# rrwick/Autocycler

Measured on NVIDIA H100. Metric: input-assembly Mbp/sec through compress->unitig GFA, higher is better.
Workload: dtype u64

## Files before the change

autocycler_b200/api.py:

```python
import ctypes as C
import os

_HERE = os.path.dirname(os.path.abspath(__file__))
DEFAULT_LIB = os.path.join(_HERE, "libautocycler_gpu.so")

AC_OK = 0


class AutocyclerGpuError(RuntimeError):
    def __init__(self, code, message):
        super().__init__(f"[{code}] {message}")
        self.code = code
        self.message = message


class AcConfig(C.Structure):
    _fields_ = [("k", C.c_uint32), ("device", C.c_int32), ("stream", C.c_void_p), ("keep_positions", C.c_uint32),
                ("n_devices", C.c_int32), ("devices", C.POINTER(C.c_int32))]


class AcCounts(C.Structure):
    _fields_ = [(n, C.c_uint64) for n in ("n_kmers", "n_unitigs", "n_links", "total_length", "seq_bytes", "n_fwd_pos",
                                         "n_rev_pos", "n_next", "n_sequences", "n_path_steps", "length_before_simplify")]


class AcUnitigs(C.Structure):
    _fields_ = [("number", C.POINTER(C.c_uint32)), ("seq_off", C.POINTER(C.c_uint64)), ("seq", C.POINTER(C.c_uint8)),
                ("depth", C.POINTER(C.c_double)),
                ("fpos_off", C.POINTER(C.c_uint64)), ("fpos", C.POINTER(C.c_uint32)), ("fpos_id_strand", C.POINTER(C.c_uint16)),
                ("rpos_off", C.POINTER(C.c_uint64)), ("rpos", C.POINTER(C.c_uint32)), ("rpos_id_strand", C.POINTER(C.c_uint16)),
                ("next_off", C.POINTER(C.c_uint64)), ("next", C.POINTER(C.c_int32))]


class AcTimings(C.Structure):
    _fields_ = [(n, C.c_float) for n in ("h2d", "pack", "insert", "adjacency", "boundaries", "runs", "unitigs", "links", "seed_sort", "emit", "d2h",
                                        "device_total", "host_graph", "host_simplify", "host_gfa", "sample", "device_simplify", "device_gfa", "insert_kernel", "trim_kernel")] + \
               [(n, C.c_uint64) for n in ("insert_occurrences", "table_capacity", "table_used", "kernel_launches", "h2d_bytes", "d2h_bytes")]

    def as_dict(self):
        return {n: getattr(self, n) for n, _ in self._fields_}


class AcResolveInfo(C.Structure):
    _fields_ = [("anchors", C.c_uint32), ("unique_bridges", C.c_uint32), ("conflicting_bridges", C.c_uint32), ("culled_bridges", C.c_uint32),
                ("jobs", C.c_uint64), ("cells", C.c_uint64), ("longest_path", C.c_uint64), ("shared_jobs", C.c_uint32), ("hbm_jobs", C.c_uint32),
                ("kernel_ms", C.c_float)]

    def as_dict(self):
        return {n: getattr(self, n) for n, _ in self._fields_}


EXPORTS = ["ac_last_error", "ac_version", "ac_create", "ac_destroy", "ac_add_sequence", "ac_clear_sequences", "ac_upload",
           "ac_build", "ac_compress", "ac_simplify", "ac_merge_linear_paths", "ac_renumber_unitigs", "ac_load_gfa", "ac_bind_host_to_device", "ac_decompress_gfa", "ac_pairwise_distances", "ac_distance_matrix_text", "ac_sequence_reconstruct", "ac_counts_get", "ac_unitigs_copy", "ac_path_copy", "ac_gfa_size", "ac_gfa_copy",
           "ac_timings_get", "ac_compress_dir", "ac_compress_dir_devices", "ac_load_sequences", "ac_sequence_get",
           "ac_build_local", "ac_entries_count", "ac_entries_export", "ac_entries_merge", "ac_runs_local", "ac_runs_export",
           "ac_runs_import", "ac_runs_import_padded", "ac_build_finish", "ac_compress_finish", "ac_gfa_data",
           "ac_compress_finish_split", "ac_path_tokens_export", "ac_path_lines_render", "ac_path_lines_data", "ac_upload_shard", "ac_strand_block",
           "ac_trim_paths", "ac_trim", "ac_trim_yaml", "ac_trim_stats", "ac_trim_dir",
           "ac_cluster", "ac_cluster_text", "ac_cluster_assignments", "ac_cluster_stats", "ac_upgma", "ac_cluster_dir",
           "ac_bridge_best_paths", "ac_resolve", "ac_resolve_text", "ac_resolve_stats", "ac_resolve_dir", "ac_combine_dir"]

_libs = {}


def load_library(path=None):
    path = os.path.abspath(path or DEFAULT_LIB)
    if path in _libs:
        return _libs[path]
    if not os.path.exists(path):
        raise AutocyclerGpuError(-2, f"{path} is missing: build it with `python -c 'import __graft_entry__ as g; g.build()'` "
                                     "(the GPU path has no CPU fallback)")
    lib = C.CDLL(path)
    lib.ac_last_error.restype = C.c_char_p
    lib.ac_last_error.argtypes = [C.c_void_p]
    lib.ac_version.restype = C.c_char_p
    lib.ac_create.argtypes = [C.POINTER(C.c_void_p), C.POINTER(AcConfig)]
    lib.ac_destroy.argtypes = [C.c_void_p]
    lib.ac_destroy.restype = None
    lib.ac_add_sequence.argtypes = [C.c_void_p, C.c_uint16, C.c_char_p, C.c_uint64, C.c_char_p, C.c_char_p]
    lib.ac_clear_sequences.argtypes = [C.c_void_p]
    for name in ("ac_upload", "ac_build", "ac_compress", "ac_simplify", "ac_renumber_unitigs"):
        getattr(lib, name).argtypes = [C.c_void_p]
    lib.ac_merge_linear_paths.argtypes = [C.c_void_p, C.c_int]
    lib.ac_load_gfa.argtypes = [C.c_void_p, C.c_char_p, C.c_uint64]
    lib.ac_bind_host_to_device.argtypes = [C.c_int32]
    lib.ac_pairwise_distances.argtypes = [C.c_void_p, C.POINTER(C.c_double), C.c_uint64]
    lib.ac_distance_matrix_text.argtypes = [C.c_void_p, C.c_void_p, C.c_uint64, C.POINTER(C.c_uint64)]
    lib.ac_decompress_gfa.argtypes = [C.c_char_p, C.c_char_p, C.c_char_p, C.c_int32, C.c_int32]
    lib.ac_sequence_reconstruct.argtypes = [C.c_void_p, C.c_uint64, C.c_void_p, C.c_uint64, C.POINTER(C.c_uint64)]
    lib.ac_counts_get.argtypes = [C.c_void_p, C.POINTER(AcCounts)]
    lib.ac_unitigs_copy.argtypes = [C.c_void_p, C.POINTER(AcUnitigs)]
    lib.ac_path_copy.argtypes = [C.c_void_p, C.c_uint64, C.POINTER(C.c_int32), C.c_uint64, C.POINTER(C.c_uint64)]
    lib.ac_gfa_size.argtypes = [C.c_void_p, C.POINTER(C.c_uint64)]
    lib.ac_gfa_copy.argtypes = [C.c_void_p, C.c_void_p, C.c_uint64]
    lib.ac_timings_get.argtypes = [C.c_void_p, C.POINTER(AcTimings)]
    lib.ac_compress_dir.argtypes = [C.c_char_p, C.c_char_p, C.c_uint32, C.c_uint32, C.c_uint32, C.c_int32, C.c_int32]
    lib.ac_compress_dir_devices.argtypes = [C.c_char_p, C.c_char_p, C.c_uint32, C.c_uint32, C.c_uint32, C.POINTER(C.c_int32), C.c_int32, C.c_int32]
    lib.ac_load_sequences.argtypes = [C.c_void_p, C.c_char_p, C.c_uint32, C.c_uint32, C.POINTER(C.c_uint64)]
    lib.ac_sequence_get.argtypes = [C.c_void_p, C.c_uint64, C.POINTER(C.c_uint16), C.POINTER(C.c_uint64), C.c_char_p, C.c_uint64,
                                    C.c_char_p, C.c_uint64, C.c_char_p, C.c_uint64]
    lib.ac_build_local.argtypes = [C.c_void_p, C.c_uint32, C.c_uint32, C.c_uint32]
    lib.ac_entries_count.argtypes = [C.c_void_p, C.POINTER(C.c_uint64)]
    lib.ac_entries_export.argtypes = [C.c_void_p, C.c_void_p, C.c_uint64]
    lib.ac_entries_merge.argtypes = [C.c_void_p, C.c_void_p, C.c_uint64]
    lib.ac_runs_local.argtypes = [C.c_void_p, C.POINTER(C.c_uint64)]
    lib.ac_runs_export.argtypes = [C.c_void_p, C.c_void_p, C.c_uint64]
    lib.ac_runs_import.argtypes = [C.c_void_p, C.c_void_p, C.c_uint64]
    lib.ac_runs_import_padded.argtypes = [C.c_void_p, C.c_void_p, C.c_uint64, C.POINTER(C.c_uint64), C.c_uint32]
    lib.ac_build_finish.argtypes = [C.c_void_p]
    lib.ac_compress_finish.argtypes = [C.c_void_p]
    lib.ac_compress_finish_split.argtypes = [C.c_void_p]
    lib.ac_upload_shard.argtypes = [C.c_void_p, C.c_uint32, C.c_uint32]
    lib.ac_strand_block.argtypes = [C.c_void_p, C.c_uint32, C.c_uint32, C.POINTER(C.c_void_p), C.POINTER(C.c_uint64)]
    lib.ac_path_tokens_export.argtypes = [C.c_void_p, C.c_void_p, C.c_uint64, C.POINTER(C.c_uint64), C.c_uint32]
    lib.ac_path_lines_render.argtypes = [C.c_void_p, C.c_void_p, C.c_uint64]
    lib.ac_path_lines_data.argtypes = [C.c_void_p, C.POINTER(C.c_void_p), C.POINTER(C.c_uint64)]
    lib.ac_gfa_data.argtypes = [C.c_void_p, C.POINTER(C.c_void_p), C.POINTER(C.c_uint64)]
    lib.ac_trim_paths.argtypes = [C.c_void_p, C.c_int32, C.POINTER(C.c_int32), C.POINTER(C.c_uint64), C.c_uint64, C.POINTER(C.c_uint32),
                                  C.c_uint64, C.c_double, C.c_uint32, C.POINTER(C.c_int32), C.POINTER(C.c_uint64), C.POINTER(C.c_uint8)]
    lib.ac_trim.argtypes = [C.c_void_p, C.c_double, C.c_uint32, C.c_double]
# ... 438 lines not shown
```

autocycler_b200/csrc/backend.h:

```cpp
#pragma once
#include <cstddef>
#include <cstdint>
#include <cstdio>
#include <cstdlib>
#include <cstring>
#include <stdexcept>
#include <string>

#ifdef AC_EMULATE
#define AC_HD inline
#define AC_D inline

template <class T> inline T ac_atomic_cas(T* p, T cmp, T val) { T old = *p; if (old == cmp) *p = val; return old; }
template <class T> inline T ac_atomic_add(T* p, T v) { T old = *p; *p = (T)(old + v); return old; }
template <class T> inline T ac_atomic_or(T* p, T v) { T old = *p; *p = (T)(old | v); return old; }
template <class T> inline T ac_atomic_and(T* p, T v) { T old = *p; *p = (T)(old & v); return old; }
template <class T> inline T ac_atomic_min(T* p, T v) { T old = *p; if (v < old) *p = v; return old; }
template <class T> inline T ac_atomic_max(T* p, T v) { T old = *p; if (v > old) *p = v; return old; }
template <class T> inline T ac_ld_volatile(const T* p) { return *p; }
template <class T> inline T ac_ld_cg(const T* p) { return *p; }
inline void ac_st_stream(uint32_t* p, uint32_t v) { *p = v; }
inline void ac_ld_group(const uint64_t* p, uint64_t out[4]) { out[0] = p[0]; out[1] = p[1]; out[2] = p[2]; out[3] = p[3]; }
inline uint64_t ac_umul64hi(uint64_t a, uint64_t b) { return (uint64_t)(((unsigned __int128)a * b) >> 64); }
inline uint32_t ac_popc(uint32_t v) { return (uint32_t)__builtin_popcount(v); }
inline int ac_ctz(uint32_t v) { return __builtin_ctz(v); }

struct AcStream { int dummy; };

inline void* ac_dev_alloc(size_t bytes) { void* p = malloc(bytes ? bytes : 1); if (!p) throw std::runtime_error("emu alloc failed"); return p; }
inline void ac_dev_free(void* p) { free(p); }
inline void ac_memset(void* p, int v, size_t bytes, AcStream*) { memset(p, v, bytes); }
inline void ac_h2d(void* d, const void* h, size_t bytes, AcStream*) { memcpy(d, h, bytes); }
inline void ac_d2h(void* h, const void* d, size_t bytes, AcStream*) { memcpy(h, d, bytes); }
inline void ac_copy_dd(void* dst, const void* src, size_t bytes, AcStream*) { memcpy(dst, src, bytes); }
inline void ac_sync(AcStream*) {}
inline void* ac_host_alloc(size_t bytes) { return malloc(bytes ? bytes : 1); }
inline void ac_host_free(void* p) { free(p); }

template <class Body> inline void ac_launch(const char*, AcStream*, const Body& body, uint64_t n);
template <int CTAS, class Body> inline void ac_launch_occ(const char* name, AcStream* st, const Body& body, uint64_t n) { ac_launch(name, st, body, n); }
template <class Body> inline void ac_launch(const char*, AcStream*, const Body& body, uint64_t n) {
    for (uint64_t i = 0; i < n; ++i) body(i);
}
struct AcGridSync { void operator()() const {} };
template <class Body> inline void ac_launch_coop(const char*, AcStream*, const Body& body, uint64_t, uint64_t = 256) { AcGridSync sync; body(0, 1, sync); }

#else
#include <cuda_runtime.h>

#ifdef __CUDACC__
#define AC_HD __host__ __device__ __forceinline__
#define AC_D __device__ __forceinline__
#else
#define AC_HD inline
#define AC_D inline
#endif

#define AC_CUDA_CHECK(expr) do { cudaError_t _e = (expr); if (_e != cudaSuccess) \
    throw std::runtime_error(std::string(#expr) + ": " + cudaGetErrorString(_e)); } while (0)

#ifdef __CUDACC__
AC_D uint64_t ac_atomic_cas(uint64_t* p, uint64_t cmp, uint64_t val) {
    return (uint64_t)atomicCAS((unsigned long long*)p, (unsigned long long)cmp, (unsigned long long)val);
}
AC_D uint32_t ac_atomic_cas(uint32_t* p, uint32_t cmp, uint32_t val) { return atomicCAS(p, cmp, val); }
AC_D uint32_t ac_atomic_add(uint32_t* p, uint32_t v) { return atomicAdd(p, v); }
AC_D uint64_t ac_atomic_add(uint64_t* p, uint64_t v) { return (uint64_t)atomicAdd((unsigned long long*)p, (unsigned long long)v); }
AC_D unsigned long long ac_atomic_add(unsigned long long* p, unsigned long long v) { return atomicAdd(p, v); }
AC_D uint32_t ac_atomic_or(uint32_t* p, uint32_t v) { return atomicOr(p, v); }
AC_D uint32_t ac_atomic_min(uint32_t* p, uint32_t v) { return atomicMin(p, v); }
AC_D uint32_t ac_atomic_max(uint32_t* p, uint32_t v) { return atomicMax(p, v); }
AC_D uint64_t ac_atomic_min(uint64_t* p, uint64_t v) { return (uint64_t)atomicMin((unsigned long long*)p, (unsigned long long)v); }
template <class T> AC_D T ac_ld_volatile(const T* p) { return *(const volatile T*)p; }
AC_D uint64_t ac_ld_cg(const uint64_t* p) { return (uint64_t)__ldcg(reinterpret_cast<const unsigned long long*>(p)); }
AC_D void ac_ld_group(const uint64_t* p, uint64_t out[4]) {
    asm volatile("ld.global.cg.v2.u64 {%0,%1}, [%2];" : "=l"(out[0]), "=l"(out[1]) : "l"(p) : "memory");
    asm volatile("ld.global.cg.v2.u64 {%0,%1}, [%2];" : "=l"(out[2]), "=l"(out[3]) : "l"(p + 2) : "memory");
}
AC_D void ac_st_stream(uint32_t* p, uint32_t v) { __stcs(p, v); }
AC_D uint64_t ac_umul64hi(uint64_t a, uint64_t b) { return __umul64hi(a, b); }
AC_D uint32_t ac_popc(uint32_t v) { return (uint32_t)__popc(v); }
AC_D int ac_ctz(uint32_t v) { return __ffs((int)v) - 1; }
AC_D uint64_t ac_atomic_or(uint64_t* p, uint64_t v) { return (uint64_t)atomicOr((unsigned long long*)p, (unsigned long long)v); }
AC_D uint64_t ac_atomic_and(uint64_t* p, uint64_t v) { return (uint64_t)atomicAnd((unsigned long long*)p, (unsigned long long)v); }
#endif

struct AcStream { cudaStream_t s; };

inline void* ac_dev_alloc(size_t bytes) { void* p = nullptr; AC_CUDA_CHECK(cudaMalloc(&p, bytes ? bytes : 1)); return p; }
inline void ac_dev_free(void* p) { if (p) cudaFree(p); }
inline void ac_memset(void* p, int v, size_t bytes, AcStream* st) { AC_CUDA_CHECK(cudaMemsetAsync(p, v, bytes, st->s)); }
inline void ac_h2d(void* d, const void* h, size_t bytes, AcStream* st) { AC_CUDA_CHECK(cudaMemcpyAsync(d, h, bytes, cudaMemcpyHostToDevice, st->s)); }
inline void ac_d2h(void* h, const void* d, size_t bytes, AcStream* st) { AC_CUDA_CHECK(cudaMemcpyAsync(h, d, bytes, cudaMemcpyDeviceToHost, st->s)); }
inline void ac_copy_dd(void* dst, const void* src, size_t bytes, AcStream* st) { AC_CUDA_CHECK(cudaMemcpyAsync(dst, src, bytes, cudaMemcpyDeviceToDevice, st->s)); }
inline void ac_sync(AcStream* st) { AC_CUDA_CHECK(cudaStreamSynchronize(st->s)); }
inline void ac_debug_sync(const char* name, AcStream* st) {
    static const bool on = getenv("AC_SYNC_LAUNCHES") != nullptr;
    if (!on) return;
    const cudaError_t e = cudaStreamSynchronize(st->s);
    if (e != cudaSuccess) throw std::runtime_error(std::string("kernel ") + name + " failed: " + cudaGetErrorString(e));
}
inline void* ac_host_alloc(size_t bytes) { void* p = nullptr; AC_CUDA_CHECK(cudaMallocHost(&p, bytes ? bytes : 1)); return p; }
inline void ac_host_free(void* p) { if (p) cudaFreeHost(p); }
inline uint64_t ac_sm_count() {
    static int sms = 0;
    if (!sms) { int dev = 0; cudaGetDevice(&dev); cudaDeviceGetAttribute(&sms, cudaDevAttrMultiProcessorCount, dev); if (sms <= 0) sms = 132; }
    return (uint64_t)sms;
}

#ifdef __CUDACC__
#include <cooperative_groups.h>
extern unsigned long long g_ac_kernel_launches;

template <class Body> __global__ void __launch_bounds__(256) ac_body_kernel(const Body body, uint64_t n) {
    const uint64_t stride = (uint64_t)gridDim.x * blockDim.x;
    const uint32_t lane = threadIdx.x & 31u;
    for (uint64_t base = (uint64_t)blockIdx.x * blockDim.x + (threadIdx.x - lane); base < n; base += stride) {
        const uint64_t i = base + lane;
        if (i < n) body(i);
        __syncwarp();
    }
}

template <class Body, int CTAS> __global__ void __launch_bounds__(256, CTAS) ac_body_kernel_occ(const Body body, uint64_t n) {
    const uint64_t stride = (uint64_t)gridDim.x * blockDim.x;
    const uint32_t lane = threadIdx.x & 31u;
    for (uint64_t base = (uint64_t)blockIdx.x * blockDim.x + (threadIdx.x - lane); base < n; base += stride) {
        const uint64_t i = base + lane;
        if (i < n) body(i);
        __syncwarp();
    }
}
template <int CTAS, class Body> inline void ac_launch_occ(const char* name, AcStream* st, const Body& body, uint64_t n) {
    if (n == 0) return;
    const int threads = 256;
    const uint64_t want = (n + threads - 1) / threads, max_blocks = ac_sm_count() * (uint64_t)CTAS * 2;
    const unsigned blocks = (unsigned)(want < max_blocks ? want : max_blocks);
    ac_body_kernel_occ<Body, CTAS><<<blocks, threads, 0, st->s>>>(body, n);
    cudaError_t e = cudaGetLastError();
    if (e != cudaSuccess) throw std::runtime_error(std::string("launch ") + name + ": " + cudaGetErrorString(e));
    ++g_ac_kernel_launches;
    ac_debug_sync(name, st);
}

struct AcGridSync { __device__ __forceinline__ void operator()() const { cooperative_groups::this_grid().sync(); } };
template <class Body> __global__ void __launch_bounds__(256) ac_coop_kernel(const Body body) {
    AcGridSync sync;
    body((uint64_t)blockIdx.x * blockDim.x + threadIdx.x, (uint64_t)gridDim.x * blockDim.x, sync);
}
template <class Body> inline void ac_launch_coop(const char* name, AcStream* st, const Body& body, uint64_t work, uint64_t per_block = 256) {
    static int resident = 0;
    if (!resident) {
        int per_sm = 0;
        cudaOccupancyMaxActiveBlocksPerMultiprocessor(&per_sm, ac_coop_kernel<Body>, 256, 0);
        resident = per_sm * (int)ac_sm_count();
        if (resident <= 0) throw std::runtime_error(std::string("cooperative launch ") + name + ": kernel does not fit");
    }
    uint64_t want = (work + per_block - 1) / per_block;
    if (want < 1) want = 1;
    const int sms = (int)ac_sm_count();
    const uint64_t cap = resident < sms ? (uint64_t)resident : (uint64_t)sms;
    const unsigned blocks = (unsigned)(want < cap ? want : cap);
    void* args[] = {(void*)&body};
    cudaError_t e = cudaLaunchCooperativeKernel((void*)ac_coop_kernel<Body>, dim3(blocks), dim3(256), args, 0, st->s);
    if (e != cudaSuccess) throw std::runtime_error(std::string("cooperative launch ") + name + ": " + cudaGetErrorString(e));
    ++g_ac_kernel_launches;
    ac_debug_sync(name, st);
}

template <class Body> inline void ac_launch(const char* name, AcStream* st, const Body& body, uint64_t n) {
    if (n == 0) return;
    const int threads = 256;
    uint64_t want = (n + threads - 1) / threads;
    const uint64_t max_blocks = ac_sm_count() * 16;
    unsigned blocks = (unsigned)(want < max_blocks ? want : max_blocks);
    ac_body_kernel<Body><<<blocks, threads, 0, st->s>>>(body, n);
    cudaError_t e = cudaGetLastError();
    if (e != cudaSuccess) throw std::runtime_error(std::string("launch ") + name + ": " + cudaGetErrorString(e));
    ++g_ac_kernel_launches;
    ac_debug_sync(name, st);
}
#endif
#endif
```

autocycler_b200/csrc/c_api.cpp:

```cpp
#include "../../include/autocycler_gpu.h"

#include <sched.h>
#include <dirent.h>
#include <sys/stat.h>
#include <unistd.h>
#include <zlib.h>

#include <algorithm>
#include <cerrno>
#include <chrono>
#include <cstdio>
#include <cstring>
#include <memory>
#include <string>
#include <vector>

#include "backend.h"
#include "host_graph.h"
#include "host_io.h"
#include "host_cluster.h"
#include "host_trim.h"
#include "host_resolve.h"
#include <immintrin.h>
#include <functional>
// ... 605 lines not shown
        if (o->seq) memcpy(o->seq + so, g.seq_ptr(u), g.rec[u].len);
        so += g.rec[u].len;
        if (o->fpos_off) o->fpos_off[n] = fo;
        if (o->rpos_off) o->rpos_off[n] = ro;
        if (have_pos) {
            for (uint64_t x = g.fpos_off[u]; x < g.fpos_off[u + 1]; ++x) { if (o->fpos) o->fpos[fo] = (uint32_t)(g.fpos[x] >> 16); if (o->fpos_id_strand) o->fpos_id_strand[fo] = (uint16_t)(g.fpos[x] & 0xFFFF); ++fo; }
            for (uint64_t x = g.rpos_off[u]; x < g.rpos_off[u + 1]; ++x) { if (o->rpos) o->rpos[ro] = (uint32_t)(g.rpos[x] >> 16); if (o->rpos_id_strand) o->rpos_id_strand[ro] = (uint16_t)(g.rpos[x] & 0xFFFF); ++ro; }
        }
        for (uint32_t rev = 0; rev < 2; ++rev) {
            if (o->next_off) o->next_off[2 * (size_t)n + rev] = no;
            const UStrand from = us_make(u, rev != 0);
            for (uint32_t x = g.next_off[from]; x < g.next_off[from + 1]; ++x) {
                if (o->next) { const int32_t num = (int32_t)g.number[us_index(g.next[x])]; o->next[no] = us_reverse(g.next[x]) ? -num : num; }
                ++no;
            }
        }
    }
    if (o->seq_off) o->seq_off[g.U] = so;
    if (o->fpos_off) o->fpos_off[g.U] = fo;
    if (o->rpos_off) o->rpos_off[g.U] = ro;
    if (o->next_off) o->next_off[2 * (size_t)g.U] = no;
    return ok(h);
    AC_GUARD_END(h)
}

int ac_path_copy(const ac_handle* h, uint64_t seq_index, int32_t* out, uint64_t cap, uint64_t* n) {
    if (!h || !n) return set_error(h, AC_EINVAL, "null argument");
    AC_GUARD_BEGIN
    if (h->built) ensure_graph(h);
    const HostGraph& g = h->graph;
    if (!h->built || seq_index >= g.n_seqs) return set_error(h, AC_EINVAL, "no such sequence");
    const uint64_t a = g.path_off[seq_index], b = g.path_off[seq_index + 1];
    *n = b - a;
    if (!out) return ok(h);
    if (cap < b - a) return set_error(h, AC_ERANGE, "path buffer too small");
    for (uint64_t x = a; x < b; ++x) { const int32_t num = (int32_t)g.number[us_index(g.path[x])]; out[x - a] = us_reverse(g.path[x]) ? -num : num; }
    return ok(h);
    AC_GUARD_END(h)
}

int ac_gfa_size(ac_handle* h, uint64_t* n_bytes) {
    if (!h || !n_bytes) return set_error(h, AC_EINVAL, "null argument");
    AC_GUARD_BEGIN
    if (!h->built) return set_error(h, AC_EINVAL, "ac_build must precede ac_gfa_size");
    if (!h->gfa_ready) {
        const double t0 = now_ms();
        ensure_graph(h);
        h->graph.gfa_text(h->seqs, h->gfa);
        h->gfa_ptr = h->gfa.data(); h->gfa_len = h->gfa.size();
        h->t.host_gfa = (float)(now_ms() - t0);
        h->gfa_ready = true;
        if (getenv("AC_HOST_PROFILE")) {
            const HostProfile& p = h->graph.prof;
            fprintf(stderr, "[host] adopt %.1f renumber(total) %.1f expand %.1f (%d passes; candidates %.1f, +compare %.1f, pass1 %.1f) gfa %.1f ms; U=%u\n",
                    p.adopt, p.renumber, p.expand, p.passes, p.candidates, p.compare, p.pass1, (double)h->t.host_gfa, h->graph.U);
        }
    }
    *n_bytes = h->gfa_len;
    return ok(h);
    AC_GUARD_END(h)
}

int ac_gfa_data(ac_handle* h, const char** data, uint64_t* n_bytes) {
    if (!data) return set_error(h, AC_EINVAL, "null argument");
    int rc = ac_gfa_size(h, n_bytes);
    if (rc != AC_OK) return rc;
    *data = h->gfa_ptr;
    return ok(h);
}

int ac_gfa_copy(ac_handle* h, char* buf, uint64_t cap) {
    uint64_t n = 0;
    int rc = ac_gfa_size(h, &n);
    if (rc != AC_OK) return rc;
    if (!buf || cap < n) return set_error(h, AC_ERANGE, "GFA buffer too small");
    memcpy(buf, h->gfa_ptr, n);
    return ok(h);
}

int ac_timings_get(const ac_handle* h, ac_timings* out) {
    if (!h || !out) return set_error(h, AC_EINVAL, "null argument");
    *out = h->t;
    out->kernel_launches = h->pipe->kernel_launches();
    return ok(h);
}

int ac_load_sequences(ac_handle* h, const char* dir, uint32_t max_contigs, uint32_t threads, uint64_t* assembly_count) {
    if (!h || !dir) return set_error(h, AC_EINVAL, "null argument");
    AC_GUARD_BEGIN
    ac_clear_sequences(h);
    const bool device_repair = h->cfg.k / 2 <= 64;
    LoadedInput in = load_sequences(dir, h->cfg.k, max_contigs, threads ? threads : 1, false, device_repair ? h->pipe.get() : nullptr);
    for (size_t i = 0; i < in.seqs.size(); ++i) {
        int rc = ac_add_sequence(h, in.seqs[i].id, (const uint8_t*)in.padded[i].data(), in.padded[i].size(),
                                 in.seqs[i].filename.c_str(), in.seqs[i].contig_header.c_str());
        if (rc != AC_OK) return rc;
    }
    if (assembly_count) *assembly_count = in.assembly_count;
    in.padded.clear(); in.padded.shrink_to_fit();
    h->loaded = std::move(in);
    return ok(h);
    AC_GUARD_END(h)
}

int ac_sequence_get(const ac_handle* h, uint64_t index, uint16_t* seq_id, uint64_t* length, char* fwd, uint64_t cap_fwd,
                    char* filename, uint64_t cap_fn, char* header, uint64_t cap_hd) {
    if (!h) return set_error(nullptr, AC_EINVAL, "null handle");
    if (index >= h->seqs.size()) return set_error(h, AC_EINVAL, "no such sequence");
    const HostSeq& s = h->seqs[index];
    const uint64_t padded = s.length + h->cfg.k - 1;
    if (seq_id) *seq_id = s.id;
    if (length) *length = s.length;
    if (fwd) {
        if (!h->ascii.p || h->infos.empty()) return set_error(h, AC_EINVAL, "this handle holds a loaded graph: its sequences have no bytes (use ac_sequence_reconstruct)");
        if (cap_fwd < padded + 1) return set_error(h, AC_ERANGE, "buffer too small");
        memcpy(fwd, h->ascii.p + s.start, padded); fwd[padded] = 0;
    }
    if (filename) { if (cap_fn < s.filename.size() + 1) return set_error(h, AC_ERANGE, "buffer too small"); memcpy(filename, s.filename.c_str(), s.filename.size() + 1); }
    if (header) { if (cap_hd < s.contig_header.size() + 1) return set_error(h, AC_ERANGE, "buffer too small"); memcpy(header, s.contig_header.c_str(), s.contig_header.size() + 1); }
    return ok(h);
}

int ac_sequence_reconstruct(const ac_handle* h, uint64_t index, char* out, uint64_t cap, uint64_t* length) {
    if (!h) return set_error(nullptr, AC_EINVAL, "null handle");
    AC_GUARD_BEGIN
    if (!h->built) return set_error(h, AC_EINVAL, "ac_build must precede ac_sequence_reconstruct");
    if (index >= h->seqs.size()) return set_error(h, AC_EINVAL, "no such sequence");
    ensure_graph(h);
    const HostGraph& g = h->graph;
    uint64_t total = 0;
    for (uint64_t x = g.path_off[index]; x < g.path_off[index + 1]; ++x) total += g.rec[us_index(g.path[x])].len;
    if (length) *length = total;
    if (!out) return ok(h);
    if (cap < total) return set_error(h, AC_ERANGE, "buffer too small");
    char* p = out;
    for (uint64_t x = g.path_off[index]; x < g.path_off[index + 1]; ++x) {
        const UStrand s = g.path[x]; const uint32_t n = g.rec[us_index(s)].len; const char* src = g.seq_ptr(us_index(s));
        if (!us_reverse(s)) memcpy(p, src, n);
        else for (uint32_t j = 0; j < n; ++j) { const char b = src[n - 1 - j]; p[j] = b == 'A' ? 'T' : b == 'C' ? 'G' : b == 'G' ? 'C' : b == 'T' ? 'A' : b; }
        p += n;
    }
    return ok(h);
    AC_GUARD_END(h)
}

int ac_compress_dir(const char* assemblies_dir, const char* autocycler_dir, uint32_t k, uint32_t max_contigs, uint32_t threads,
                    int32_t device, int32_t verbose) {
    return ac_compress_dir_devices(assemblies_dir, autocycler_dir, k, max_contigs, threads, &device, 1, verbose);
}

int ac_compress_dir_devices(const char* assemblies_dir, const char* autocycler_dir, uint32_t k, uint32_t max_contigs, uint32_t threads,
                            const int32_t* devices, int32_t n_devices, int32_t verbose) {
    if (!assemblies_dir || !autocycler_dir || !devices || n_devices < 1) return set_error(nullptr, AC_EINVAL, "null argument");
    ac_handle* h = nullptr;
    AC_GUARD_BEGIN
    struct stat st;
    if (stat(assemblies_dir, &st) != 0) return set_error(nullptr, AC_EINPUT, std::string("directory does not exist: ") + assemblies_dir);
    if (!S_ISDIR(st.st_mode)) return set_error(nullptr, AC_EINPUT, std::string(assemblies_dir) + " is not a directory");
    if (stat(autocycler_dir, &st) == 0 && !S_ISDIR(st.st_mode)) return set_error(nullptr, AC_EINPUT, std::string(autocycler_dir) + " exists but is not a directory");
    if (k < 11) return set_error(nullptr, AC_EINPUT, "--kmer cannot be less than 11");
    if (k > 501) return set_error(nullptr, AC_EINPUT, "--kmer cannot be greater than 501");
    if (k % 2 == 0) return set_error(nullptr, AC_EINPUT, "--kmer must be odd");
    if (threads < 1) return set_error(nullptr, AC_EINPUT, "--threads cannot be less than 1");
    if (threads > 100) return set_error(nullptr, AC_EINPUT, "--threads cannot be greater than 100");
    if (k > AC_MAX_K) return set_error(nullptr, AC_EINPUT, "--kmer above " + std::to_string(AC_MAX_K) + " is not supported by this build of the GPU path (there is no CPU fallback)");
    ac_config cfg{}; cfg.k = k; cfg.device = devices[0]; cfg.stream = nullptr; cfg.keep_positions = 0; cfg.n_devices = n_devices; cfg.devices = devices;
// ... 537 lines not shown
```

autocycler_b200/csrc/pipeline.cu:

```cuda
#include "pipeline.h"

#include <algorithm>
#include <cmath>
#include <vector>

#ifndef AC_EMULATE
unsigned long long g_ac_kernel_launches = 0;
#else
static unsigned long long g_ac_kernel_launches = 0;
#endif

#define AC_NONE32 0xFFFFFFFFu
#define AC_CHUNK 32
#define AC_MINCHUNK 128
#define AC_MAX_RANKS 16
#define AC_BOUND_STRIPES 64
#ifndef AC_INSERT_CTAS
#define AC_INSERT_CTAS 2
#endif

struct TableView {
    Slot* slots;
    uint64_t cap;
    const uint64_t* packed;
    const SeqInfo* seqs;
    uint32_t n_seqs;
    uint32_t* count_big;
    uint32_t gb;
    uint32_t alarm;
};
AC_D uint64_t table_home(const TableView& t, uint64_t h) { return ac_umul64hi(h, t.cap >> 2) << 2; }
AC_D uint32_t table_depth(const TableView& t, uint64_t slot) { return t.count_big ? t.count_big[slot] : slot_count(t.slots[slot]); }

template <int W> AC_D Key<W> window_key(const TableView& t, uint64_t g, bool dotted, const KParams& p) {
    Key<W> key = fetch_codes<W>(t.packed, g, p);
    if (dotted) {
        const SeqInfo s = t.seqs[find_seq(t.seqs, t.n_seqs, g)];
        key.d = window_dots(s, g - s.start, p.k);
    }
    return key;
}

template <int W> AC_D uint32_t table_find(const TableView& t, const Key<W>& a, const Key<W>& arc, const KParams& p) {
    const uint64_t h = key_hash(key_select(key_is_canonical(a, p), a, arc));
    const uint32_t tag = make_tag(a.d != 0, h, t.gb);
    uint64_t slot = table_home(t, h);
    for (;;) {
        const Slot e = t.slots[slot];
        if (e == AC_EMPTY_SLOT) return AC_NONE32;
        if (slot_tag(e, t.gb) == tag) {
            Key<W> rep = window_key<W>(t, slot_gpos(e, t.gb), a.d != 0, p);
            if (key_eq(rep, a) || key_eq(rep, arc)) return (uint32_t)slot;
        }
        if (++slot == t.cap) slot = 0;
    }
}

AC_D void slot_add_occurrence(const TableView& t, uint64_t slot, Slot seen, uint64_t g, uint32_t add, uint32_t flags, bool track_min, unsigned long long* counters) {
    if (!t.count_big && slot_count(seen) + add >= t.alarm) counters[3] = 1;
    if (!track_min) {
        if (t.count_big) ac_atomic_add(&t.count_big[slot], add);
        else ac_atomic_add(&t.slots[slot], (uint64_t)add << AC_SLOT_COUNT_SHIFT);
        if (flags & ~slot_flags(seen)) ac_atomic_or(&t.slots[slot], (uint64_t)flags);
        return;
    }
    if (t.count_big) ac_atomic_add(&t.count_big[slot], add);
    Slot old = seen;
    for (;;) {
        Slot nw = old | flags;
        if (!t.count_big) { nw += (uint64_t)add << AC_SLOT_COUNT_SHIFT; if (slot_count(old) + add >= t.alarm) counters[3] = 1; }
        if (g < slot_gpos(old, t.gb)) nw = slot_with_gpos(nw, g, t.gb);
        const Slot was = ac_atomic_cas(&t.slots[slot], old, nw);
        if (was == old) return;
        old = was;
    }
}

template <int W, class F> AC_D void for_each_successor(const Key<W>& a, const Key<W>& arc, bool any_dotted, const KParams& p, F&& f) {
    if (a.d == 0) {
        for (uint64_t x = 0; x < 4; ++x) {
            Key<W> s = a, src = arc;
            key_push_right(s, x, p); key_push_left(src, 3 - x, p);
            f(s, src);
        }
        if (any_dotted) { Key<W> s = a; key_push_right(s, 0, p); s.d = -1; f(s, key_rc(s, p)); }
    } else if (a.d > 0) {
        for (uint64_t x = 0; x < 4; ++x) { Key<W> s = a; key_push_right(s, x, p); s.d = a.d - 1; f(s, key_rc(s, p)); }
        if (a.d == 1) { Key<W> s = a; key_push_right(s, 0, p); s.d = -1; f(s, key_rc(s, p)); }
    } else {
        Key<W> s = a; key_push_right(s, 0, p); s.d = a.d - 1; f(s, key_rc(s, p));
    }
}

struct PackBody {
    const uint8_t* ascii; uint64_t total; uint64_t* packed; const SeqInfo* seqs; uint32_t n_seqs; uint8_t* interior;
// ... 601 lines not shown
        }
        uint32_t n = 0;
        for_each_successor<W>(tail, tail_rc, any_dotted, p, [&](const Key<W>& a, const Key<W>& arc) {
            const uint32_t s2 = table_find<W>(t, a, arc, p);
            if (s2 == AC_NONE32) return;
            const uint32_t j2 = slot_unitig[s2];
            const DeviceUnitig v = unitigs[j2];
            const bool a_canon = key_is_canonical(a, p);
            const bool head_fwd = v.head_slot == s2 && ((packed_base(t.packed, v.start + p.h) < 2) == a_canon);
            if (n < AC_MAX_LINKS) links[i * AC_MAX_LINKS + n] = (j2 << 1) | (head_fwd ? 0u : 1u);
            ++n;
        });
        link_count[i] = n;
    }
};

struct alignas(16) SortRec { uint64_t a, b; uint32_t c, d, id, pad; };
struct SeedLess {
    const DeviceUnitig* unitigs; int W;
    typedef SortRec Key;
    AC_D Key load(uint32_t id) const {
        const DeviceUnitig& x = unitigs[id];
        Key k; k.id = id; k.pad = 0; k.a = x.min_w[0]; k.b = W > 1 ? x.min_w[1] : 0; k.c = x.min_d > 0 ? (uint32_t)x.min_d : 0u; k.d = x.min_d < 0 ? (uint32_t)-x.min_d : 0u;
        return k;
    }
    AC_D bool less_keys(const Key& x, const Key& y, uint32_t ia, uint32_t ib) const {
        if (x.c != y.c) return x.c > y.c;
        if (x.a != y.a) return x.a < y.a;
        if (x.b != y.b) return x.b < y.b;
        if (W > 2) return (*this)(ia, ib);
        return x.d > y.d;
    }
    AC_D bool operator()(uint32_t a, uint32_t b) const {
        const DeviceUnitig& x = unitigs[a]; const DeviceUnitig& y = unitigs[b];
        const int lx = x.min_d > 0 ? x.min_d : 0, ly = y.min_d > 0 ? y.min_d : 0;
        if (lx != ly) return lx > ly;
        for (int w = 0; w < W; ++w) if (x.min_w[w] != y.min_w[w]) return x.min_w[w] < y.min_w[w];
        const int tx = x.min_d < 0 ? -x.min_d : 0, ty = y.min_d < 0 ? -y.min_d : 0;
        return tx > ty;
    }
};
#define AC_SORT_LEAF 8
#define AC_SORT_WAYS 8
template <class Less> struct MergeWaysBody {
    Less less; uint32_t n, width, steps; const SortRec* in; SortRec* out; uint32_t* idx_out;
    AC_D void operator()(uint64_t i) const {
        const SortRec me = in[i];
        const uint64_t run = i / width, group = run / AC_SORT_WAYS, group_start = group * AC_SORT_WAYS * (uint64_t)width;
        uint32_t lo[AC_SORT_WAYS], hi[AC_SORT_WAYS];
#pragma unroll
        for (int s = 0; s < AC_SORT_WAYS; ++s) {
            const uint64_t first = group_start + (uint64_t)s * width, last = first + width;
            lo[s] = (uint32_t)(first < n ? first : n); hi[s] = (uint32_t)(last < n ? last : n);
            if (group * AC_SORT_WAYS + s == run) hi[s] = lo[s];
        }
        for (uint32_t step = 0; step < steps; ++step) {
#pragma unroll
            for (int s = 0; s < AC_SORT_WAYS; ++s) {
                if (lo[s] < hi[s]) {
                    const uint32_t mid = (lo[s] + hi[s]) >> 1;
                    const SortRec x = in[mid];
                    const bool earlier = group * AC_SORT_WAYS + s < run;
                    const bool before = earlier ? !less.less_keys(me, x, me.id, x.id) : less.less_keys(x, me, x.id, me.id);
                    if (before) lo[s] = mid + 1; else hi[s] = mid;
                }
            }
        }
        uint64_t pos = group_start + (i - run * width);
#pragma unroll
        for (int s = 0; s < AC_SORT_WAYS; ++s) {
            const uint64_t first = group_start + (uint64_t)s * width;
            if (group * AC_SORT_WAYS + s != run && first < n) pos += lo[s] - (uint32_t)first;
        }
        out[pos] = me; idx_out[pos] = me.id;
    }
};

#ifndef AC_EMULATE
#define AC_SORT_TILE 2048
#else
#define AC_SORT_TILE 16
#endif
#ifndef AC_EMULATE
template <class Less> __global__ void __launch_bounds__(1024) ac_tile_sort_kernel(const Less less, uint32_t n, uint32_t* __restrict__ idx, SortRec* __restrict__ recs) {
    extern __shared__ __align__(16) unsigned char tile_smem[];
    SortRec* keys = reinterpret_cast<SortRec*>(tile_smem);
    uint16_t* buf0 = reinterpret_cast<uint16_t*>(tile_smem + AC_SORT_TILE * sizeof(SortRec));
    uint16_t* buf1 = buf0 + AC_SORT_TILE;
    const uint32_t base = blockIdx.x * AC_SORT_TILE, count = n - base < AC_SORT_TILE ? n - base : AC_SORT_TILE;
    for (uint32_t i = threadIdx.x; i < count; i += blockDim.x) { SortRec r = less.load(base + i); r.id = base + i; r.pad = 0; keys[i] = r; }
    __syncthreads();
    auto before = [&](uint32_t x, uint32_t y) { return less.less_keys(keys[x], keys[y], base + x, base + y); };
    if (threadIdx.x < AC_SORT_TILE / AC_SORT_LEAF) {
        const uint32_t a = threadIdx.x * AC_SORT_LEAF, b = a + AC_SORT_LEAF < count ? a + AC_SORT_LEAF : count;
        uint16_t v[AC_SORT_LEAF];
        for (uint32_t x = a; x < b; ++x) {
            uint32_t y = x - a;
            while (y > 0 && before(x, v[y - 1])) { v[y] = v[y - 1]; --y; }
            v[y] = (uint16_t)x;
        }
        for (uint32_t x = a; x < b; ++x) buf0[x] = v[x - a];
    }
    __syncthreads();
    uint16_t* in = buf0; uint16_t* out = buf1;
    for (uint32_t width = AC_SORT_LEAF; width < count; width *= 2) {
        for (uint32_t i = threadIdx.x; i < count; i += blockDim.x) {
            const uint32_t me = in[i];
            const uint32_t run = i / width, pair_start = (run & ~1u) * width, run_start = run * width;
            const bool left = !(run & 1u);
            uint32_t lo, hi;
            if (left) { lo = run_start + width; hi = lo + width; } else { lo = pair_start; hi = run_start; }
            if (lo > count) lo = count;
            if (hi > count) hi = count;
            const uint32_t first = lo;
            while (lo < hi) { const uint32_t mid = (lo + hi) >> 1; const bool bf = left ? before(in[mid], me) : !before(me, in[mid]); if (bf) lo = mid + 1; else hi = mid; }
            out[pair_start + (i - run_start) + (lo - first)] = (uint16_t)me;
        }
        __syncthreads();
        uint16_t* t = in; in = out; out = t;
    }
    for (uint32_t i = threadIdx.x; i < count; i += blockDim.x) { const SortRec r = keys[in[i]]; recs[base + i] = r; idx[base + i] = r.id; }
}
#endif
template <class Less> struct TileSortBody {
    Less less; uint32_t n; uint32_t* idx; SortRec* recs;
    AC_D void operator()(uint64_t c) const {
        const uint32_t a = (uint32_t)c * AC_SORT_TILE, b = a + AC_SORT_TILE < n ? a + AC_SORT_TILE : n;
        for (uint32_t x = a; x < b; ++x) {
            uint32_t y = x;
            while (y > a && less(x, idx[y - 1])) { idx[y] = idx[y - 1]; --y; }
            idx[y] = x;
        }
        for (uint32_t x = a; x < b; ++x) { SortRec r = less.load(idx[x]); r.id = idx[x]; r.pad = 0; recs[x] = r; }
    }
};
template <class Less> static uint32_t* sort_indices(AcStream* stream, const Less& less, uint32_t n, uint32_t* a, uint32_t* b, SortRec* ra, SortRec* rb) {
    if (n == 0) return a;
    const uint64_t tiles = ((uint64_t)n + AC_SORT_TILE - 1) / AC_SORT_TILE;
#ifndef AC_EMULATE
    const size_t smem = AC_SORT_TILE * (sizeof(SortRec) + 2 * sizeof(uint16_t));
    AC_CUDA_CHECK(cudaFuncSetAttribute(ac_tile_sort_kernel<Less>, cudaFuncAttributeMaxDynamicSharedMemorySize, (int)smem));
    ac_tile_sort_kernel<Less><<<(unsigned)tiles, 1024, smem, stream->s>>>(less, n, a, ra); ++g_ac_kernel_launches;
    cudaError_t e = cudaGetLastError();
    if (e != cudaSuccess) throw std::runtime_error(std::string("launch tile sort: ") + cudaGetErrorString(e));
    ac_debug_sync("tile_sort", stream);
#else
    ac_launch("tile_sort", stream, TileSortBody<Less>{less, n, a, ra}, tiles);
#endif
    for (uint64_t width = AC_SORT_TILE; width < n; width *= AC_SORT_WAYS) {
        uint32_t steps = 1; while ((1ull << steps) <= width) ++steps;
        ac_launch("merge_pass", stream, MergeWaysBody<Less>{less, n, (uint32_t)width, steps, ra, rb, b}, n);
        std::swap(a, b); std::swap(ra, rb);
    }
    return a;
}

struct NumberKeyBody {
    const UnitigRec* rec; const char* arena; uint64_t* prefix;
    AC_D void operator()(uint64_t s) const {
        const unsigned char* q = (const unsigned char*)(arena + rec[s].seq_off);
        const uint32_t m = rec[s].len < 8 ? rec[s].len : 8;
        uint64_t v = 0;
        for (uint32_t i = 0; i < m; ++i) v |= (uint64_t)q[i] << (56 - 8 * i);
        prefix[s] = v;
    }
};
struct InversePermBody { const uint32_t* order; uint32_t* pos; AC_D void operator()(uint64_t n) const { pos[order[n]] = (uint32_t)n; } };
struct NumberLess {
    const UnitigRec* rec; const uint32_t* depth; const char* arena; const uint64_t* prefix;
    const uint32_t* pos;
    typedef SortRec Key;
    AC_D Key load(uint32_t id) const { Key k; k.id = id; k.pad = 0; k.a = prefix[id]; k.b = pos ? pos[id] : id; k.c = rec[id].len; k.d = depth[id]; return k; }
    AC_D bool less_keys(const Key& x, const Key& y, uint32_t ia, uint32_t ib) const {
        if (x.c != y.c) return x.c > y.c;
        if (x.a != y.a) return x.a < y.a;
        if (x.c > 8) return (*this)(ia, ib);
        if (x.d != y.d) return x.d > y.d;
        return x.b < y.b;
    }
    AC_D bool operator()(uint32_t a, uint32_t b) const {
        const uint32_t la = rec[a].len, lb = rec[b].len;
        if (la != lb) return la > lb;
        if (prefix[a] != prefix[b]) return prefix[a] < prefix[b];
        const char* x = arena + rec[a].seq_off; const char* y = arena + rec[b].seq_off;
        for (uint32_t i = 8; i < la; ++i) if (x[i] != y[i]) return (unsigned char)x[i] < (unsigned char)y[i];
        if (depth[a] != depth[b]) return depth[a] > depth[b];
        return pos ? pos[a] < pos[b] : a < b;
    }
};


struct SeedGatherBody {
    const uint32_t* perm; const DeviceUnitig* unitigs; uint32_t n;
    uint32_t* rank; uint32_t* len; uint32_t* depth; uint32_t* need; uint32_t* min_fpos; uint32_t* min_rpos;
    AC_D void operator()(uint64_t s) const {
        if (s == n) { need[s] = 0; return; }
        const uint32_t j = perm[s];
        const DeviceUnitig& u = unitigs[j];
        rank[j] = (uint32_t)s; len[s] = u.len; depth[s] = u.depth; need[s] = u.len + 2 * AC_SEQ_SLACK;
        min_fpos[s] = 0xFFFFFFFFu; min_rpos[s] = 0xFFFFFFFFu;
    }
};
struct SeqOffBody { const uint32_t* need_off; uint64_t* seq_off; AC_D void operator()(uint64_t s) const { seq_off[s] = (uint64_t)need_off[s] + AC_SEQ_SLACK; } };

struct EmitSeqBody {
    const uint64_t* packed; uint32_t h; const DeviceUnitig* unitigs; uint32_t n_unitigs; const uint32_t* chunk_off;
    const uint32_t* rank; const uint64_t* seq_off; char* arena;
    AC_D void operator()(uint64_t c) const {
        uint32_t lo = 0, hi = n_unitigs;
        while (hi - lo > 1) { uint32_t mid = (lo + hi) >> 1; if (chunk_off[mid] <= c) lo = mid; else hi = mid; }
        const DeviceUnitig u = unitigs[lo];
        const uint64_t first = (c - chunk_off[lo]) * AC_MINCHUNK;
        const uint64_t n = (u.len - first < AC_MINCHUNK) ? u.len - first : AC_MINCHUNK;
        char* dst = arena + seq_off[rank[lo]];
        const uint64_t g0 = u.start + h + first;
        if (!u.flip) for (uint64_t t = 0; t < n; ++t) dst[first + t] = "ACGT"[packed_base(packed, g0 + t)];
        else for (uint64_t t = 0; t < n; ++t) dst[u.len - 1 - (first + t)] = "TGCA"[packed_base(packed, g0 + t)];
    }
};

AC_D UStrand seed_strand(uint32_t dev_strand, const uint32_t* rank, const DeviceUnitig* unitigs) {
    const uint32_t j = dev_strand >> 1;
    return (rank[j] << 1) | ((dev_strand & 1u) ^ (unitigs[j].flip & 1u));
}

struct LinkCountBody {
    const uint32_t* link_count; const uint32_t* rank; const DeviceUnitig* unitigs; uint32_t n_strands; uint32_t* cnt;
    AC_D void operator()(uint64_t i) const {
        if (i == n_strands) { cnt[i] = 0; return; }
        cnt[seed_strand((uint32_t)i, rank, unitigs)] = link_count[i];
    }
};

struct LinkOrderBody {
// ... 787 lines not shown
#define AC_BRIDGE_THREADS 256
AC_HD uint32_t bridge_weight(const uint32_t* w, int32_t u) { return w[u < 0 ? (uint32_t)(-(int64_t)u) : (uint32_t)u]; }
AC_HD void bridge_cell(uint32_t* cur, const uint32_t* prev, const uint32_t* prev2, uint32_t i, uint32_t j, const int32_t* pa, const int32_t* pb,
                       const uint32_t* w) {
    if (i == 0) { cur[0] = prev[0] + bridge_weight(w, pb[j - 1]); return; }
    const int32_t a = pa[i - 1];
    const uint32_t wa = bridge_weight(w, a);
    if (j == 0) { cur[i] = prev[i - 1] + wa; return; }
    const int32_t b = pb[j - 1];
    const uint32_t wb = bridge_weight(w, b);
    const uint32_t match_or_mismatch = prev2[i - 1] + (a == b ? 0u : (wa > wb ? wa : wb));
    const uint32_t delete_cost = prev[i - 1] + wa, insert_cost = prev[i] + wb;
    const uint32_t m = match_or_mismatch < delete_cost ? match_or_mismatch : delete_cost;
    cur[i] = m < insert_cost ? m : insert_cost;
}
AC_HD uint32_t bridge_diag_lo(uint32_t d, uint32_t m) { return d > m ? d - m : 0u; }
AC_HD uint32_t bridge_diag_hi(uint32_t d, uint32_t n) { return d < n ? d : n; }
struct BridgeLaunchJob { uint64_t a_off, b_off, scratch_off; uint32_t n, m, slot, pad; };

#ifndef AC_EMULATE
__global__ void __launch_bounds__(AC_BRIDGE_THREADS) ac_bridge_distance_kernel(const BridgeLaunchJob* __restrict__ jobs, const int32_t* __restrict__ values,
                                                                               const uint32_t* __restrict__ weights, uint32_t* scratch,
                                                                               uint32_t* __restrict__ dist, int use_shared) {
    extern __shared__ uint32_t bridge_smem[];
    const BridgeLaunchJob J = jobs[blockIdx.x];
    const uint32_t n = J.n, m = J.m, stride = n + 1;
    uint32_t* D = use_shared ? bridge_smem : scratch + J.scratch_off;
    const int32_t* pa = values + J.a_off;
    const int32_t* pb = values + J.b_off;
    if (threadIdx.x == 0) D[0] = 0;
    __syncthreads();
    for (uint32_t d = 1; d <= n + m; ++d) {
        uint32_t* cur = D + (size_t)(d % 3) * stride;
        const uint32_t* prev = D + (size_t)((d - 1) % 3) * stride;
        const uint32_t* prev2 = D + (size_t)((d + 1) % 3) * stride;
        const uint32_t hi = bridge_diag_hi(d, n);
        for (uint32_t i = bridge_diag_lo(d, m) + threadIdx.x; i <= hi; i += AC_BRIDGE_THREADS) bridge_cell(cur, prev, prev2, i, d - i, pa, pb, weights);
        __syncthreads();
    }
    if (threadIdx.x == 0) dist[J.slot] = D[(size_t)((n + m) % 3) * stride + n];
}
#endif

#ifndef AC_EMULATE
#define AC_SCAN_TILE 4096
__global__ void __launch_bounds__(256) ac_scan_reduce_kernel(const uint32_t* __restrict__ in, uint64_t n, uint32_t* __restrict__ sums) {
    const uint64_t tile0 = (uint64_t)blockIdx.x * AC_SCAN_TILE;
    uint32_t s = 0;
#pragma unroll
    for (int r = 0; r < AC_SCAN_TILE / 256; ++r) { const uint64_t i = tile0 + (uint64_t)r * 256 + threadIdx.x; if (i < n) s += in[i]; }
    for (int o = 16; o; o >>= 1) s += __shfl_down_sync(0xFFFFFFFFu, s, o);
    __shared__ uint32_t w[8];
    if ((threadIdx.x & 31) == 0) w[threadIdx.x >> 5] = s;
    __syncthreads();
    if (threadIdx.x == 0) { uint32_t t = 0; for (int i = 0; i < 8; ++i) t += w[i]; sums[blockIdx.x] = t; }
}
__global__ void __launch_bounds__(256) ac_scan_apply_kernel(const uint32_t* in, uint64_t n, const uint32_t* __restrict__ block_off, uint32_t* out) {
    __shared__ uint32_t warp_tot[8];
    const uint32_t lane = threadIdx.x & 31, warp = threadIdx.x >> 5;
    uint32_t carry = block_off ? block_off[blockIdx.x] : 0;
    const uint64_t tile0 = (uint64_t)blockIdx.x * AC_SCAN_TILE;
#pragma unroll 1
    for (int r = 0; r < AC_SCAN_TILE / 1024; ++r) {
        const uint64_t i = tile0 + (uint64_t)r * 1024 + threadIdx.x * 4;
        uint32_t v[4];
        if (i + 3 < n) { const uint4 q = *reinterpret_cast<const uint4*>(in + i); v[0] = q.x; v[1] = q.y; v[2] = q.z; v[3] = q.w; }
        else { for (int j = 0; j < 4; ++j) v[j] = (i + j < n) ? in[i + j] : 0; }
        const uint32_t t = v[0] + v[1] + v[2] + v[3];
        uint32_t inc = t;
        for (int o = 1; o < 32; o <<= 1) { const uint32_t u = __shfl_up_sync(0xFFFFFFFFu, inc, o); if (lane >= (uint32_t)o) inc += u; }
        if (lane == 31) warp_tot[warp] = inc;
        __syncthreads();
        uint32_t wbase = 0, total = 0;
        for (uint32_t w2 = 0; w2 < 8; ++w2) { const uint32_t x = warp_tot[w2]; if (w2 < warp) wbase += x; total += x; }
        uint32_t e = carry + wbase + inc - t;
        if (i + 3 < n) { uint4 q; q.x = e; q.y = e + v[0]; q.z = q.y + v[1]; q.w = q.z + v[2]; *reinterpret_cast<uint4*>(out + i) = q; }
        else { for (int j = 0; j < 4; ++j) { if (i + j < n) out[i + j] = e; e += v[j]; } }
        carry += total;
        __syncthreads();
    }
}
#define AC_SCAN_STATE(epoch, status, value) (((unsigned long long)(epoch) << 34) | ((unsigned long long)(status) << 32) | (unsigned long long)(value))
__global__ void __launch_bounds__(256) ac_scan_chained_kernel(const uint32_t* in, uint64_t n, uint32_t* out, unsigned long long* state, unsigned long long epoch,
                                                               unsigned long long* ticket, unsigned long long ticket_base, uint32_t n_tiles, uint32_t* total_out) {
    __shared__ uint32_t warp_tot[8];
    __shared__ uint32_t s_tile, s_prefix;
    const uint32_t lane = threadIdx.x & 31, warp = threadIdx.x >> 5;
    if (threadIdx.x == 0) s_tile = (uint32_t)(atomicAdd(ticket, 1ull) - ticket_base);
    __syncthreads();
    const uint32_t tile = s_tile;
    const uint64_t tile0 = (uint64_t)tile * AC_SCAN_TILE;
    uint32_t v[AC_SCAN_TILE / 1024][4], t[AC_SCAN_TILE / 1024], mine = 0;
#pragma unroll
    for (int r = 0; r < AC_SCAN_TILE / 1024; ++r) {
        const uint64_t i = tile0 + (uint64_t)r * 1024 + threadIdx.x * 4;
        if (i + 3 < n) { const uint4 q = *reinterpret_cast<const uint4*>(in + i); v[r][0] = q.x; v[r][1] = q.y; v[r][2] = q.z; v[r][3] = q.w; }
        else { for (int j = 0; j < 4; ++j) v[r][j] = (i + j < n) ? in[i + j] : 0; }
        t[r] = v[r][0] + v[r][1] + v[r][2] + v[r][3]; mine += t[r];
    }
    uint32_t sum = mine;
    for (int o = 16; o; o >>= 1) sum += __shfl_down_sync(0xFFFFFFFFu, sum, o);
    if (lane == 0) warp_tot[warp] = sum;
    __syncthreads();
    if (warp == 0) {
        uint32_t total = 0;
        for (int w2 = 0; w2 < 8; ++w2) total += warp_tot[w2];
        uint32_t prefix = 0;
        if (tile > 0) {
            if (lane == 0) *(volatile unsigned long long*)&state[tile] = AC_SCAN_STATE(epoch, 1, total);
            for (int64_t first = (int64_t)tile - 1; first >= 0; first -= 32) {
                const int64_t j = first - lane;
                unsigned long long w = AC_SCAN_STATE(epoch, 2, 0);
                if (j >= 0) do { w = *(volatile unsigned long long*)&state[j]; } while ((w >> 34) != epoch || ((w >> 32) & 3ull) == 0);
                const unsigned closed = __ballot_sync(0xFFFFFFFFu, ((w >> 32) & 3ull) == 2);
                const int stop = closed ? __ffs((int)closed) - 1 : 31;
                uint32_t part = (int)lane <= stop ? (uint32_t)w : 0u;
                for (int o = 16; o; o >>= 1) part += __shfl_down_sync(0xFFFFFFFFu, part, o);
                prefix += __shfl_sync(0xFFFFFFFFu, part, 0);
                if (closed) break;
            }
        }
        if (lane == 0) {
            *(volatile unsigned long long*)&state[tile] = AC_SCAN_STATE(epoch, 2, prefix + total);
            s_prefix = prefix;
            if (tile + 1 == n_tiles && total_out) *total_out = prefix + total;
        }
    }
    __syncthreads();
    uint32_t carry = s_prefix;
#pragma unroll
    for (int r = 0; r < AC_SCAN_TILE / 1024; ++r) {
        const uint64_t i = tile0 + (uint64_t)r * 1024 + threadIdx.x * 4;
        uint32_t inc = t[r];
        for (int o = 1; o < 32; o <<= 1) { const uint32_t u = __shfl_up_sync(0xFFFFFFFFu, inc, o); if (lane >= (uint32_t)o) inc += u; }
        __syncthreads();
        if (lane == 31) warp_tot[warp] = inc;
        __syncthreads();
        uint32_t wbase = 0, total = 0;
        for (uint32_t w2 = 0; w2 < 8; ++w2) { const uint32_t x = warp_tot[w2]; if (w2 < warp) wbase += x; total += x; }
        uint32_t e = carry + wbase + inc - t[r];
        if (i + 3 < n) { uint4 q; q.x = e; q.y = e + v[r][0]; q.z = q.y + v[r][1]; q.w = q.z + v[r][2]; *reinterpret_cast<uint4*>(out + i) = q; }
        else { for (int j = 0; j < 4; ++j) { if (i + j < n) out[i + j] = e; e += v[r][j]; } }
        carry += total;
    }
}
#endif

struct DevBuf {
    void* p = nullptr; size_t cap = 0;
    void ensure(size_t bytes) {
        if (bytes > cap) {
            ac_dev_free(p); p = nullptr; cap = 0; p = ac_dev_alloc(bytes); cap = bytes;
#ifdef AC_EMULATE
            static const bool poison = getenv("AC_EMU_POISON") != nullptr;
            if (poison) memset(p, 0xA5, cap);
#endif
        }
    }
    template <class T> T* as() { return (T*)p; }
    ~DevBuf() { ac_dev_free(p); }
};

struct PinBuf {
    void* p = nullptr; size_t cap = 0;
    void ensure(size_t bytes) { if (bytes > cap) { ac_host_free(p); p = nullptr; cap = 0; p = ac_host_alloc(bytes); cap = bytes; } }
    template <class T> T* as() { return (T*)p; }
    ~PinBuf() { ac_host_free(p); }
};

struct DevicePipeline::Impl {
    int device = 0;
    AcStream stream;
    bool own_stream = false;
    uint64_t total = 0; uint32_t n_seqs = 0, k = 0; int W = 0;
    DevBuf ascii, packed, seqs, slots, pos_slot, flags8, bmask, bcount, boff, counters, uid_rep, slot_unitig;
    DevBuf run_start, run_len, run_uk, run_dir, is_rep, rep_idx, run_unitig, unitigs, nchunks, chunk_off, partial, link_count, links;
    DevBuf scan_tmp[4];
    DevBuf d_fixed, cand_flag, cand_index, d_cands, d_cand_at, d_deps, d_spec;
    DevBuf sort_a, sort_b, sort_ra, sort_rb, num_prefix, rank, d_len, d_depth, need, d_seq_off, d_arena, d_min_fpos, d_min_rpos;
    DevBuf strand_cnt, d_next_off, d_next, prev_cnt, d_prev_off, d_prev, d_path, d_path_off;
    DevBuf d_rec;
    PinBuf h_cands, h_deps, h_spec, h_fixed;
    DevBuf dist_member, dist_shared, d_pred, d_level, d_flagmax, d_counters64, d_dirty, d_exhausted, d_arena2, d_arena3, d_pos, sort_c, sort_d, d_pos2, gfa_s_size, gfa_l_size, gfa_p_size, gfa_pieces, d_text, d_ptext, d_last, d_pbound, d_due;
    PinBuf h_order2, h_text, h_ptext, h_pbound;
    PinBuf h_rec, h_depth, h_order, h_arena, h_next_off, h_next, h_prev_off, h_prev, h_path, h_path_off, h_run_start, h_run_len;
#ifndef AC_EMULATE
    cudaEvent_t ev[24];
#endif

    void mark(int i) {
#ifndef AC_EMULATE
        AC_CUDA_CHECK(cudaEventRecord(ev[i], stream.s));
#else
        (void)i;
#endif
    }
    void wait_mark(int i) {
#ifndef AC_EMULATE
        AC_CUDA_CHECK(cudaEventSynchronize(ev[i]));
#else
        (void)i;
#endif
    }
    bool arena_pending = false;
    const std::function<void()>* before_results = nullptr;
    void do_complete(PipelineResult& out);
    float between(int a, int b) {
#ifndef AC_EMULATE
        float ms = 0; AC_CUDA_CHECK(cudaEventElapsedTime(&ms, ev[a], ev[b])); return ms;
#else
        (void)a; (void)b; return 0.f;
#endif
    }

#ifndef AC_EMULATE
    DevBuf scan_state; unsigned long long scan_epoch = 0, scan_tickets = 0;
    uint32_t exclusive_scan(const uint32_t* in, uint32_t* out, uint64_t n, int = 0, bool want_total = true) {
        if (n == 0) return 0;
        const uint64_t nb = (n + AC_SCAN_TILE - 1) / AC_SCAN_TILE;
        if (nb > 0x7FFFFFFFull) throw std::runtime_error("scan too large");
        if ((nb + 4) * 8 > scan_state.cap) {
            scan_state.ensure((nb + 4) * 8 * 2);
            ac_memset(scan_state.p, 0, scan_state.cap, &stream);
            scan_tickets = 0;
        }
        unsigned long long* st = scan_state.as<unsigned long long>();
        scan_epoch = (scan_epoch + 1) & 0x3FFFFFFFull; if (scan_epoch == 0) scan_epoch = 1;
        ac_scan_chained_kernel<<<(unsigned)nb, 256, 0, stream.s>>>(in, n, out, st + 2, scan_epoch, st, scan_tickets, (uint32_t)nb, (uint32_t*)(st + 1)); ++g_ac_kernel_launches;
        scan_tickets += nb;
        cudaError_t e = cudaGetLastError();
        if (e != cudaSuccess) throw std::runtime_error(std::string("launch scan: ") + cudaGetErrorString(e));
        ac_debug_sync("scan", &stream);
        uint32_t total_sum = 0;
        if (want_total) { ac_d2h(&total_sum, st + 1, sizeof(uint32_t), &stream); ac_sync(&stream); }
        return total_sum;
    }
#else
    uint32_t exclusive_scan(const uint32_t* in, uint32_t* out, uint64_t n, int level = 0, bool want_total = true) {
        if (n == 0) return 0;
        if (level >= 4) throw std::runtime_error("scan too deep");
        const uint64_t tile = 256;
        const uint64_t nb = (n + tile - 1) / tile;
        scan_tmp[level].ensure((nb + 4) * sizeof(uint32_t));
        uint32_t* sums = scan_tmp[level].as<uint32_t>();
        if (nb > 0x7FFFFFFFull) throw std::runtime_error("scan too large");
        ac_launch("scan_reduce", &stream, ScanReduceBody{in, n, sums}, nb);
        uint32_t total_sum = 0;
        if (nb == 1) {
            if (want_total) { ac_d2h(&total_sum, sums, sizeof(uint32_t), &stream); ac_sync(&stream); }
            ac_launch("scan_apply", &stream, ScanApplyBody{in, n, nullptr, out}, nb);
        } else {
            total_sum = exclusive_scan(sums, sums, nb, level + 1, want_total);
            ac_launch("scan_apply", &stream, ScanApplyBody{in, n, sums, out}, nb);
        }
        return total_sum;
    }
#endif

    std::vector<SeqInfo> host_seqs;
    uint64_t cap = 0, n_windows = 0, n_runs = 0, g_begin = 0, g_end = 0, n_slots_used = 0, n_dotted = 0, n_fwords = 0;
    bool any_dotted = false, is_multi = false, big_counts = false;
    int stage = 0;
    DevBuf run_hs, run_ts, claimed, claimed_cnt, occ_list, ext_filter, needles, hits, count_big, interior8;
    TableView table_view() { return TableView{slots.as<Slot>(), cap, packed.as<uint64_t>(), seqs.as<SeqInfo>(), n_seqs, big_counts ? count_big.as<uint32_t>() : nullptr, slot_gpos_bits(total), count_alarm()}; }
    static uint32_t count_alarm() { static const uint32_t a = getenv("AC_COUNT_ALARM") ? (uint32_t)atoi(getenv("AC_COUNT_ALARM")) : AC_SLOT_COUNT_ALARM; return a; }
    void set_device() {
#ifndef AC_EMULATE
        AC_CUDA_CHECK(cudaSetDevice(device));
#endif
    }
    template <int W> void local_w(uint32_t seq_lo, uint32_t seq_hi, bool multi);
    template <int W> void insert_w();
    uint64_t safe_cap = 0;
    int table_attempt = 0;
    std::vector<std::pair<const void*, uint64_t>> merged;
    template <int W> void merge_w(const void* dev_ptr, uint64_t n);
    template <int W> void runs_local_w();
    template <int W> void finish_w(PipelineResult& out, bool keep_positions, bool fused, bool split_paths);
    struct Pending {
        uint32_t U = 0, n_strands = 0; uint64_t n_links = 0, n_cands = 0;
        uint32_t* order_built = nullptr; uint32_t* final_order = nullptr; uint8_t* fix_start = nullptr;
        DevBuf* arena_src = nullptr; uint64_t arena_final = 0;
        bool any_moved = false, gfa_on_device = false, hairpins_ready = false, paths_split = false;
        uint64_t bases_removed = 0, gfa_bytes = 0;
    } R;
    bool pending_keep_positions = false;
    void pull_graph(PipelineResult& out, bool keep_positions);
    DevBuf d_small, d_totals, d_wrap_off, d_pre_len, d_suf_len, d_blob, d_blob_off;
    std::vector<char> path_blob; std::vector<uint32_t> path_pre, path_suf; uint64_t path_wrap_total = 0;
    void scan_keep_total(uint32_t* x, uint64_t n, uint32_t* total_dst) {
        exclusive_scan(x, x, n, 0, false);
        ac_copy_dd(total_dst, x + (n - 1), 4, &stream);
    }
    uint64_t uploaded_bytes = 0;
    uint64_t exp_n = 0, n_own_runs = 0; uint32_t own_seq_lo = 0, own_seq_hi = 0; bool exp_valid = false;
    void do_export_path_tokens(void* dst, uint64_t stride, const uint64_t* counts, uint32_t n_ranks);
    void do_render_path_lines(const void* tokens, uint64_t n_tokens, const char** text, uint64_t* bytes);
    DevBuf d_own_off, d_own_last, d_own_size; uint64_t path_lines_d2h = 0;
    template <int W> uint64_t list_claimed(bool with_filter);
    template <int W> uint64_t do_count_entries();
    void do_export_entries(void* dst, uint64_t cap_records);
    void do_export_runs(void* dst, uint64_t cap_records);
    void do_import_runs(const void* dev_ptr, uint64_t n);
    void do_import_runs_from(const void* const* ptrs, const uint64_t* counts, uint32_t n_ranks);
    DevBuf own_entries, own_runs;
    DevBuf trim_jobs, trim_vals, trim_w, trim_bits, trim_scratch, trim_out, trim_len;
    DevBuf br_jobs, br_vals, br_w, br_scratch, br_dist;
    DevBuf dist_asym, upgma_m, upgma_alive, upgma_cnt, upgma_node, upgma_rd, upgma_rj, upgma_list, upgma_out, upgma_done;
    uint32_t sym_n = 0;
    void upload_paths(const UStrand* path, const uint64_t* path_off, uint32_t n, const uint32_t* unitig_len, uint32_t U);
    void share_lengths(uint64_t steps, uint32_t n, uint32_t U);
#ifdef AC_EMULATE
    void poison() {
        static const bool on = getenv("AC_EMU_POISON") != nullptr;
        if (!on) return;
        DevBuf* all[] = {&packed, &slots, &pos_slot, &flags8, &bmask, &bcount, &boff, &counters, &uid_rep, &slot_unitig, &run_start, &run_len, &run_uk, &run_dir, &is_rep, &rep_idx,
                         &run_unitig, &unitigs, &nchunks, &chunk_off, &partial, &link_count, &links, &scan_tmp[0], &scan_tmp[1], &scan_tmp[2], &scan_tmp[3], &d_fixed, &cand_flag, &cand_index,
                         &d_cands, &d_cand_at, &d_deps, &d_spec, &sort_a, &sort_b, &sort_ra, &sort_rb, &num_prefix, &rank, &d_len, &d_depth, &need, &d_seq_off, &d_arena, &d_min_fpos, &d_min_rpos,
                         &strand_cnt, &d_next_off, &d_next, &prev_cnt, &d_prev_off, &d_prev, &d_path, &d_path_off, &d_rec, &d_pred, &d_level, &d_flagmax, &d_counters64, &d_dirty, &d_exhausted,
                         &d_arena2, &d_arena3, &d_pos, &sort_c, &sort_d, &d_pos2, &gfa_s_size, &gfa_l_size, &gfa_p_size, &gfa_pieces, &d_text, &d_ptext, &d_last, &run_hs, &run_ts, &claimed,
                         &claimed_cnt, &occ_list, &ext_filter, &count_big, &interior8, &d_small, &d_totals, &d_own_off, &d_own_last, &d_own_size, &own_entries, &own_runs, &d_due};
        for (DevBuf* b : all) if (b->p) memset(b->p, 0xA5, b->cap);
    }
    void poison_table() {
        static const bool on = getenv("AC_EMU_POISON") != nullptr;
        if (!on) return;
        DevBuf* all[] = {&slots, &pos_slot, &claimed, &claimed_cnt, &occ_list, &count_big, &counters};
        for (DevBuf* b : all) if (b->p) memset(b->p, 0xA5, b->cap);
    }
#else
    void poison() {}
    void poison_table() {}
#endif
};

DevicePipeline::DevicePipeline(int device, void* stream) : impl(new Impl) {
    impl->device = device; impl->before_results = &before_results;
#ifndef AC_EMULATE
    int n = 0;
    cudaError_t e = cudaGetDeviceCount(&n);
    if (e != cudaSuccess || n == 0)
        throw std::runtime_error(std::string("autocycler_gpu: no CUDA device available (") + cudaGetErrorString(e) +
                                 "); this library has no CPU path");
    AC_CUDA_CHECK(cudaSetDevice(device));
    if (stream) { impl->stream.s = (cudaStream_t)stream; }
    else { AC_CUDA_CHECK(cudaStreamCreateWithFlags(&impl->stream.s, cudaStreamNonBlocking)); impl->own_stream = true; }
    for (auto& ev : impl->ev) AC_CUDA_CHECK(cudaEventCreate(&ev));
#else
    (void)stream;
#endif
}

DevicePipeline::~DevicePipeline() {
#ifndef AC_EMULATE
    cudaSetDevice(impl->device);
    for (auto& ev : impl->ev) cudaEventDestroy(ev);
#endif
    Impl* p = impl; impl = nullptr;
#ifndef AC_EMULATE
    cudaStream_t s = p->stream.s; bool own = p->own_stream;
    delete p;
    if (own) cudaStreamDestroy(s);
#else
    delete p;
#endif
}

unsigned long long DevicePipeline::kernel_launches() const { return g_ac_kernel_launches; }

void DevicePipeline::upload(const uint8_t* ascii, uint64_t total, const SeqInfo* seqs, uint32_t n_seqs, uint32_t k, uint32_t seq_lo, uint32_t seq_hi) {
    Impl& m = *impl;
#ifndef AC_EMULATE
    AC_CUDA_CHECK(cudaSetDevice(m.device));
#endif
    if (k < 3 || (k & 1) == 0) throw std::runtime_error("k must be odd and >= 3");
    const int W = (int)((2 * k + 63) / 64);
    if (W > AC_MAX_W) throw std::runtime_error("k-mer sizes above " + std::to_string(AC_MAX_K) + " are not supported by the GPU path (no CPU fallback exists)");
    if (total >= 0xFFFFFFF0ull) throw std::runtime_error("more than 2^32 padded input bytes are not supported");
    if (n_seqs == 0 || total == 0) throw std::runtime_error("no sequences");
    m.total = total; m.n_seqs = n_seqs; m.k = k; m.W = W; m.stage = 0;
    m.host_seqs.assign(seqs, seqs + n_seqs);
    m.mark(0);
    m.ascii.ensure(total);
    if (seq_lo == 0 && seq_hi >= n_seqs) { ac_h2d(m.ascii.p, ascii, total, &m.stream); m.uploaded_bytes = total; }
    else {
        if (seq_lo > seq_hi || seq_hi > n_seqs) throw std::runtime_error("bad sequence shard");
        const uint64_t b0 = seq_lo < n_seqs ? seqs[seq_lo].start : total, b1 = seq_hi < n_seqs ? seqs[seq_hi].start : total;
        if (b1 > b0) ac_h2d(m.ascii.as<uint8_t>() + b0, ascii + b0, b1 - b0, &m.stream);
        m.uploaded_bytes = b1 - b0;
    }
    m.seqs.ensure(n_seqs * sizeof(SeqInfo));
    ac_h2d(m.seqs.p, seqs, n_seqs * sizeof(SeqInfo), &m.stream);
    if (m.path_pre.size() == n_seqs) {
        std::vector<uint64_t> wrap((size_t)n_seqs + 1, 0), boff((size_t)n_seqs + 1, 0);
        for (uint32_t i = 0; i < n_seqs; ++i) { wrap[i + 1] = wrap[i] + m.path_pre[i] + m.path_suf[i]; boff[i + 1] = wrap[i + 1]; }
        m.path_wrap_total = wrap[n_seqs];
        m.d_wrap_off.ensure(wrap.size() * 8); m.d_blob_off.ensure(boff.size() * 8); m.d_pre_len.ensure((size_t)n_seqs * 4); m.d_suf_len.ensure((size_t)n_seqs * 4); m.d_blob.ensure(m.path_blob.size() + 8);
        ac_h2d(m.d_wrap_off.p, wrap.data(), wrap.size() * 8, &m.stream); ac_h2d(m.d_blob_off.p, boff.data(), boff.size() * 8, &m.stream);
        ac_h2d(m.d_pre_len.p, m.path_pre.data(), (size_t)n_seqs * 4, &m.stream); ac_h2d(m.d_suf_len.p, m.path_suf.data(), (size_t)n_seqs * 4, &m.stream);
        if (!m.path_blob.empty()) ac_h2d(m.d_blob.p, m.path_blob.data(), m.path_blob.size(), &m.stream);
        ac_sync(&m.stream);
    } else m.path_wrap_total = 0;
    m.mark(1);
}

void DevicePipeline::set_path_line_texts(const char* blob, const uint32_t* prefix_len, const uint32_t* suffix_len, uint32_t n) {
    Impl& m = *impl;
    m.path_pre.assign(prefix_len, prefix_len + n); m.path_suf.assign(suffix_len, suffix_len + n);
    uint64_t bytes = 0; for (uint32_t i = 0; i < n; ++i) bytes += (uint64_t)prefix_len[i] + suffix_len[i];
    m.path_blob.assign(blob, blob + bytes);
}

void DevicePipeline::Impl::upload_paths(const UStrand* path, const uint64_t* path_off, uint32_t n, const uint32_t* unitig_len, uint32_t U) {
    const uint64_t steps = path_off[n];
    const uint32_t words = (n + 31) / 32;
    d_path.ensure(steps * 4 + 4); d_path_off.ensure(((size_t)n + 1) * 8); d_len.ensure((size_t)U * 4 + 4);
    dist_member.ensure((size_t)U * words * 4 + 4); dist_shared.ensure((size_t)n * n * 8);
    if (steps) ac_h2d(d_path.p, path, steps * 4, &stream);
    ac_h2d(d_path_off.p, path_off, ((size_t)n + 1) * 8, &stream);
    if (U) ac_h2d(d_len.p, unitig_len, (size_t)U * 4, &stream);
    ac_memset(dist_member.p, 0, (size_t)U * words * 4 + 4, &stream);
    ac_memset(dist_shared.p, 0, (size_t)n * n * 8, &stream);
}
void DevicePipeline::Impl::share_lengths(uint64_t steps, uint32_t n, uint32_t U) {
    const uint32_t words = (n + 31) / 32;
    ac_launch("path_member", &stream, PathMemberBody{d_path.as<UStrand>(), d_path_off.as<uint64_t>(), n, words, dist_member.as<uint32_t>()}, steps);
    ac_launch("pair_share", &stream, PairShareBody{dist_member.as<uint32_t>(), d_len.as<uint32_t>(), n, words, dist_shared.as<unsigned long long>()}, U);
}

void DevicePipeline::pair_shared_lengths(const UStrand* path, const uint64_t* path_off, uint32_t n, const uint32_t* unitig_len, uint32_t U, uint64_t* shared) {
    Impl& m = *impl; m.set_device();
    if (n == 0) return;
    m.upload_paths(path, path_off, n, unitig_len, U);
    m.share_lengths(path_off[n], n, U);
    ac_d2h(shared, m.dist_shared.p, (size_t)n * n * 8, &m.stream);
    ac_sync(&m.stream);
}

float DevicePipeline::cluster_distances(const UStrand* path, const uint64_t* path_off, uint32_t n, const uint32_t* unitig_len, uint32_t U, double* asym) {
    Impl& m = *impl; m.set_device();
    m.sym_n = 0;
    if (n == 0) return 0.f;
    const size_t nn = (size_t)n * n;
    m.dist_asym.ensure(nn * 8); m.upgma_m.ensure(nn * 8);
    float ms = 0.f;
    m.upload_paths(path, path_off, n, unitig_len, U);
#ifndef AC_EMULATE
    cudaEvent_t e0, e1;
    AC_CUDA_CHECK(cudaEventCreate(&e0)); AC_CUDA_CHECK(cudaEventCreate(&e1));
    AC_CUDA_CHECK(cudaEventRecord(e0, m.stream.s));
#endif
// ... 246 lines not shown
    std::vector<uint32_t> own;
    for (const BridgeLaunchJob& L : lj) {
        const uint32_t stride = L.n + 1;
        uint32_t* D;
        if (L.n <= shared_n) { own.assign(3 * (size_t)stride, 0xA5A5A5A5u); D = own.data(); }
        else D = m.br_scratch.as<uint32_t>() + L.scratch_off;
        D[0] = 0;
        for (uint32_t d = 1; d <= L.n + L.m; ++d) {
            uint32_t* cur = D + (size_t)(d % 3) * stride;
            const uint32_t* prev = D + (size_t)((d - 1) % 3) * stride;
            const uint32_t* prev2 = D + (size_t)((d + 1) % 3) * stride;
            for (uint32_t i = bridge_diag_lo(d, L.m); i <= bridge_diag_hi(d, L.n); ++i) bridge_cell(cur, prev, prev2, i, d - i, vals + L.a_off, vals + L.b_off, w);
        }
        m.br_dist.as<uint32_t>()[L.slot] = D[(size_t)((L.n + L.m) % 3) * stride + L.n];
    }
    ac_d2h(dist, m.br_dist.p, (size_t)n_jobs * 4, &m.stream);
#endif
    return ms;
}

void DevicePipeline::find_literals(const uint8_t* ascii_host, uint64_t total_bytes, const SeqInfo* host_seq, uint32_t n, uint32_t h,
                                   const uint64_t* needle_words, uint32_t n_needles, std::vector<LiteralHit>& out) {
    Impl& m = *impl; m.set_device();
    const int WH = (int)((2 * h + 63) / 64);
    if (WH > 2) throw std::runtime_error("end repair literals longer than 64 bases are not supported by the GPU path");
    const KParams p = make_kparams(h, WH);
    m.ascii.ensure(total_bytes); ac_h2d(m.ascii.p, ascii_host, total_bytes, &m.stream);
    m.seqs.ensure(n * sizeof(SeqInfo)); ac_h2d(m.seqs.p, host_seq, n * sizeof(SeqInfo), &m.stream);
    const uint64_t n_words = (total_bytes + 31) / 32;
    m.packed.ensure((n_words + 6) * sizeof(uint64_t));
    ac_memset(m.packed.as<uint64_t>() + n_words, 0, 6 * sizeof(uint64_t), &m.stream);
    ac_launch("pack", &m.stream, PackBody{m.ascii.as<uint8_t>(), total_bytes, m.packed.as<uint64_t>(), nullptr, 0, nullptr}, n_words);
    uint64_t cap = 64; while (cap < 4ull * n_needles) cap <<= 1;
    std::vector<NeedleSlot> table(cap);
    for (auto& t : table) { t.w[0] = t.w[1] = 0; t.id = 0; t.used = 0; }
    for (uint32_t i = 0; i < n_needles; ++i) {
        Key<2> k2; k2.w[0] = needle_words[2 * i]; k2.w[1] = needle_words[2 * i + 1]; k2.d = 0;
        uint64_t hsh;
        if (WH == 1) { Key<1> k1; k1.w[0] = k2.w[1]; k1.d = 0; hsh = key_hash(k1); } else hsh = key_hash(k2);
        uint64_t slot = hsh & (cap - 1);
        while (table[slot].used) slot = (slot + 1) & (cap - 1);
        table[slot].w[0] = WH == 1 ? k2.w[1] : k2.w[0]; table[slot].w[1] = k2.w[1]; table[slot].id = i; table[slot].used = 1;
    }
    m.needles.ensure(cap * sizeof(NeedleSlot)); ac_h2d(m.needles.p, table.data(), cap * sizeof(NeedleSlot), &m.stream);
    m.counters.ensure(8 * sizeof(unsigned long long));
    uint64_t hit_cap = 1u << 20;
    for (;;) {
        m.hits.ensure(hit_cap * sizeof(LiteralHit));
        ac_memset(m.counters.p, 0, sizeof(unsigned long long), &m.stream);
        if (WH == 1) ac_launch("literal_scan", &m.stream, LiteralScanBody<1>{m.packed.as<uint64_t>(), m.seqs.as<SeqInfo>(), n, p, total_bytes, m.needles.as<NeedleSlot>(), cap - 1,
                                                                           m.hits.as<LiteralHit>(), hit_cap, m.counters.as<unsigned long long>()}, (total_bytes + 63) / 64);
        else ac_launch("literal_scan", &m.stream, LiteralScanBody<2>{m.packed.as<uint64_t>(), m.seqs.as<SeqInfo>(), n, p, total_bytes, m.needles.as<NeedleSlot>(), cap - 1,
                                                                     m.hits.as<LiteralHit>(), hit_cap, m.counters.as<unsigned long long>()}, (total_bytes + 63) / 64);
        unsigned long long found = 0;
        ac_d2h(&found, m.counters.p, sizeof found, &m.stream); ac_sync(&m.stream);
        if (found <= hit_cap) { out.resize(found); if (found) { ac_d2h(out.data(), m.hits.p, found * sizeof(LiteralHit), &m.stream); ac_sync(&m.stream); } break; }
        hit_cap = found + 1024;
    }
    m.stage = 0;
}

#define AC_N_COUNTERS 4
template <int W> void DevicePipeline::Impl::local_w(uint32_t seq_lo, uint32_t seq_hi, bool multi) {
    const KParams p = make_kparams(k, W);
    if (seq_lo > seq_hi || seq_hi > n_seqs) throw std::runtime_error("bad sequence shard");
    const SeqInfo* hs = host_seqs.data();
    if (seq_lo == seq_hi) { g_begin = g_end = 0; }
    else { g_begin = hs[seq_lo].start; g_end = hs[seq_hi - 1].start + hs[seq_hi - 1].len; }
    is_multi = multi; own_seq_lo = seq_lo; own_seq_hi = seq_hi; exp_valid = false;
    poison();
    n_windows = total - (uint64_t)n_seqs * (k - 1);
    cap = (n_windows + n_windows / 2 + 64 + 3) & ~3ull;
    if (cap >= 0xFFFFFFF0ull) throw std::runtime_error("input too large for 32-bit slot indices");

    mark(2);
    const uint64_t n_words = (total + 31) / 32;
    packed.ensure((n_words + W + 2) * sizeof(uint64_t));
    ac_memset(packed.as<uint64_t>() + n_words, 0, (W + 2) * sizeof(uint64_t), &stream);
    interior8.ensure(n_words + 8);
    ac_launch("pack", &stream, PackBody{ascii.as<uint8_t>(), total, packed.as<uint64_t>(), seqs.as<SeqInfo>(), n_seqs, interior8.as<uint8_t>()}, n_words);
    mark(3);

    const uint64_t safe_cap = cap;
    counters.ensure(AC_N_COUNTERS * sizeof(unsigned long long));
    unsigned long long hc[AC_N_COUNTERS] = {0, 0, 0, 0};
    big_counts = getenv("AC_BIG_COUNTS") != nullptr;
    const double load = getenv("AC_TABLE_LOAD") ? atof(getenv("AC_TABLE_LOAD")) : 0.5;
    if (load > 0 && n_windows > (1u << 16) && k >= 7) {
        const uint64_t sample_cap = (n_windows / 64 * 4 + 4096) & ~3ull;
        slots.ensure(sample_cap * sizeof(Slot));
        ac_memset(slots.p, 0xFF, sample_cap * sizeof(Slot), &stream);
        ac_memset(counters.p, 0, sizeof hc, &stream);
        const TableView sv{slots.as<Slot>(), sample_cap, packed.as<uint64_t>(), seqs.as<SeqInfo>(), n_seqs, nullptr, slot_gpos_bits(total), AC_SLOT_COUNT_ALARM};
        const InsertBody<W> sample_ins{sv, p, interior8.as<uint8_t>(), 0, 0, (uint32_t)total, false, nullptr, counters.as<unsigned long long>(), true, nullptr};
        ac_launch("sample", &stream, SampleBody<W>{sample_ins, (uint32_t)total}, ((total + 31) / 32 + 31) / 32 * 32);
        ac_d2h(hc, counters.p, sizeof hc, &stream); ac_sync(&stream);
        if (!hc[2]) {
            const uint64_t est = (hc[0] + 3 * (uint64_t)std::sqrt((double)hc[0]) + 16) * 64 + (uint64_t)n_seqs * 2 * k;
            cap = std::min<uint64_t>(safe_cap, ((uint64_t)((double)est / load) + 4096 + 3) & ~3ull);
        }
    }
    mark(15);
    this->safe_cap = safe_cap;
    table_attempt = 0;
    merged.clear();
    insert_w<W>();
    mark(4);
    stage = 1;
}

template <int W> void DevicePipeline::Impl::insert_w() {
    const KParams p = make_kparams(k, W);
    const uint64_t n_words = (total + 31) / 32;
    unsigned long long hc[AC_N_COUNTERS] = {0, 0, 0, 0};
    pos_slot.ensure(total * sizeof(uint32_t));
    for (;; ++table_attempt) {
        if (table_attempt > 3) throw std::runtime_error("k-mer table build did not settle");
        if (getenv("AC_HOST_PROFILE")) fprintf(stderr, "[device] k-mer table attempt %d: capacity %llu, side counts %d\n", table_attempt, (unsigned long long)cap, (int)big_counts);
        poison_table();
        slots.ensure(cap * sizeof(Slot));
        ac_memset(slots.p, 0xFF, cap * sizeof(Slot), &stream);
        if (big_counts) { count_big.ensure(cap * 4); ac_memset(count_big.p, 0, cap * 4, &stream); }
        ac_memset(counters.p, 0, sizeof hc, &stream);
        const TableView tv = table_view();
        const uint64_t g_first = g_begin & ~63ull;
        claimed.ensure((n_words + 8) * 4); ac_memset(claimed.p, 0, (n_words + 8) * 4, &stream);
        const InsertBody<W> ins{tv, p, interior8.as<uint8_t>(), (uint32_t)g_first, (uint32_t)g_begin, (uint32_t)g_end, is_multi, pos_slot.as<uint32_t>(), counters.as<unsigned long long>(), false, claimed.as<uint32_t>()};
        mark(20);
        ac_launch_occ<AC_INSERT_CTAS>("insert", &stream, ins, (g_end - g_first + 63) / 64 * 32);
        mark(21);
        ac_d2h(hc, counters.p, sizeof hc, &stream); ac_sync(&stream);
        if (hc[2] && cap != safe_cap) { cap = safe_cap; continue; }
        if (hc[2]) throw std::runtime_error("k-mer table overflow");
        if (hc[3] && !big_counts) { big_counts = true; continue; }
        break;
    }
    ++table_attempt;
    n_dotted = hc[1];
}

template <int W> uint64_t DevicePipeline::Impl::list_claimed(bool with_filter) {
    const uint64_t n_words = (total + 31) / 32;
    claimed_cnt.ensure((n_words + 1) * 4);
    ac_launch("claimed_count", &stream, ClaimedCountBody{claimed.as<uint32_t>(), n_words, claimed_cnt.as<uint32_t>()}, n_words + 1);
    const uint64_t n = exclusive_scan(claimed_cnt.as<uint32_t>(), claimed_cnt.as<uint32_t>(), n_words + 1);
    occ_list.ensure((n + 1) * 4);
    if (with_filter) {
        static const uint64_t words_env = getenv("AC_EXT_FILTER_WORDS") ? strtoull(getenv("AC_EXT_FILTER_WORDS"), nullptr, 10) : 0;
        n_fwords = words_env ? words_env : n / 2 + 64;
        ext_filter.ensure(n_fwords * 8);
        ac_memset(ext_filter.p, 0, n_fwords * 8, &stream);
    }
    ac_launch("claimed_list", &stream, ClaimedListBody<W>{claimed.as<uint32_t>(), claimed_cnt.as<uint32_t>(), pos_slot.as<uint32_t>(), occ_list.as<uint32_t>(),
                                                          table_view(), make_kparams(k, W), interior8.as<uint8_t>(), with_filter ? ext_filter.as<uint64_t>() : nullptr, n_fwords}, n_words * 32);
    return n;
}
template <int W> uint64_t DevicePipeline::Impl::do_count_entries() {
    if (stage < 1) throw std::runtime_error("build_local must precede the entry export");
    exp_n = list_claimed<W>(false);
    exp_valid = true;
    return exp_n;
}
void DevicePipeline::Impl::do_export_entries(void* dst, uint64_t cap_records) {
    if (cap_records < exp_n) throw std::runtime_error("entry buffer too small");
    ac_launch("export_scatter", &stream, ExportScatterBody{table_view(), occ_list.as<uint32_t>(), (SlotRec*)dst}, exp_n);
    ac_sync(&stream);
}

template <int W> void DevicePipeline::Impl::merge_w(const void* dev_ptr, uint64_t n) {
    if (stage < 1) throw std::runtime_error("build_local must precede merge_entries");
    const KParams p = make_kparams(k, W);
    ac_launch("merge", &stream, MergeBody<W>{table_view(), p, (const SlotRec*)dev_ptr, pos_slot.as<uint32_t>(), counters.as<unsigned long long>(), claimed.as<uint32_t>()}, n);
    merged.emplace_back(dev_ptr, n);
}

template <int W> void DevicePipeline::Impl::runs_local_w() {
    if (stage < 1) throw std::runtime_error("build_local must precede runs_local");
    const KParams p = make_kparams(k, W);
    mark(13);
    if (is_multi) {
        unsigned long long hc[AC_N_COUNTERS];
        ac_d2h(hc, counters.p, sizeof hc, &stream); ac_sync(&stream);
        if (hc[2] && cap != safe_cap) {
            cap = safe_cap;
            insert_w<W>();
            const TableView tv = table_view();
            for (const auto& e : merged)
                ac_launch("merge", &stream, MergeBody<W>{tv, p, (const SlotRec*)e.first, pos_slot.as<uint32_t>(), counters.as<unsigned long long>(), claimed.as<uint32_t>()}, e.second);
            ac_d2h(hc, counters.p, sizeof hc, &stream); ac_sync(&stream);
        }
        if (hc[2]) throw std::runtime_error("k-mer table overflow while merging");
        if (hc[3] && !big_counts) throw std::runtime_error("a k-mer occurs more than 524287 times across the ranks: not supported by the multi-GPU exchange");
        n_dotted = hc[1];
    }
    any_dotted = n_dotted != 0;
    const TableView tv = table_view();

    flags8.ensure(cap);
    n_slots_used = list_claimed<W>(true);
    const AdjacencyBody<W> adj{tv, p, any_dotted, occ_list.as<uint32_t>(), flags8.as<uint8_t>(), ext_filter.as<uint64_t>(), n_fwords};
    if (is_multi && exp_valid && exp_n + 64 < n_slots_used) {
        const uint64_t n_cw = (total + 31) / 32, n_adj = exp_n + 64;
        if (getenv("AC_HOST_PROFILE")) fprintf(stderr, "[device] adjacency flags for this rank's own k-mers: at most %llu of %llu\n", (unsigned long long)n_adj, (unsigned long long)n_slots_used);
        ac_launch("adjacency", &stream, AdjacencyOwnBody<W>{adj, claimed_cnt.as<uint32_t>(), g_begin >> 5, std::min<uint64_t>((g_end + 31) >> 5, n_cw)}, n_adj);
    } else ac_launch("adjacency", &stream, adj, n_slots_used);
    mark(5);

    const uint64_t n_bwords = (total + 31) / 32;
    bmask.ensure(n_bwords * sizeof(uint32_t)); bcount.ensure(n_bwords * sizeof(uint32_t)); boff.ensure(n_bwords * sizeof(uint32_t));
    ac_launch("boundaries", &stream, BoundaryBody{packed.as<uint64_t>(), seqs.as<SeqInfo>(), n_seqs, p.h, g_begin, g_end, pos_slot.as<uint32_t>(),
                                                  flags8.as<uint8_t>(), interior8.as<uint8_t>(), bmask.as<uint32_t>(), bcount.as<uint32_t>()}, n_bwords * 32);
    n_runs = exclusive_scan(bcount.as<uint32_t>(), boff.as<uint32_t>(), n_bwords);
    mark(6);
    run_start.ensure(n_runs * sizeof(uint64_t)); run_len.ensure(n_runs * 4); run_hs.ensure(n_runs * 4); run_ts.ensure(n_runs * 4);
    ac_launch("run_scatter", &stream, RunScatterBody{bmask.as<uint32_t>(), boff.as<uint32_t>(), run_start.as<uint64_t>()}, n_bwords);
    ac_launch("run_ends", &stream, RunEndsLocalBody{seqs.as<SeqInfo>(), n_seqs, run_start.as<uint64_t>(), n_runs, pos_slot.as<uint32_t>(),
                                                    run_len.as<uint32_t>(), run_hs.as<uint32_t>(), run_ts.as<uint32_t>()}, n_runs);
    n_own_runs = n_runs;
    stage = 2;
}

void DevicePipeline::Impl::do_export_runs(void* dst, uint64_t cap_records) {
    if (stage < 2) throw std::runtime_error("runs_local must precede export_runs");
    if (cap_records < n_runs) throw std::runtime_error("run buffer too small");
    ac_launch("run_export", &stream, RunExportBody{run_start.as<uint64_t>(), run_len.as<uint32_t>(), run_hs.as<uint32_t>(), run_ts.as<uint32_t>(),
                                                   slots.as<Slot>(), slot_gpos_bits(total), (RunRec*)dst}, n_runs);
    ac_sync(&stream);
}

void DevicePipeline::Impl::do_import_runs(const void* dev_ptr, uint64_t n) {
    if (stage < 2) throw std::runtime_error("runs_local must precede import_runs");
    n_runs = n;
    run_start.ensure(n_runs * sizeof(uint64_t)); run_len.ensure(n_runs * 4); run_hs.ensure(n_runs * 4); run_ts.ensure(n_runs * 4);
    RunImportBody body{(const RunRec*)dev_ptr, pos_slot.as<uint32_t>(), run_start.as<uint64_t>(), run_len.as<uint32_t>(), run_hs.as<uint32_t>(), run_ts.as<uint32_t>(), 0, {0}, {nullptr}};
    ac_launch("run_import", &stream, body, n_runs);
}

void DevicePipeline::Impl::do_import_runs_from(const void* const* ptrs, const uint64_t* counts, uint32_t n_ranks) {
    if (stage < 2) throw std::runtime_error("runs_local must precede import_runs");
    if (n_ranks == 0 || n_ranks > AC_MAX_RANKS) throw std::runtime_error("import_runs: bad rank count");
    RunImportBody body{nullptr, pos_slot.as<uint32_t>(), nullptr, nullptr, nullptr, nullptr, n_ranks, {0}, {nullptr}};
    for (uint32_t q = 0; q < n_ranks; ++q) { body.first[q + 1] = body.first[q] + counts[q]; body.src[q] = (const RunRec*)ptrs[q]; }
    n_runs = body.first[n_ranks];
    run_start.ensure(n_runs * sizeof(uint64_t)); run_len.ensure(n_runs * 4); run_hs.ensure(n_runs * 4); run_ts.ensure(n_runs * 4);
    body.run_start = run_start.as<uint64_t>(); body.run_len = run_len.as<uint32_t>(); body.run_hs = run_hs.as<uint32_t>(); body.run_ts = run_ts.as<uint32_t>();
    ac_launch("run_import", &stream, body, n_runs);
}

template <int W> void DevicePipeline::Impl::finish_w(PipelineResult& out, bool keep_positions, bool fused, bool split_paths) {
    if (stage < 2) throw std::runtime_error("runs_local must precede finish");
    const KParams p = make_kparams(k, W);
    const TableView tv = table_view();
    out = PipelineResult();
    out.W = W; out.capacity = cap; out.n_slots_used = n_slots_used; out.n_dotted = n_dotted;
    const uint64_t n_runs = this->n_runs;
    const bool any_dotted = this->any_dotted;
    const uint64_t n_windows = this->n_windows;
    mark(14);
    run_uk.ensure(n_runs * 4); run_dir.ensure(n_runs);
    is_rep.ensure(n_runs * 4); rep_idx.ensure(n_runs * 4); run_unitig.ensure(n_runs * 4);
    uid_rep.ensure(cap * 4); slot_unitig.ensure(cap * 4);
    ac_memset(uid_rep.p, 0xFF, cap * 4, &stream);
    ac_launch("run_key", &stream, RunKeyBody{packed.as<uint64_t>(), p.h, run_start.as<uint64_t>(), run_hs.as<uint32_t>(), run_ts.as<uint32_t>(),
                                             run_uk.as<uint32_t>(), run_dir.as<uint8_t>(), uid_rep.as<uint32_t>()}, n_runs);
    ac_launch("rep_flag", &stream, RepFlagBody{run_uk.as<uint32_t>(), uid_rep.as<uint32_t>(), is_rep.as<uint32_t>()}, n_runs);
    const uint32_t n_unitigs = exclusive_scan(is_rep.as<uint32_t>(), rep_idx.as<uint32_t>(), n_runs);
    unitigs.ensure((size_t)n_unitigs * sizeof(DeviceUnitig));
    ac_launch("run_assign", &stream, RunAssignBody{run_start.as<uint64_t>(), run_len.as<uint32_t>(), run_uk.as<uint32_t>(), run_dir.as<uint8_t>(),
                                                   uid_rep.as<uint32_t>(), rep_idx.as<uint32_t>(), run_hs.as<uint32_t>(), run_ts.as<uint32_t>(), tv,
                                                   run_unitig.as<uint32_t>(), unitigs.as<DeviceUnitig>(), slot_unitig.as<uint32_t>()}, n_runs);
    mark(7);

    nchunks.ensure(((size_t)n_unitigs + 1) * 4); chunk_off.ensure(((size_t)n_unitigs + 1) * 4);
    ac_launch("chunk_count", &stream, ChunkCountBody{unitigs.as<DeviceUnitig>(), nchunks.as<uint32_t>()}, n_unitigs);
    ac_memset(nchunks.as<uint32_t>() + n_unitigs, 0, 4, &stream);
    const uint32_t n_chunks = exclusive_scan(nchunks.as<uint32_t>(), chunk_off.as<uint32_t>(), (uint64_t)n_unitigs + 1);
    partial.ensure((size_t)n_chunks * sizeof(MinPartial<W>));
    ac_launch("chunk_min", &stream, ChunkMinBody<W>{packed.as<uint64_t>(), seqs.as<SeqInfo>(), n_seqs, p, unitigs.as<DeviceUnitig>(), n_unitigs,
                                                    chunk_off.as<uint32_t>(), partial.as<MinPartial<W>>()}, n_chunks);
    ac_launch("unitig_min", &stream, UnitigMinBody<W>{chunk_off.as<uint32_t>(), partial.as<MinPartial<W>>(), unitigs.as<DeviceUnitig>()}, n_unitigs);
    mark(8);

    link_count.ensure((size_t)n_unitigs * 2 * 4); links.ensure((size_t)n_unitigs * 2 * AC_MAX_LINKS * 4);
    ac_launch("links", &stream, LinkBody<W>{tv, p, any_dotted, unitigs.as<DeviceUnitig>(), pos_slot.as<uint32_t>(), slot_unitig.as<uint32_t>(),
                                            link_count.as<uint32_t>(), links.as<uint32_t>()}, (uint64_t)n_unitigs * 2);
    mark(9);

    const uint32_t U = n_unitigs;
    sort_a.ensure((size_t)U * 4); sort_b.ensure((size_t)U * 4); sort_ra.ensure((size_t)U * sizeof(SortRec)); sort_rb.ensure((size_t)U * sizeof(SortRec));
    const SeedLess seed_less{unitigs.as<DeviceUnitig>(), W};
    const uint32_t* perm = sort_indices(&stream, seed_less, U, sort_a.as<uint32_t>(), sort_b.as<uint32_t>(), sort_ra.as<SortRec>(), sort_rb.as<SortRec>());
    mark(10);

    rank.ensure((size_t)U * 4); d_len.ensure((size_t)U * 4); d_depth.ensure((size_t)U * 4); need.ensure(((size_t)U + 1) * 4);
    d_seq_off.ensure((size_t)U * 8); d_min_fpos.ensure((size_t)U * 4); d_min_rpos.ensure((size_t)U * 4);
    ac_launch("seed_gather", &stream, SeedGatherBody{perm, unitigs.as<DeviceUnitig>(), U, rank.as<uint32_t>(), d_len.as<uint32_t>(), d_depth.as<uint32_t>(),
                                                     need.as<uint32_t>(), d_min_fpos.as<uint32_t>(), d_min_rpos.as<uint32_t>()}, (uint64_t)U + 1);
    {
        if (n_windows + (uint64_t)U * 2 * AC_SEQ_SLACK >= 0xFFFFFFF0ull) throw std::runtime_error("unitig sequence arena would exceed 4 GB");
    }
    const uint64_t arena_bytes = exclusive_scan(need.as<uint32_t>(), need.as<uint32_t>(), (uint64_t)U + 1);
    ac_launch("seq_off", &stream, SeqOffBody{need.as<uint32_t>(), d_seq_off.as<uint64_t>()}, U);
    d_arena.ensure(arena_bytes);
    ac_launch("emit_seq", &stream, EmitSeqBody{packed.as<uint64_t>(), p.h, unitigs.as<DeviceUnitig>(), U, chunk_off.as<uint32_t>(), rank.as<uint32_t>(),
                                               d_seq_off.as<uint64_t>(), d_arena.as<char>()}, n_chunks);
    const uint32_t n_strands = 2 * U;
    strand_cnt.ensure(((size_t)n_strands + 1) * 4); d_next_off.ensure(((size_t)n_strands + 1) * 4);
    prev_cnt.ensure(((size_t)n_strands + 1) * 4); d_prev_off.ensure(((size_t)n_strands + 1) * 4);
    ac_launch("link_count", &stream, LinkCountBody{link_count.as<uint32_t>(), rank.as<uint32_t>(), unitigs.as<DeviceUnitig>(), n_strands, strand_cnt.as<uint32_t>()},
              (uint64_t)n_strands + 1);
    const uint64_t n_links = exclusive_scan(strand_cnt.as<uint32_t>(), d_next_off.as<uint32_t>(), (uint64_t)n_strands + 1);
    d_next.ensure(n_links * 4); d_prev.ensure(n_links * 4);
    ac_memset(prev_cnt.p, 0, ((size_t)n_strands + 1) * 4, &stream);
    d_small.ensure(64); ac_memset(d_small.p, 0, 64, &stream);
    ac_launch("link_order", &stream, LinkOrderBody{link_count.as<uint32_t>(), links.as<uint32_t>(), rank.as<uint32_t>(), unitigs.as<DeviceUnitig>(),
                                                   d_next_off.as<uint32_t>(), d_next.as<UStrand>(), prev_cnt.as<uint32_t>(), d_small.as<uint32_t>()}, n_strands);
    exclusive_scan(prev_cnt.as<uint32_t>(), d_prev_off.as<uint32_t>(), (uint64_t)n_strands + 1, 0, false);
    ac_memset(prev_cnt.p, 0, ((size_t)n_strands + 1) * 4, &stream);
    ac_launch("prev_fill", &stream, PrevFillBody{d_next_off.as<uint32_t>(), d_next.as<UStrand>(), d_prev_off.as<uint32_t>(), prev_cnt.as<uint32_t>(), d_prev.as<UStrand>()}, n_strands);
    ac_launch("prev_sort", &stream, PrevSortBody{d_prev_off.as<uint32_t>(), d_prev.as<UStrand>()}, n_strands);
    d_path.ensure(n_runs * 4); d_path_off.ensure(((size_t)n_seqs + 1) * 8);
    ac_launch("path", &stream, PathBody{seqs.as<SeqInfo>(), n_seqs, run_start.as<uint64_t>(), run_len.as<uint32_t>(), run_unitig.as<uint32_t>(), rank.as<uint32_t>(),
                                        unitigs.as<DeviceUnitig>(), d_path.as<UStrand>(), d_min_fpos.as<uint32_t>(), d_min_rpos.as<uint32_t>()}, n_runs);
    d_rec.ensure((size_t)U * sizeof(UnitigRec));
    ac_launch("pack_rec", &stream, PackRecBody{d_seq_off.as<uint64_t>(), d_len.as<uint32_t>(), d_min_fpos.as<uint32_t>(), d_min_rpos.as<uint32_t>(), d_rec.as<UnitigRec>()}, U);
    ac_launch("path_off", &stream, PathOffBody{seqs.as<SeqInfo>(), n_seqs, run_start.as<uint64_t>(), n_runs, d_path_off.as<uint64_t>()}, (uint64_t)n_seqs + 1);
    num_prefix.ensure((size_t)U * 8);
    ac_launch("number_key", &stream, NumberKeyBody{d_rec.as<UnitigRec>(), d_arena.as<char>(), num_prefix.as<uint64_t>()}, U);
    const NumberLess number_less{d_rec.as<UnitigRec>(), d_depth.as<uint32_t>(), d_arena.as<char>(), num_prefix.as<uint64_t>(), nullptr};
    uint32_t* ord_in = sort_indices(&stream, number_less, U, sort_a.as<uint32_t>(), sort_b.as<uint32_t>(), sort_ra.as<SortRec>(), sort_rb.as<SortRec>());
    d_fixed.ensure((size_t)U * 4); ac_memset(d_fixed.p, 0, (size_t)U * 4, &stream);
    uint8_t* seed_start = d_fixed.as<uint8_t>(); uint8_t* seed_end = seed_start + U; uint8_t* fix_start = seed_end + U; uint8_t* fix_end = fix_start + U;
    ac_launch("fixed_seed", &stream, FixedSeedBody{d_path_off.as<uint64_t>(), d_path.as<UStrand>(), seed_start, seed_end}, n_seqs);
    ac_copy_dd(fix_start, seed_start, (size_t)U * 2, &stream);
    ac_launch("fixed_spread", &stream, FixedSpreadBody{seed_start, seed_end, d_next_off.as<uint32_t>(), d_next.as<UStrand>(), d_prev_off.as<uint32_t>(), d_prev.as<UStrand>(),
                                                       fix_start, fix_end}, U);
    const CandidateView cview{ord_in, d_next_off.as<uint32_t>(), d_next.as<UStrand>(), d_prev_off.as<uint32_t>(), d_prev.as<UStrand>(), fix_start, fix_end};
    cand_flag.ensure((2 * (size_t)U + 1) * 4); cand_index.ensure((2 * (size_t)U + 1) * 4);
    ac_launch("candidate_flag", &stream, CandidateFlagBody{cview, U, cand_flag.as<uint32_t>()}, 2ull * U + 1);
    const uint64_t n_cands = exclusive_scan(cand_flag.as<uint32_t>(), cand_index.as<uint32_t>(), 2ull * U + 1);
    d_cands.ensure((n_cands + 1) * sizeof(ExpandCandidate)); d_cand_at.ensure(2 * (size_t)U * 4 + 4); d_deps.ensure((size_t)U * sizeof(ExpandDeps) + 4); d_spec.ensure((n_cands + 1) * 4);
    ac_launch("candidate_fill", &stream, CandidateFillBody{cview, cand_flag.as<uint32_t>(), cand_index.as<uint32_t>(), d_cands.as<ExpandCandidate>(), d_cand_at.as<int32_t>()}, 2ull * U);
    ac_launch("dependents", &stream, DependentsBody{d_next_off.as<uint32_t>(), d_next.as<UStrand>(), d_prev_off.as<uint32_t>(), d_prev.as<UStrand>(), d_cand_at.as<int32_t>(),
                                                    d_deps.as<ExpandDeps>()}, U);
    ac_launch("common_length", &stream, CommonLengthBody{d_cands.as<ExpandCandidate>(), d_rec.as<UnitigRec>(), d_arena.as<char>(), d_spec.as<uint32_t>()}, n_cands);
    R = Pending();
    R.U = U; R.n_links = n_links; R.n_cands = n_cands; R.n_strands = n_strands; R.order_built = ord_in; R.fix_start = fix_start;
    R.arena_final = arena_bytes; R.arena_src = &d_arena;
    mark(11);
    if (fused && n_cands > 0) {
        d_pred.ensure(n_cands * 7 * 4); d_level.ensure(n_cands * 4); d_flagmax.ensure(32); d_counters64.ensure((AC_PASS_WORDS + 8) * 8);
        d_dirty.ensure(((n_cands + 63) / 64) * 8 + 8); d_exhausted.ensure(n_cands + 8);
        unsigned long long* c64 = d_counters64.as<unsigned long long>();
        unsigned long long* res = c64 + AC_PASS_WORDS;
        ac_launch("level_pred", &stream, LevelPredBody{d_cands.as<ExpandCandidate>(), d_deps.as<ExpandDeps>(), d_pred.as<int32_t>()}, n_cands);
        ac_memset(d_level.p, 0, n_cands * 4, &stream); ac_memset(d_flagmax.p, 0, 32, &stream);
        ac_launch_coop("levels", &stream, LevelsCoopBody{d_pred.as<int32_t>(), d_level.as<uint32_t>(), d_flagmax.as<uint32_t>(), n_cands}, n_cands, 4096);
        ac_memset(d_counters64.p, 0, (AC_PASS_WORDS + 8) * 8, &stream);
        const RelocBoundBody bound_body{d_cands.as<ExpandCandidate>(), d_rec.as<UnitigRec>(), d_cand_at.as<int32_t>(), c64 + AC_PASS_SET(1) + 1};
        ac_launch("reloc_bound", &stream, bound_body, n_cands);
        uint32_t fm[8]; unsigned long long h64[AC_PASS_WORDS + 8];
        ac_d2h(fm, d_flagmax.p, 32, &stream); ac_d2h(h64, c64, sizeof h64, &stream); ac_sync(&stream);
        if (fm[4]) throw std::runtime_error("candidate levels did not settle");
        unsigned long long bound = 0; for (int x = 0; x < AC_BOUND_STRIPES; ++x) bound += h64[AC_PASS_SET(1) + 1 + x];
        if (arena_bytes + bound >= 0xFFFFFFF0ull) throw std::runtime_error("unitig sequence arena would exceed 4 GB");
        d_arena2.ensure(arena_bytes + 2 * bound + 64);
        ac_copy_dd(d_arena2.p, d_arena.p, arena_bytes, &stream);
        const unsigned long long start = arena_bytes;
        ac_h2d(c64, &start, 8, &stream);
        ac_memset(c64 + AC_PASS_SET(1), 0, AC_PASS_SET_WORDS * 8, &stream);
        ac_memset(d_dirty.p, 0, ((n_cands + 63) / 64) * 8 + 8, &stream); ac_memset(d_exhausted.p, 0, n_cands + 8, &stream);
        static const bool always_grow = getenv("AC_DEVICE_TIGHT_ARENA") != nullptr;
        uint32_t next_set = 0, next_due = 0; uint64_t passes = 0;
        const uint32_t due_stride = fm[3] + 2;
        d_due.ensure((size_t)3 * due_stride * 4); ac_memset(d_due.p, 0, (size_t)3 * due_stride * 4, &stream);
        for (bool first = true;; first = false) {
            const ApplyLevelBody apply{d_cands.as<ExpandCandidate>(), d_deps.as<ExpandDeps>(), d_level.as<uint32_t>(), 0, d_spec.as<uint32_t>(),
                                       d_rec.as<UnitigRec>(), d_arena2.as<char>(), c64, c64, d_dirty.as<uint64_t>(), d_exhausted.as<uint8_t>(), first, c64 + AC_PASS_REMOVED};
            const uint64_t room = always_grow ? 0 : d_arena2.cap;
            ac_launch_coop("simplify", &stream, SimplifyCoopBody{apply, bound_body, n_cands, d_flagmax.as<uint32_t>() + 3, c64, res, room, next_set, first,
                                                                 d_due.as<uint32_t>(), due_stride, next_due}, n_cands, 64);
            ac_d2h(h64, c64, sizeof h64, &stream); ac_sync(&stream);
            const unsigned long long* r = h64 + AC_PASS_WORDS;
            R.arena_final = h64[0]; R.bases_removed = h64[AC_PASS_REMOVED]; R.any_moved = r[1] != 0;
            passes += r[2]; next_set = (uint32_t)r[5]; next_due = (uint32_t)r[7];
            if (getenv("AC_HOST_PROFILE")) fprintf(stderr, "[device] expand_repeats launch: %llu passes (%llu so far), %u levels, %llu candidates, %llu left on the work list, last pass moved %llu bases\n",
                                                   r[2], (unsigned long long)passes, fm[3], (unsigned long long)n_cands, r[4], r[0]);
            if (r[0] == 0) break;
            if (passes > 1000000) throw std::runtime_error("repeat expansion did not settle");
            bound = r[3];
            if (R.arena_final + bound >= 0xFFFFFFF0ull) throw std::runtime_error("unitig sequence arena would exceed 4 GB");
            d_arena3.ensure(std::max<size_t>((R.arena_final + bound) * 2 + 64, d_arena3.cap + (always_grow ? 64 : 0)));
            ac_copy_dd(d_arena3.p, d_arena2.p, R.arena_final, &stream); ac_sync(&stream);
            std::swap(d_arena2.p, d_arena3.p); std::swap(d_arena2.cap, d_arena3.cap);
        }
        R.arena_src = &d_arena2;
    }
    mark(17);
    if (fused) {
        if (R.any_moved) {
            d_pos.ensure((size_t)U * 4); sort_c.ensure((size_t)U * 4); sort_d.ensure((size_t)U * 4);
            ac_launch("inverse_perm", &stream, InversePermBody{ord_in, d_pos.as<uint32_t>()}, U);
            ac_launch("number_key", &stream, NumberKeyBody{d_rec.as<UnitigRec>(), R.arena_src->as<char>(), num_prefix.as<uint64_t>()}, U);
            const NumberLess final_less{d_rec.as<UnitigRec>(), d_depth.as<uint32_t>(), R.arena_src->as<char>(), num_prefix.as<uint64_t>(), d_pos.as<uint32_t>()};
            R.final_order = sort_indices(&stream, final_less, U, sort_c.as<uint32_t>(), sort_d.as<uint32_t>(), sort_ra.as<SortRec>(), sort_rb.as<SortRec>());
        } else R.final_order = ord_in;
        if (U < 100000000u) {
            uint32_t* fin = R.final_order;
            d_pos2.ensure((size_t)U * 4);
            ac_launch("inverse_perm", &stream, InversePermBody{fin, d_pos2.as<uint32_t>()}, U);
            const GfaView gv{fin, d_pos2.as<uint32_t>(), d_rec.as<UnitigRec>(), R.arena_src->as<char>(), d_depth.as<uint32_t>(), d_next_off.as<uint32_t>(), d_next.as<UStrand>()};
            gfa_s_size.ensure(((size_t)U + 1) * 4); gfa_l_size.ensure(((size_t)U + 1) * 4); gfa_pieces.ensure(((size_t)U + 1) * 4);
            const uint64_t steps = split_paths ? 0 : n_runs;
            d_last.ensure(steps + 8); gfa_p_size.ensure((steps + 1) * 4);
            ac_launch("gfa_size", &stream, GfaSizeBody{gv, U, gfa_s_size.as<uint32_t>(), gfa_l_size.as<uint32_t>()}, (uint64_t)U + 1);
            ac_launch("gfa_chunk_count", &stream, GfaChunkCountBody{gv, U, gfa_pieces.as<uint32_t>()}, (uint64_t)U + 1);
            d_totals.ensure(64); ac_memset(d_totals.p, 0, 64, &stream);
            if (!split_paths) {
                ac_memset(d_last.p, 0, steps + 8, &stream);
                ac_launch("path_last", &stream, PathLastBody{d_path_off.as<uint64_t>(), d_last.as<uint8_t>()}, n_seqs);
                ac_launch("path_size", &stream, PathSizeBody{d_path.as<UStrand>(), d_pos2.as<uint32_t>(), d_last.as<uint8_t>(), steps, gfa_p_size.as<uint32_t>()}, steps + 1);
                scan_keep_total(gfa_p_size.as<uint32_t>(), steps + 1, d_totals.as<uint32_t>() + 3);
            }
            scan_keep_total(gfa_s_size.as<uint32_t>(), (uint64_t)U + 1, d_totals.as<uint32_t>() + 0);
            scan_keep_total(gfa_l_size.as<uint32_t>(), (uint64_t)U + 1, d_totals.as<uint32_t>() + 1);
            scan_keep_total(gfa_pieces.as<uint32_t>(), (uint64_t)U + 1, d_totals.as<uint32_t>() + 2);
            uint32_t tot[4];
            ac_d2h(tot, d_totals.p, 16, &stream); ac_sync(&stream);
            const uint64_t s_bytes = tot[0], l_bytes = tot[1], n_pieces = tot[2], p_list_bytes = tot[3];
            char head[64]; const uint64_t head_bytes = (uint64_t)snprintf(head, sizeof head, "H\tVN:Z:1.0\tKM:i:%u\n", k);
            if (path_wrap_total == 0 && n_seqs) throw std::runtime_error("set_path_line_texts() must precede a build that renders the GFA");
            const uint64_t p_bytes = split_paths ? 0 : p_list_bytes + path_wrap_total;
            R.gfa_bytes = head_bytes + s_bytes + l_bytes + p_bytes;
            d_text.ensure(R.gfa_bytes + 64);
            char* text = d_text.as<char>();
            ac_h2d(text, head, head_bytes, &stream);
            ac_launch("gfa_segment", &stream, GfaSegmentBody{gv, gfa_s_size.as<uint32_t>(), text + head_bytes}, U);
            ac_launch("gfa_sequence", &stream, GfaSequenceBody{gv, U, gfa_pieces.as<uint32_t>(), gfa_s_size.as<uint32_t>(), text + head_bytes}, n_pieces);
            ac_launch("gfa_link", &stream, GfaLinkBody{gv, gfa_l_size.as<uint32_t>(), text + head_bytes + s_bytes}, U);
            const PathLineView pv{d_path_off.as<uint64_t>(), n_seqs, gfa_p_size.as<uint32_t>(), d_wrap_off.as<uint64_t>(), d_pre_len.as<uint32_t>(), d_suf_len.as<uint32_t>(),
                                  d_blob.as<char>(), d_blob_off.as<uint64_t>(), 0};
            char* p_text = text + head_bytes + s_bytes + l_bytes;
            if (!split_paths) {
                ac_launch("path_text", &stream, PathTextFullBody{d_path.as<UStrand>(), d_pos2.as<uint32_t>(), d_last.as<uint8_t>(), pv, p_text}, steps);
                ac_launch("path_wrap", &stream, PathWrapBody{pv, p_text}, 2ull * n_seqs);
            }
            R.paths_split = split_paths;
            R.gfa_on_device = true;
        }
    }
    mark(18);
    R.hairpins_ready = true;

    if (before_results && *before_results) (*before_results)();
    out.fused = fused; out.graph_fetched = false;
    if (fused && !R.gfa_on_device) throw std::runtime_error("fused build: the device GFA writer did not run");
    uint64_t d2h = 0;
    if (R.gfa_on_device) {
        h_text.ensure(R.gfa_bytes + 64);
        ac_d2h(h_text.p, d_text.p, R.gfa_bytes, &stream); d2h += R.gfa_bytes;
    }
    uint32_t small[16];
    ac_d2h(small, d_small.p, 64, &stream); ac_sync(&stream); d2h += 64;
    out.links_single = (n_links - small[0]) / 2 + small[0];
    out.length_before = n_slots_used;
    out.length_after = n_slots_used - R.bases_removed;
    out.gfa_text = R.gfa_on_device ? h_text.as<char>() : nullptr; out.gfa_bytes = R.gfa_on_device ? R.gfa_bytes : 0;
    out.n_unitigs = U; out.n_runs = n_runs; out.n_seqs = n_seqs; out.n_links = n_links;
    out.h2d_bytes = uploaded_bytes + (uint64_t)n_seqs * sizeof(SeqInfo);
    out.d2h_bytes = d2h;
    pending_keep_positions = keep_positions;
    if (!fused) pull_graph(out, keep_positions);
    else { mark(16); mark(12); arena_pending = true; }
}

void DevicePipeline::Impl::pull_graph(PipelineResult& out, bool keep_positions) {
    const uint32_t U = R.U; const uint64_t n_links = R.n_links, n_cands = R.n_cands; const uint32_t n_strands = R.n_strands;
    const uint64_t arena_cap = R.arena_final + R.arena_final / 4 + (1u << 20);
    h_rec.ensure((size_t)U * sizeof(UnitigRec)); h_depth.ensure((size_t)U * 4);
    h_arena.ensure(arena_cap); h_next_off.ensure(((size_t)n_strands + 1) * 4); h_prev_off.ensure(((size_t)n_strands + 1) * 4);
    h_next.ensure(n_links * 4 + 4); h_prev.ensure(n_links * 4 + 4); h_path.ensure(n_runs * 4 + 4); h_path_off.ensure(((size_t)n_seqs + 1) * 8);
    uint64_t d2h = 0;
    auto pull = [&](PinBuf& dst, DevBuf& src, size_t bytes) { if (bytes) ac_d2h(dst.p, src.p, bytes, &stream); d2h += bytes; };
    pull(h_rec, d_rec, (size_t)U * sizeof(UnitigRec)); pull(h_depth, d_depth, (size_t)U * 4);
    const bool plain = !out.fused;
    if (plain) { h_order.ensure((size_t)U * 4 + 4); if (U) { ac_d2h(h_order.p, R.order_built, (size_t)U * 4, &stream); d2h += (size_t)U * 4; } }
    pull(h_next_off, d_next_off, ((size_t)n_strands + 1) * 4); pull(h_prev_off, d_prev_off, ((size_t)n_strands + 1) * 4);
    pull(h_next, d_next, n_links * 4); pull(h_prev, d_prev, n_links * 4); pull(h_path, d_path, n_runs * 4); pull(h_path_off, d_path_off, ((size_t)n_seqs + 1) * 8);
    if (keep_positions) {
        h_run_start.ensure(n_runs * 8 + 8); h_run_len.ensure(n_runs * 4 + 4);
        pull(h_run_start, run_start, n_runs * 8); pull(h_run_len, run_len, n_runs * 4);
    }
    if (plain) {
        h_cands.ensure((n_cands + 1) * sizeof(ExpandCandidate)); h_deps.ensure((size_t)U * sizeof(ExpandDeps) + 4); h_spec.ensure((n_cands + 1) * 4); h_fixed.ensure((size_t)U * 2 + 4);
        pull(h_cands, d_cands, n_cands * sizeof(ExpandCandidate)); pull(h_deps, d_deps, (size_t)U * sizeof(ExpandDeps)); pull(h_spec, d_spec, n_cands * 4);
        if (U) { ac_d2h(h_fixed.p, R.fix_start, (size_t)U * 2, &stream); d2h += (size_t)U * 2; }
    } else { h_order2.ensure((size_t)U * 4 + 4); if (U) { ac_d2h(h_order2.p, R.final_order, (size_t)U * 4, &stream); d2h += (size_t)U * 4; } }
    mark(16);
    pull(h_arena, *R.arena_src, R.arena_final);
    out.d2h_bytes += d2h;
    mark(12);
    wait_mark(16);
    out.graph_fetched = true;
    out.rec = h_rec.as<UnitigRec>(); out.depth = h_depth.as<uint32_t>();
    out.order = plain ? h_order.as<uint32_t>() : nullptr; out.final_order = plain ? nullptr : h_order2.as<uint32_t>();
    out.n_cands = plain ? n_cands : 0; out.cands = plain ? h_cands.as<ExpandCandidate>() : nullptr; out.deps = plain ? h_deps.as<ExpandDeps>() : nullptr;
    out.spec_len = plain ? h_spec.as<uint32_t>() : nullptr;
    out.fixed_start = plain ? h_fixed.as<uint8_t>() : nullptr; out.fixed_end = plain ? h_fixed.as<uint8_t>() + U : nullptr;
    out.arena = h_arena.as<char>(); out.arena_used = R.arena_final; out.arena_cap = arena_cap;
    out.next_off = h_next_off.as<uint32_t>(); out.next = h_next.as<UStrand>(); out.prev_off = h_prev_off.as<uint32_t>(); out.prev = h_prev.as<UStrand>();
    out.path_off = h_path_off.as<uint64_t>(); out.path = h_path.as<UStrand>();
    out.run_start = keep_positions ? h_run_start.as<uint64_t>() : nullptr; out.run_len = keep_positions ? h_run_len.as<uint32_t>() : nullptr;
    arena_pending = true;
}

void DevicePipeline::Impl::do_complete(PipelineResult& out) {
    if (!arena_pending) return;
    ac_sync(&stream);
    arena_pending = false;
    out.t.h2d = between(0, 1); out.t.pack = between(2, 3); out.t.insert = between(15, 4); out.t.insert_kernel = between(20, 21); out.t.sample = between(3, 15); out.t.adjacency = between(13, 5);
    out.t.boundaries = between(5, 6); out.t.runs = between(14, 7); out.t.unitigs = between(7, 8); out.t.links = between(8, 9);
    out.t.seed_sort = between(9, 10); out.t.emit = between(10, 11); out.t.simplify = between(11, 17); out.t.gfa = between(17, 18);
    out.t.d2h = between(18, 12); out.t.total = between(2, 4) + between(13, 6) + between(14, 12);
}

void DevicePipeline::Impl::do_export_path_tokens(void* dst, uint64_t stride, const uint64_t* counts, uint32_t n_ranks) {
    if (stage < 2 || !R.gfa_on_device || !R.paths_split) throw std::runtime_error("export_path_tokens follows a finish with split path lines");
    if (n_ranks == 0 || n_ranks > AC_MAX_RANKS) throw std::runtime_error("export_path_tokens: bad rank count");
    PathTokenBody body{d_path.as<UStrand>(), d_pos2.as<uint32_t>(), (uint32_t*)dst, stride, n_ranks, {0}};
    for (uint32_t q = 0; q < n_ranks; ++q) { if (counts[q] > stride) throw std::runtime_error("export_path_tokens: a rank holds more occurrences than the stride"); body.first[q + 1] = body.first[q] + counts[q]; }
    if (body.first[n_ranks] != n_runs) throw std::runtime_error("export_path_tokens: the counts do not add up to the occurrences imported");
    ac_launch("path_tokens", &stream, body, n_runs);
}
void DevicePipeline::Impl::do_render_path_lines(const void* tokens, uint64_t n_tokens, const char** text, uint64_t* bytes) {
    if (stage < 2) throw std::runtime_error("runs_local must precede render_path_lines");
    if (n_tokens != n_own_runs) throw std::runtime_error("render_path_lines: one token per occurrence of this rank's sequences is expected");
    if (path_pre.size() != n_seqs) throw std::runtime_error("set_path_line_texts() must precede render_path_lines");
    const uint32_t n_own = own_seq_hi - own_seq_lo;
    uint64_t wrap_lo = 0, wrap_hi = 0;
    for (uint32_t i = 0; i < own_seq_hi; ++i) { if (i == own_seq_lo) wrap_lo = wrap_hi; wrap_hi += (uint64_t)path_pre[i] + path_suf[i]; }
    if (own_seq_lo == own_seq_hi) wrap_lo = wrap_hi;
    mark(19);
    uint64_t total_bytes = 0;
    if (n_own) {
        const uint64_t steps = n_tokens;
        d_own_off.ensure(((size_t)n_own + 1) * 8); d_own_last.ensure(steps + 8); d_own_size.ensure((steps + 1) * 4);
        ac_launch("path_off", &stream, PathOffBody{seqs.as<SeqInfo>() + own_seq_lo, n_own, run_start.as<uint64_t>(), steps, d_own_off.as<uint64_t>()}, (uint64_t)n_own + 1);
        ac_memset(d_own_last.p, 0, steps + 8, &stream);
        ac_launch("path_last", &stream, PathLastBody{d_own_off.as<uint64_t>(), d_own_last.as<uint8_t>()}, n_own);
        ac_launch("path_size", &stream, PathSizeBody{(const UStrand*)tokens, nullptr, d_own_last.as<uint8_t>(), steps, d_own_size.as<uint32_t>()}, steps + 1);
        const uint64_t list_bytes = exclusive_scan(d_own_size.as<uint32_t>(), d_own_size.as<uint32_t>(), steps + 1);
        total_bytes = list_bytes + (wrap_hi - wrap_lo);
        d_ptext.ensure(total_bytes + 64);
        const PathLineView pv{d_own_off.as<uint64_t>(), n_own, d_own_size.as<uint32_t>(), d_wrap_off.as<uint64_t>() + own_seq_lo, d_pre_len.as<uint32_t>() + own_seq_lo,
                              d_suf_len.as<uint32_t>() + own_seq_lo, d_blob.as<char>(), d_blob_off.as<uint64_t>() + own_seq_lo, wrap_lo};
        ac_launch("path_text", &stream, PathTextFullBody{(const UStrand*)tokens, nullptr, d_own_last.as<uint8_t>(), pv, d_ptext.as<char>()}, steps);
        ac_launch("path_wrap", &stream, PathWrapBody{pv, d_ptext.as<char>()}, 2ull * n_own);
        h_ptext.ensure(total_bytes + 64);
        ac_d2h(h_ptext.p, d_ptext.p, total_bytes, &stream);
    }
    ac_sync(&stream);
    path_lines_d2h = total_bytes;
    *text = total_bytes ? h_ptext.as<char>() : nullptr; *bytes = total_bytes;
}

#define AC_W_CASE(fn, n, ...) case n: fn<n>(__VA_ARGS__); break;
#define AC_DISPATCH_W(fn, ...) switch (W) { AC_W_CASE(fn, 1, __VA_ARGS__) AC_W_CASE(fn, 2, __VA_ARGS__) AC_W_CASE(fn, 3, __VA_ARGS__) AC_W_CASE(fn, 4, __VA_ARGS__) \
    AC_W_CASE(fn, 5, __VA_ARGS__) AC_W_CASE(fn, 6, __VA_ARGS__) AC_W_CASE(fn, 7, __VA_ARGS__) AC_W_CASE(fn, 8, __VA_ARGS__) AC_W_CASE(fn, 9, __VA_ARGS__) AC_W_CASE(fn, 10, __VA_ARGS__) \
    AC_W_CASE(fn, 11, __VA_ARGS__) AC_W_CASE(fn, 12, __VA_ARGS__) AC_W_CASE(fn, 13, __VA_ARGS__) AC_W_CASE(fn, 14, __VA_ARGS__) AC_W_CASE(fn, 15, __VA_ARGS__) AC_W_CASE(fn, 16, __VA_ARGS__) \
    default: throw std::runtime_error("upload() must precede build()"); }

void DevicePipeline::build_local(uint32_t seq_lo, uint32_t seq_hi, bool multi) {
    Impl& m = *impl; m.set_device(); const int W = m.W;
    AC_DISPATCH_W(m.local_w, seq_lo, seq_hi, multi)
}
uint64_t DevicePipeline::count_entries() {
    Impl& m = *impl; m.set_device(); const int W = m.W;
    uint64_t count = 0;
    AC_DISPATCH_W(count = m.do_count_entries)
// ... 84 lines not shown
```

autocycler_b200/csrc/pipeline.h:

```cpp
#pragma once
#include <cstdint>
#include <functional>
#include <string>
#include <vector>

#include "kmer_key.h"

#define AC_MAX_W 16
#define AC_MAX_K (32 * AC_MAX_W - 1)
#define AC_MAX_LINKS 5
#define AC_SEQ_SLACK 32

struct PipelineTimings {
    float h2d = 0, pack = 0, sample = 0, insert = 0, insert_kernel = 0, adjacency = 0, boundaries = 0, runs = 0, unitigs = 0, links = 0, seed_sort = 0, emit = 0, simplify = 0, gfa = 0, d2h = 0, total = 0;
};

struct DeviceUnitig {
    uint64_t start;
    uint32_t len;
    uint32_t depth;
    uint32_t flip;
    int32_t min_d;
    uint64_t min_w[AC_MAX_W];
    uint32_t head_slot, tail_slot;
// ... 16 lines not shown

struct PipelineResult {
    uint32_t W = 0;
    uint64_t n_slots_used = 0;
    uint64_t capacity = 0;
    uint64_t n_dotted = 0;
    uint64_t h2d_bytes = 0, d2h_bytes = 0;
    uint32_t n_unitigs = 0;
    uint64_t n_runs = 0;
    uint32_t n_seqs = 0;
    UnitigRec* rec = nullptr;
    uint32_t* depth = nullptr;
    uint32_t* order = nullptr;
    uint64_t n_cands = 0;
    ExpandCandidate* cands = nullptr;
    uint32_t* spec_len = nullptr;
    ExpandDeps* deps = nullptr;
    uint8_t* fixed_start = nullptr; uint8_t* fixed_end = nullptr;
    uint32_t* final_order = nullptr;
    char* gfa_text = nullptr; uint64_t gfa_bytes = 0;
    bool fused = false, graph_fetched = true;
    uint64_t links_single = 0;
    uint64_t length_before = 0, length_after = 0;
    char* arena = nullptr; uint64_t arena_used = 0, arena_cap = 0;
    uint32_t* next_off = nullptr;
    UStrand* next = nullptr;
    uint32_t* prev_off = nullptr;
    UStrand* prev = nullptr;
    uint64_t n_links = 0;
    uint64_t* path_off = nullptr;
    UStrand* path = nullptr;
    uint64_t* run_start = nullptr;
    uint32_t* run_len = nullptr;
    PipelineTimings t;
};

struct LiteralHit { uint32_t needle; uint32_t pad; uint64_t gpos; };

struct OverlapJob { uint64_t a_off, b_off; uint32_t n, k, skip_diagonal, pad; };
struct AlignPiece { int32_t a_unitig, a_index, b_unitig, b_index; };
struct BridgeJob { uint64_t a_off, b_off; uint32_t n, m; };
struct BridgeRun { uint32_t shared_jobs = 0, hbm_jobs = 0; };
struct UpgmaMerge { uint32_t node, left, right, pad; double dist; };

class DevicePipeline {
public:
    DevicePipeline(int device, void* stream);
    ~DevicePipeline();
    void upload(const uint8_t* ascii, uint64_t total, const SeqInfo* seqs, uint32_t n_seqs, uint32_t k, uint32_t seq_lo = 0, uint32_t seq_hi = 0xFFFFFFFFu);
    void* strand_block(uint32_t seq_lo, uint32_t seq_hi, uint64_t* n_bytes);
    void set_path_line_texts(const char* blob, const uint32_t* prefix_len, const uint32_t* suffix_len, uint32_t n_seqs);
    void complete(PipelineResult& out);
    std::function<void()> before_results;
    void build(PipelineResult& out, bool keep_positions, bool fused = false);
    void fetch_graph(PipelineResult& out, bool keep_positions);
    void build_local(uint32_t seq_lo, uint32_t seq_hi, bool multi);
    uint64_t count_entries();
    void export_entries(void* dst, uint64_t cap_records);
    void merge_entries(const void* dev_ptr, uint64_t n);
    void runs_local();
    uint64_t local_runs() const;
    void export_runs(void* dst, uint64_t cap_records);
    void import_runs(const void* dev_ptr, uint64_t n);
    void import_runs_padded(const void* dev_ptr, uint64_t stride, const uint64_t* counts, uint32_t n_ranks);
    static void enable_peer_access(const int* devices, int n);
    const void* export_entries_own(uint64_t* n);
    const void* export_runs_own(uint64_t* n);
    void import_runs_from(const void* const* ptrs, const uint64_t* counts, uint32_t n_ranks);
    void finish(PipelineResult& out, bool keep_positions, bool fused = false, bool split_paths = false);
    void export_path_tokens(void* dst, uint64_t stride, const uint64_t* counts, uint32_t n_ranks);
    void render_path_lines(const void* tokens_dev, uint64_t n_tokens, const char** text, uint64_t* bytes);
    void pair_shared_lengths(const UStrand* path, const uint64_t* path_off, uint32_t n_seqs, const uint32_t* unitig_len, uint32_t n_unitigs, uint64_t* shared);
    float cluster_distances(const UStrand* path, const uint64_t* path_off, uint32_t n_seqs, const uint32_t* unitig_len, uint32_t n_unitigs, double* asym);
    float upgma(const double* sym, uint32_t n, const uint32_t* ids, UpgmaMerge* merges);
    float overlap_align(const int32_t* values, uint64_t n_values, const uint32_t* weights, uint64_t n_weights,
                        const OverlapJob* jobs, uint32_t n_jobs, std::vector<std::vector<AlignPiece>>& out);
    uint32_t overlap_shared_k_max();
    float bridge_distances(const int32_t* values, uint64_t n_values, const uint32_t* weights, uint64_t n_weights,
                           const BridgeJob* jobs, uint32_t n_jobs, uint32_t* dist, BridgeRun* run);
    uint32_t bridge_shared_n_max();
    void find_literals(const uint8_t* ascii, uint64_t total, const SeqInfo* seqs, uint32_t n_seqs, uint32_t h,
                       const uint64_t* needle_words, uint32_t n_needles, std::vector<LiteralHit>& hits);
    unsigned long long kernel_launches() const;
    struct Impl;
private:
    Impl* impl;
};
```

include/autocycler_gpu.h:

```cpp
#ifndef AUTOCYCLER_GPU_H
#define AUTOCYCLER_GPU_H

#include <stdint.h>

#ifdef __cplusplus
extern "C" {
#endif

#define AC_OK 0
#define AC_EINVAL (-1)
#define AC_ENODEVICE (-2)
#define AC_ECUDA (-3)
#define AC_ERANGE (-4)
#define AC_EIO (-5)
#define AC_EINPUT (-6)

typedef struct ac_handle ac_handle;

typedef struct {
    uint32_t k;
    int32_t device;
    void* stream;
    uint32_t keep_positions;
    int32_t n_devices;
    const int32_t* devices;
} ac_config;

typedef struct {
    uint64_t n_kmers;
    uint64_t n_unitigs;
    uint64_t n_links;
    uint64_t total_length;
    uint64_t seq_bytes;
    uint64_t n_fwd_pos, n_rev_pos;
    uint64_t n_next;
    uint64_t n_sequences;
    uint64_t n_path_steps;
    uint64_t length_before_simplify;
} ac_counts;

typedef struct {
    uint32_t* number;
    uint64_t* seq_off;
    uint8_t* seq;
    double* depth;
    uint64_t* fpos_off;
    uint32_t* fpos;
    uint16_t* fpos_id_strand;
    uint64_t* rpos_off; uint32_t* rpos; uint16_t* rpos_id_strand;
    uint64_t* next_off;
    int32_t* next;
} ac_unitigs;

typedef struct {
    float h2d, pack, insert, adjacency, boundaries, runs, unitigs, links, seed_sort, emit, d2h, device_total;
    float host_graph, host_simplify, host_gfa;
    float sample, device_simplify, device_gfa;
    float insert_kernel;
    float trim_kernel;
    uint64_t insert_occurrences;
    uint64_t table_capacity, table_used;
    uint64_t kernel_launches;
    uint64_t h2d_bytes, d2h_bytes;
} ac_timings;

const char* ac_last_error(const ac_handle* h);
const char* ac_version(void);

int ac_create(ac_handle** out, const ac_config* cfg);
void ac_destroy(ac_handle* h);

int ac_add_sequence(ac_handle* h, uint16_t seq_id, const uint8_t* fwd_padded, uint64_t padded_len,
                    const char* filename, const char* contig_header);
int ac_clear_sequences(ac_handle* h);
int ac_upload(ac_handle* h);
int ac_upload_shard(ac_handle* h, uint32_t seq_lo, uint32_t seq_hi);
int ac_strand_block(ac_handle* h, uint32_t seq_lo, uint32_t seq_hi, void** dev_ptr, uint64_t* n_bytes);
int ac_build(ac_handle* h);
int ac_simplify(ac_handle* h);
int ac_compress(ac_handle* h);
int ac_merge_linear_paths(ac_handle* h, int use_paths);
int ac_renumber_unitigs(ac_handle* h);

int ac_build_local(ac_handle* h, uint32_t seq_lo, uint32_t seq_hi, uint32_t multi);
int ac_entries_count(ac_handle* h, uint64_t* n);
int ac_entries_export(ac_handle* h, void* dst, uint64_t cap_records);
int ac_entries_merge(ac_handle* h, const void* src, uint64_t n);
int ac_runs_local(ac_handle* h, uint64_t* n_runs);
int ac_runs_export(ac_handle* h, void* dst, uint64_t cap_records);
int ac_runs_import(ac_handle* h, const void* src, uint64_t n);
int ac_runs_import_padded(ac_handle* h, const void* src, uint64_t stride_records, const uint64_t* counts, uint32_t n_ranks);
int ac_build_finish(ac_handle* h);
int ac_compress_finish(ac_handle* h);
int ac_compress_finish_split(ac_handle* h);
int ac_path_tokens_export(ac_handle* h, void* dst, uint64_t stride_tokens, const uint64_t* counts, uint32_t n_ranks);
int ac_path_lines_render(ac_handle* h, const void* tokens, uint64_t n_tokens);
int ac_path_lines_data(ac_handle* h, const char** data, uint64_t* n_bytes);
int ac_counts_get(const ac_handle* h, ac_counts* out);
int ac_unitigs_copy(const ac_handle* h, ac_unitigs* out);
int ac_path_copy(const ac_handle* h, uint64_t seq_index, int32_t* out, uint64_t cap, uint64_t* n);
int ac_gfa_size(ac_handle* h, uint64_t* n_bytes);
int ac_gfa_copy(ac_handle* h, char* buf, uint64_t cap);
int ac_gfa_data(ac_handle* h, const char** data, uint64_t* n_bytes);
int ac_timings_get(const ac_handle* h, ac_timings* out);

int ac_compress_dir(const char* assemblies_dir, const char* autocycler_dir, uint32_t k, uint32_t max_contigs,
                    uint32_t threads, int32_t device, int32_t verbose);
int ac_compress_dir_devices(const char* assemblies_dir, const char* autocycler_dir, uint32_t k, uint32_t max_contigs,
                            uint32_t threads, const int32_t* devices, int32_t n_devices, int32_t verbose);

int ac_load_sequences(ac_handle* h, const char* assemblies_dir, uint32_t max_contigs, uint32_t threads,
                      uint64_t* assembly_count);
int ac_sequence_get(const ac_handle* h, uint64_t index, uint16_t* seq_id, uint64_t* length,
                    char* fwd_padded, uint64_t cap_fwd, char* filename, uint64_t cap_fn, char* header, uint64_t cap_hd);

int ac_load_gfa(ac_handle* h, const char* gfa_text, uint64_t length);

int ac_bind_host_to_device(int32_t device);

int ac_pairwise_distances(ac_handle* h, double* out, uint64_t cap);
int ac_distance_matrix_text(ac_handle* h, char* out, uint64_t cap, uint64_t* length);

int ac_decompress_gfa(const char* in_gfa, const char* out_dir, const char* out_file, int32_t device, int32_t verbose);

int ac_sequence_reconstruct(const ac_handle* h, uint64_t index, char* out, uint64_t cap, uint64_t* length);

#define AC_TRIM_START_END 0
#define AC_TRIM_HAIRPIN_START 1
#define AC_TRIM_HAIRPIN_END 2
int ac_trim_paths(ac_handle* h, int32_t mode, const int32_t* paths, const uint64_t* path_off, uint64_t n_paths,
                  const uint32_t* weights, uint64_t n_weights, double min_identity, uint32_t max_unitigs,
                  int32_t* out, uint64_t* out_off, uint8_t* trimmed);
int ac_trim(ac_handle* h, double min_identity, uint32_t max_unitigs, double mad);
int ac_trim_yaml(ac_handle* h, char* out, uint64_t cap, uint64_t* length);
int ac_trim_stats(const ac_handle* h, uint64_t* jobs, uint64_t* cells, uint32_t* max_window, uint64_t* max_path);
int ac_trim_dir(const char* cluster_dir, double min_identity, uint32_t max_unitigs, double mad, uint32_t threads, int32_t device, int32_t verbose);

#define AC_CLUSTER_PHYLIP 0
#define AC_CLUSTER_NEWICK 1
#define AC_CLUSTER_TSV 2
#define AC_CLUSTER_YAML 3
#define AC_CLUSTER_GFA 4
#define AC_CLUSTER_UNTRIMMED_YAML 5
int ac_cluster(ac_handle* h, double cutoff, int64_t min_assemblies, const uint16_t* manual, uint64_t n_manual);
int ac_cluster_text(ac_handle* h, int32_t what, uint32_t cluster, char* out, uint64_t cap, uint64_t* length);
int ac_cluster_assignments(const ac_handle* h, uint16_t* cluster, uint8_t* pass, uint64_t cap);
// ... 30 lines not shown
```

Measured before the change: 5323.

## Drive kernel sizes from device-side counts to remove host round-trip syncs

Adds launch helpers (ac_launch_n, count-aware scan and tile sort) that read element counts from a device metadata buffer inside the kernel instead of copying them to the host first. Many stream synchronisations and small D2H reads in compress/simplify are dropped or deferred, so the host can keep queuing work while the GPU runs. In exchange, grids are sized by an upper bound and can spawn idle threads, and correctness now depends on the bound checks. It also adds a host_waits counter and a profiling script for idle gaps.

```diff
diff --git a/autocycler_b200/api.py b/autocycler_b200/api.py
--- a/autocycler_b200/api.py
+++ b/autocycler_b200/api.py
@@ -35,7 +35,7 @@
 class AcTimings(C.Structure):
     _fields_ = [(n, C.c_float) for n in ("h2d", "pack", "insert", "adjacency", "boundaries", "runs", "unitigs", "links", "seed_sort", "emit", "d2h",
                                         "device_total", "host_graph", "host_simplify", "host_gfa", "sample", "device_simplify", "device_gfa", "insert_kernel", "trim_kernel")] + \
-               [(n, C.c_uint64) for n in ("insert_occurrences", "table_capacity", "table_used", "kernel_launches", "h2d_bytes", "d2h_bytes")]
+               [(n, C.c_uint64) for n in ("insert_occurrences", "table_capacity", "table_used", "kernel_launches", "h2d_bytes", "d2h_bytes", "host_waits")]
 
     def as_dict(self):
         return {n: getattr(self, n) for n, _ in self._fields_}
diff --git a/autocycler_b200/csrc/backend.h b/autocycler_b200/csrc/backend.h
--- a/autocycler_b200/csrc/backend.h
+++ b/autocycler_b200/csrc/backend.h
@@ -7,9 +7,15 @@
 #include <stdexcept>
 #include <string>
 
+#include <type_traits>
+
+struct AcDevCount { const uint32_t* p = nullptr; uint32_t mul = 1, add = 0; };
+#define AC_COUNT_FIELD(name, member) struct name { template <class B> AC_HD static void set(B& b, uint64_t v) { b.member = (decltype(b.member))v; } };
+
 #ifdef AC_EMULATE
 #define AC_HD inline
 #define AC_D inline
+struct AcNoField { template <class B> AC_HD static void set(B&, uint64_t) {} };
 
 template <class T> inline T ac_atomic_cas(T* p, T cmp, T val) { T old = *p; if (old == cmp) *p = val; return old; }
 template <class T> inline T ac_atomic_add(T* p, T v) { T old = *p; *p = (T)(old + v); return old; }
@@ -25,7 +31,7 @@
 inline uint32_t ac_popc(uint32_t v) { return (uint32_t)__builtin_popcount(v); }
 inline int ac_ctz(uint32_t v) { return __builtin_ctz(v); }
 
-struct AcStream { int dummy; };
+struct AcStream { int dummy; unsigned long long waits = 0; };
 
 inline void* ac_dev_alloc(size_t bytes) { void* p = malloc(bytes ? bytes : 1); if (!p) throw std::runtime_error("emu alloc failed"); return p; }
 inline void ac_dev_free(void* p) { free(p); }
@@ -33,14 +39,22 @@
 inline void ac_h2d(void* d, const void* h, size_t bytes, AcStream*) { memcpy(d, h, bytes); }
 inline void ac_d2h(void* h, const void* d, size_t bytes, AcStream*) { memcpy(h, d, bytes); }
 inline void ac_copy_dd(void* dst, const void* src, size_t bytes, AcStream*) { memcpy(dst, src, bytes); }
-inline void ac_sync(AcStream*) {}
+inline void ac_sync(AcStream* st) { ++st->waits; }
 inline void* ac_host_alloc(size_t bytes) { return malloc(bytes ? bytes : 1); }
 inline void ac_host_free(void* p) { free(p); }
 
 template <class Body> inline void ac_launch(const char*, AcStream*, const Body& body, uint64_t n);
+inline uint64_t ac_count_value(const AcDevCount& c) { return c.p ? (uint64_t)*c.p * c.mul + c.add : 0; }
 template <int CTAS, class Body> inline void ac_launch_occ(const char* name, AcStream* st, const Body& body, uint64_t n) { ac_launch(name, st, body, n); }
 template <class Body> inline void ac_launch(const char*, AcStream*, const Body& body, uint64_t n) {
     for (uint64_t i = 0; i < n; ++i) body(i);
+}
+template <class Set = AcNoField, class Body> inline void ac_launch_n(const char* name, AcStream* st, const Body& body, AcDevCount c, uint64_t bound, AcDevCount field = AcDevCount{}) {
+    const uint64_t n = ac_count_value(c);
+    if (n > bound) throw std::runtime_error(std::string("launch ") + name + ": count " + std::to_string(n) + " above its bound " + std::to_string(bound));
+    Body b = body;
+    Set::set(b, ac_count_value(field));
+    ac_launch(name, st, b, n);
 }
 struct AcGridSync { void operator()() const {} };
 template <class Body> inline void ac_launch_coop(const char*, AcStream*, const Body& body, uint64_t, uint64_t = 256) { AcGridSync sync; body(0, 1, sync); }
@@ -55,6 +69,7 @@
 #define AC_HD inline
 #define AC_D inline
 #endif
+struct AcNoField { template <class B> AC_HD static void set(B&, uint64_t) {} };
 
 #define AC_CUDA_CHECK(expr) do { cudaError_t _e = (expr); if (_e != cudaSuccess) \
     throw std::runtime_error(std::string(#expr) + ": " + cudaGetErrorString(_e)); } while (0)
@@ -85,7 +100,7 @@
 AC_D uint64_t ac_atomic_and(uint64_t* p, uint64_t v) { return (uint64_t)atomicAnd((unsigned long long*)p, (unsigned long long)v); }
 #endif
 
-struct AcStream { cudaStream_t s; };
+struct AcStream { cudaStream_t s; unsigned long long waits = 0; };
 
 inline void* ac_dev_alloc(size_t bytes) { void* p = nullptr; AC_CUDA_CHECK(cudaMalloc(&p, bytes ? bytes : 1)); return p; }
 inline void ac_dev_free(void* p) { if (p) cudaFree(p); }
@@ -93,7 +108,7 @@
 inline void ac_h2d(void* d, const void* h, size_t bytes, AcStream* st) { AC_CUDA_CHECK(cudaMemcpyAsync(d, h, bytes, cudaMemcpyHostToDevice, st->s)); }
 inline void ac_d2h(void* h, const void* d, size_t bytes, AcStream* st) { AC_CUDA_CHECK(cudaMemcpyAsync(h, d, bytes, cudaMemcpyDeviceToHost, st->s)); }
 inline void ac_copy_dd(void* dst, const void* src, size_t bytes, AcStream* st) { AC_CUDA_CHECK(cudaMemcpyAsync(dst, src, bytes, cudaMemcpyDeviceToDevice, st->s)); }
-inline void ac_sync(AcStream* st) { AC_CUDA_CHECK(cudaStreamSynchronize(st->s)); }
+inline void ac_sync(AcStream* st) { ++st->waits; AC_CUDA_CHECK(cudaStreamSynchronize(st->s)); }
 inline void ac_debug_sync(const char* name, AcStream* st) {
     static const bool on = getenv("AC_SYNC_LAUNCHES") != nullptr;
     if (!on) return;
@@ -110,6 +125,7 @@
 
 #ifdef __CUDACC__
 #include <cooperative_groups.h>
+AC_HD uint64_t ac_count_value(const AcDevCount& c) { return c.p ? (uint64_t)*c.p * c.mul + c.add : 0; }
 extern unsigned long long g_ac_kernel_launches;
 
 template <class Body> __global__ void __launch_bounds__(256) ac_body_kernel(const Body body, uint64_t n) {
@@ -180,5 +196,29 @@
     ++g_ac_kernel_launches;
     ac_debug_sync(name, st);
 }
-#endif
-#endif
+
+template <class Body, class Set> __global__ void __launch_bounds__(256) ac_body_kernel_n(const Body body0, const AcDevCount c, const AcDevCount field) {
+    const uint64_t n = ac_count_value(c);
+    Body body = body0;
+    Set::set(body, ac_count_value(field));
+    const uint64_t stride = (uint64_t)gridDim.x * blockDim.x;
+    const uint32_t lane = threadIdx.x & 31u;
+    for (uint64_t base = (uint64_t)blockIdx.x * blockDim.x + (threadIdx.x - lane); base < n; base += stride) {
+        const uint64_t i = base + lane;
+        if (i < n) body(i);
+        __syncwarp();
+    }
+}
+template <class Set = AcNoField, class Body> inline void ac_launch_n(const char* name, AcStream* st, const Body& body, AcDevCount c, uint64_t bound, AcDevCount field = AcDevCount{}) {
+    if (bound == 0) return;
+    const int threads = 256;
+    const uint64_t want = (bound + threads - 1) / threads, max_blocks = ac_sm_count() * 16;
+    const unsigned blocks = (unsigned)(want < max_blocks ? want : max_blocks);
+    ac_body_kernel_n<Body, Set><<<blocks, threads, 0, st->s>>>(body, c, field);
+    cudaError_t e = cudaGetLastError();
+    if (e != cudaSuccess) throw std::runtime_error(std::string("launch ") + name + ": " + cudaGetErrorString(e));
+    ++g_ac_kernel_launches;
+    ac_debug_sync(name, st);
+}
+#endif
+#endif
diff --git a/autocycler_b200/csrc/c_api.cpp b/autocycler_b200/csrc/c_api.cpp
--- a/autocycler_b200/csrc/c_api.cpp
+++ b/autocycler_b200/csrc/c_api.cpp
@@ -711,6 +711,7 @@
     if (!h || !out) return set_error(h, AC_EINVAL, "null argument");
     *out = h->t;
     out->kernel_launches = h->pipe->kernel_launches();
+    out->host_waits = h->pipe->host_waits();
     return ok(h);
 }
 
diff --git a/autocycler_b200/csrc/pipeline.cu b/autocycler_b200/csrc/pipeline.cu
--- a/autocycler_b200/csrc/pipeline.cu
+++ b/autocycler_b200/csrc/pipeline.cu
@@ -11,6 +11,7 @@
 #endif
 
 #define AC_NONE32 0xFFFFFFFFu
+AC_COUNT_FIELD(AcSetN, n) AC_COUNT_FIELD(AcSetNUnitigs, n_unitigs) AC_COUNT_FIELD(AcSetNStrands, n_strands)
 #define AC_CHUNK 32
 #define AC_MINCHUNK 128
 #define AC_MAX_RANKS 16
@@ -778,8 +779,9 @@
 #define AC_SORT_TILE 16
 #endif
 #ifndef AC_EMULATE
-template <class Less> __global__ void __launch_bounds__(1024) ac_tile_sort_kernel(const Less less, uint32_t n, uint32_t* __restrict__ idx, SortRec* __restrict__ recs) {
+template <class Less> __global__ void __launch_bounds__(1024) ac_tile_sort_kernel(const Less less, uint32_t n, uint32_t* __restrict__ idx, SortRec* __restrict__ recs, AcDevCount dn) {
     extern __shared__ __align__(16) unsigned char tile_smem[];
+    if (dn.p) { n = (uint32_t)ac_count_value(dn); if (blockIdx.x * AC_SORT_TILE >= n) return; }
     SortRec* keys = reinterpret_cast<SortRec*>(tile_smem);
     uint16_t* buf0 = reinterpret_cast<uint16_t*>(tile_smem + AC_SORT_TILE * sizeof(SortRec));
     uint16_t* buf1 = buf0 + AC_SORT_TILE;
@@ -830,22 +832,28 @@
         for (uint32_t x = a; x < b; ++x) { SortRec r = less.load(idx[x]); r.id = idx[x]; r.pad = 0; recs[x] = r; }
     }
 };
-template <class Less> static uint32_t* sort_indices(AcStream* stream, const Less& less, uint32_t n, uint32_t* a, uint32_t* b, SortRec* ra, SortRec* rb) {
+template <class Less> static uint32_t* sort_indices(AcStream* stream, const Less& less, uint32_t n, uint32_t* a, uint32_t* b, SortRec* ra, SortRec* rb, AcDevCount dn = AcDevCount{}) {
     if (n == 0) return a;
     const uint64_t tiles = ((uint64_t)n + AC_SORT_TILE - 1) / AC_SORT_TILE;
 #ifndef AC_EMULATE
     const size_t smem = AC_SORT_TILE * (sizeof(SortRec) + 2 * sizeof(uint16_t));
     AC_CUDA_CHECK(cudaFuncSetAttribute(ac_tile_sort_kernel<Less>, cudaFuncAttributeMaxDynamicSharedMemorySize, (int)smem));
-    ac_tile_sort_kernel<Less><<<(unsigned)tiles, 1024, smem, stream->s>>>(less, n, a, ra); ++g_ac_kernel_launches;
+    ac_tile_sort_kernel<Less><<<(unsigned)tiles, 1024, smem, stream->s>>>(less, n, a, ra, dn); ++g_ac_kernel_launches;
     cudaError_t e = cudaGetLastError();
     if (e != cudaSuccess) throw std::runtime_error(std::string("launch tile sort: ") + cudaGetErrorString(e));
     ac_debug_sync("tile_sort", stream);
 #else
-    ac_launch("tile_sort", stream, TileSortBody<Less>{less, n, a, ra}, tiles);
+    if (dn.p) {
+        const uint64_t m = ac_count_value(dn);
+        if (m > n) throw std::runtime_error("sort: count above its bound");
+        ac_launch("tile_sort", stream, TileSortBody<Less>{less, (uint32_t)m, a, ra}, (m + AC_SORT_TILE - 1) / AC_SORT_TILE);
+    } else ac_launch("tile_sort", stream, TileSortBody<Less>{less, n, a, ra}, tiles);
 #endif
     for (uint64_t width = AC_SORT_TILE; width < n; width *= AC_SORT_WAYS) {
         uint32_t steps = 1; while ((1ull << steps) <= width) ++steps;
-        ac_launch("merge_pass", stream, MergeWaysBody<Less>{less, n, (uint32_t)width, steps, ra, rb, b}, n);
+        const MergeWaysBody<Less> pass{less, n, (uint32_t)width, steps, ra, rb, b};
+        if (dn.p) ac_launch_n<AcSetN>("merge_pass", stream, pass, dn, n, dn);
+        else ac_launch("merge_pass", stream, pass, n);
         std::swap(a, b); std::swap(ra, rb);
     }
     return a;
@@ -1799,7 +1807,8 @@
 }
 #define AC_SCAN_STATE(epoch, status, value) (((unsigned long long)(epoch) << 34) | ((unsigned long long)(status) << 32) | (unsigned long long)(value))
 __global__ void __launch_bounds__(256) ac_scan_chained_kernel(const uint32_t* in, uint64_t n, uint32_t* out, unsigned long long* state, unsigned long long epoch,
-                                                               unsigned long long* ticket, unsigned long long ticket_base, uint32_t n_tiles, uint32_t* total_out) {
+                                                               unsigned long long* ticket, unsigned long long ticket_base, uint32_t n_tiles, uint32_t* total_out, AcDevCount dn) {
+    if (dn.p) n = ac_count_value(dn);
     __shared__ uint32_t warp_tot[8];
     __shared__ uint32_t s_tile, s_prefix;
     const uint32_t lane = threadIdx.x & 31, warp = threadIdx.x >> 5;
@@ -1913,6 +1922,7 @@
 #endif
     }
     void wait_mark(int i) {
+        ++stream.waits;
 #ifndef AC_EMULATE
         AC_CUDA_CHECK(cudaEventSynchronize(ev[i]));
 #else
@@ -1932,7 +1942,7 @@
 
 #ifndef AC_EMULATE
     DevBuf scan_state; unsigned long long scan_epoch = 0, scan_tickets = 0;
-    uint32_t exclusive_scan(const uint32_t* in, uint32_t* out, uint64_t n, int = 0, bool want_total = true) {
+    uint32_t exclusive_scan(const uint32_t* in, uint32_t* out, uint64_t n, int = 0, bool want_total = true, AcDevCount dn = AcDevCount{}, uint32_t* total_dst = nullptr) {
         if (n == 0) return 0;
         const uint64_t nb = (n + AC_SCAN_TILE - 1) / AC_SCAN_TILE;
         if (nb > 0x7FFFFFFFull) throw std::runtime_error("scan too large");
@@ -1943,17 +1953,25 @@
         }
         unsigned long long* st = scan_state.as<unsigned long long>();
         scan_epoch = (scan_epoch + 1) & 0x3FFFFFFFull; if (scan_epoch == 0) scan_epoch = 1;
-        ac_scan_chained_kernel<<<(unsigned)nb, 256, 0, stream.s>>>(in, n, out, st + 2, scan_epoch, st, scan_tickets, (uint32_t)nb, (uint32_t*)(st + 1)); ++g_ac_kernel_launches;
+        ac_scan_chained_kernel<<<(unsigned)nb, 256, 0, stream.s>>>(in, n, out, st + 2, scan_epoch, st, scan_tickets, (uint32_t)nb, total_dst ? total_dst : (uint32_t*)(st + 1), dn); ++g_ac_kernel_launches;
         scan_tickets += nb;
         cudaError_t e = cudaGetLastError();
         if (e != cudaSuccess) throw std::runtime_error(std::string("launch scan: ") + cudaGetErrorString(e));
         ac_debug_sync("scan", &stream);
         uint32_t total_sum = 0;
-        if (want_total) { ac_d2h(&total_sum, st + 1, sizeof(uint32_t), &stream); ac_sync(&stream); }
+        if (want_total && !dn.p) { ac_d2h(&total_sum, st + 1, sizeof(uint32_t), &stream); ac_sync(&stream); }
         return total_sum;
     }
 #else
-    uint32_t exclusive_scan(const uint32_t* in, uint32_t* out, uint64_t n, int level = 0, bool want_total = true) {
+    uint32_t exclusive_scan(const uint32_t* in, uint32_t* out, uint64_t n, int level = 0, bool want_total = true, AcDevCount dn = AcDevCount{}, uint32_t* total_dst = nullptr) {
+        if (dn.p || total_dst) {
+            const uint64_t m = dn.p ? ac_count_value(dn) : n;
+            if (m > n) throw std::runtime_error("scan: count " + std::to_string(m) + " above its bound " + std::to_string(n));
+            uint32_t acc = 0;
+            for (uint64_t i = 0; i < m; ++i) { const uint32_t v = in[i]; out[i] = acc; acc += v; }
+            if (total_dst) *total_dst = acc;
+            return 0;
+        }
         if (n == 0) return 0;
         if (level >= 4) throw std::runtime_error("scan too deep");
         const uint64_t tile = 256;
@@ -1976,6 +1994,11 @@
 
     std::vector<SeqInfo> host_seqs;
     uint64_t cap = 0, n_windows = 0, n_runs = 0, g_begin = 0, g_end = 0, n_slots_used = 0, n_dotted = 0, n_fwords = 0;
+    uint64_t n_est = 0;
+    enum { M_KMERS, M_UNITIGS, M_CHUNKS, M_ARENA, M_LINKS, M_CANDS, M_HAIRPINS, M_WORDS = 16 };
+    DevBuf d_meta; PinBuf h_meta;
+    uint32_t* meta() { return d_meta.as<uint32_t>(); }
+    AcDevCount dcount(int word, uint32_t mul = 1, uint32_t add = 0) { return AcDevCount{meta() + word, mul, add}; }
     bool any_dotted = false, is_multi = false, big_counts = false;
     int stage = 0;
     DevBuf run_hs, run_ts, claimed, claimed_cnt, occ_list, ext_filter, needles, hits, count_big, interior8;
@@ -1995,8 +2018,8 @@
     template <int W> void runs_local_w();
     template <int W> void finish_w(PipelineResult& out, bool keep_positions, bool fused, bool split_paths);
     struct Pending {
-        uint32_t U = 0, n_strands = 0; uint64_t n_links = 0, n_cands = 0;
-        uint32_t* order_built = nullptr; uint32_t* final_order = nullptr; uint8_t* fix_start = nullptr;
+        uint32_t U = 0, U_b = 0, n_strands = 0, hairpins = 0; uint64_t n_links = 0, n_cands = 0;
+        uint32_t* order_built = nullptr; uint32_t* final_order = nullptr; uint8_t* fix_start = nullptr; uint8_t* fix_end = nullptr;
         DevBuf* arena_src = nullptr; uint64_t arena_final = 0;
         bool any_moved = false, gfa_on_device = false, hairpins_ready = false, paths_split = false;
         uint64_t bases_removed = 0, gfa_bytes = 0;
@@ -2014,7 +2037,7 @@
     void do_export_path_tokens(void* dst, uint64_t stride, const uint64_t* counts, uint32_t n_ranks);
     void do_render_path_lines(const void* tokens, uint64_t n_tokens, const char** text, uint64_t* bytes);
     DevBuf d_own_off, d_own_last, d_own_size; uint64_t path_lines_d2h = 0;
-    template <int W> uint64_t list_claimed(bool with_filter);
+    template <int W> uint64_t list_claimed(bool with_filter, bool want_n);
     template <int W> uint64_t do_count_entries();
     void do_export_entries(void* dst, uint64_t cap_records);
     void do_export_runs(void* dst, uint64_t cap_records);
@@ -2084,6 +2107,7 @@
 }
 
 unsigned long long DevicePipeline::kernel_launches() const { return g_ac_kernel_launches; }
+unsigned long long DevicePipeline::host_waits() const { return impl->stream.waits; }
 
 void DevicePipeline::upload(const uint8_t* ascii, uint64_t total, const SeqInfo* seqs, uint32_t n_seqs, uint32_t k, uint32_t seq_lo, uint32_t seq_hi) {
     Impl& m = *impl;
@@ -2496,6 +2520,7 @@
     mark(3);
 
     const uint64_t safe_cap = cap;
+    n_est = n_windows;
     counters.ensure(AC_N_COUNTERS * sizeof(unsigned long long));
     unsigned long long hc[AC_N_COUNTERS] = {0, 0, 0, 0};
     big_counts = getenv("AC_BIG_COUNTS") != nullptr;
@@ -2512,6 +2537,7 @@
         if (!hc[2]) {
             const uint64_t est = (hc[0] + 3 * (uint64_t)std::sqrt((double)hc[0]) + 16) * 64 + (uint64_t)n_seqs * 2 * k;
             cap = std::min<uint64_t>(safe_cap, ((uint64_t)((double)est / load) + 4096 + 3) & ~3ull);
+            n_est = std::min<uint64_t>(est, n_windows);
         }
     }
     mark(15);
@@ -2553,15 +2579,17 @@
     n_dotted = hc[1];
 }
 
-template <int W> uint64_t DevicePipeline::Impl::list_claimed(bool with_filter) {
+template <int W> uint64_t DevicePipeline::Impl::list_claimed(bool with_filter, bool want_n) {
     const uint64_t n_words = (total + 31) / 32;
     claimed_cnt.ensure((n_words + 1) * 4);
     ac_launch("claimed_count", &stream, ClaimedCountBody{claimed.as<uint32_t>(), n_words, claimed_cnt.as<uint32_t>()}, n_words + 1);
-    const uint64_t n = exclusive_scan(claimed_cnt.as<uint32_t>(), claimed_cnt.as<uint32_t>(), n_words + 1);
-    occ_list.ensure((n + 1) * 4);
+    exclusive_scan(claimed_cnt.as<uint32_t>(), claimed_cnt.as<uint32_t>(), n_words + 1, 0, false, AcDevCount{}, meta() + M_KMERS);
+    uint64_t n = 0;
+    if (want_n) { uint32_t v = 0; ac_d2h(&v, meta() + M_KMERS, 4, &stream); ac_sync(&stream); n = v; }
+    occ_list.ensure((cap + 1) * 4);
     if (with_filter) {
         static const uint64_t words_env = getenv("AC_EXT_FILTER_WORDS") ? strtoull(getenv("AC_EXT_FILTER_WORDS"), nullptr, 10) : 0;
-        n_fwords = words_env ? words_env : n / 2 + 64;
+        n_fwords = words_env ? words_env : n_est / 2 + 64;
         ext_filter.ensure(n_fwords * 8);
         ac_memset(ext_filter.p, 0, n_fwords * 8, &stream);
     }
@@ -2571,7 +2599,8 @@
 }
 template <int W> uint64_t DevicePipeline::Impl::do_count_entries() {
     if (stage < 1) throw std::runtime_error("build_local must precede the entry export");
-    exp_n = list_claimed<W>(false);
+    d_meta.ensure(M_WORDS * 4);
+    exp_n = list_claimed<W>(false, true);
     exp_valid = true;
     return exp_n;
 }
@@ -2611,13 +2640,15 @@
     const TableView tv = table_view();
 
     flags8.ensure(cap);
-    n_slots_used = list_claimed<W>(true);
+    d_meta.ensure(M_WORDS * 4);
+    n_slots_used = list_claimed<W>(true, is_multi);
     const AdjacencyBody<W> adj{tv, p, any_dotted, occ_list.as<uint32_t>(), flags8.as<uint8_t>(), ext_filter.as<uint64_t>(), n_fwords};
     if (is_multi && exp_valid && exp_n + 64 < n_slots_used) {
         const uint64_t n_cw = (total + 31) / 32, n_adj = exp_n + 64;
         if (getenv("AC_HOST_PROFILE")) fprintf(stderr, "[device] adjacency flags for this rank's own k-mers: at most %llu of %llu\n", (unsigned long long)n_adj, (unsigned long long)n_slots_used);
         ac_launch("adjacency", &stream, AdjacencyOwnBody<W>{adj, claimed_cnt.as<uint32_t>(), g_begin >> 5, std::min<uint64_t>((g_end + 31) >> 5, n_cw)}, n_adj);
-    } else ac_launch("adjacency", &stream, adj, n_slots_used);
+    } else if (is_multi) ac_launch("adjacency", &stream, adj, n_slots_used);
+    else ac_launch_n("adjacency", &stream, adj, dcount(M_KMERS), cap);
     mark(5);
 
     const uint64_t n_bwords = (total + 31) / 32;
@@ -2671,6 +2702,15 @@
     const bool any_dotted = this->any_dotted;
     const uint64_t n_windows = this->n_windows;
     mark(14);
+    d_meta.ensure(M_WORDS * 4);
+    uint32_t* const M = meta();
+    const uint64_t n_b = std::min<uint64_t>(cap, n_windows);
+    const uint32_t U_b = (uint32_t)std::min<uint64_t>(n_runs, n_b);
+    const uint64_t chunks_b = (uint64_t)U_b + n_b / AC_MINCHUNK, strands_b = 2ull * U_b, cands_b = 2ull * U_b + 1;
+    if (n_b + (uint64_t)U_b * 2 * AC_SEQ_SLACK >= 0xFFFFFFF0ull) throw std::runtime_error("unitig sequence arena would exceed 4 GB");
+    const uint64_t arena_b = n_b + (uint64_t)U_b * 2 * AC_SEQ_SLACK;
+    const AcDevCount cU = dcount(M_UNITIGS), cU1 = dcount(M_UNITIGS, 1, 1), cS = dcount(M_UNITIGS, 2), cS1 = dcount(M_UNITIGS, 2, 1), cC = dcount(M_CANDS);
+    ac_memset(M + M_UNITIGS, 0, (M_WORDS - M_UNITIGS) * 4, &stream);
     run_uk.ensure(n_runs * 4); run_dir.ensure(n_runs);
     is_rep.ensure(n_runs * 4); rep_idx.ensure(n_runs * 4); run_unitig.ensure(n_runs * 4);
     uid_rep.ensure(cap * 4); slot_unitig.ensure(cap * 4);
@@ -2678,105 +2718,113 @@
     ac_launch("run_key", &stream, RunKeyBody{packed.as<uint64_t>(), p.h, run_start.as<uint64_t>(), run_hs.as<uint32_t>(), run_ts.as<uint32_t>(),
                                              run_uk.as<uint32_t>(), run_dir.as<uint8_t>(), uid_rep.as<uint32_t>()}, n_runs);
     ac_launch("rep_flag", &stream, RepFlagBody{run_uk.as<uint32_t>(), uid_rep.as<uint32_t>(), is_rep.as<uint32_t>()}, n_runs);
-    const uint32_t n_unitigs = exclusive_scan(is_rep.as<uint32_t>(), rep_idx.as<uint32_t>(), n_runs);
-    unitigs.ensure((size_t)n_unitigs * sizeof(DeviceUnitig));
+    exclusive_scan(is_rep.as<uint32_t>(), rep_idx.as<uint32_t>(), n_runs, 0, false, AcDevCount{}, M + M_UNITIGS);
+    unitigs.ensure((size_t)U_b * sizeof(DeviceUnitig));
     ac_launch("run_assign", &stream, RunAssignBody{run_start.as<uint64_t>(), run_len.as<uint32_t>(), run_uk.as<uint32_t>(), run_dir.as<uint8_t>(),
                                                    uid_rep.as<uint32_t>(), rep_idx.as<uint32_t>(), run_hs.as<uint32_t>(), run_ts.as<uint32_t>(), tv,
                                                    run_unitig.as<uint32_t>(), unitigs.as<DeviceUnitig>(), slot_unitig.as<uint32_t>()}, n_runs);
     mark(7);
 
-    nchunks.ensure(((size_t)n_unitigs + 1) * 4); chunk_off.ensure(((size_t)n_unitigs + 1) * 4);
-    ac_launch("chunk_count", &stream, ChunkCountBody{unitigs.as<DeviceUnitig>(), nchunks.as<uint32_t>()}, n_unitigs);
-    ac_memset(nchunks.as<uint32_t>() + n_unitigs, 0, 4, &stream);
-    const uint32_t n_chunks = exclusive_scan(nchunks.as<uint32_t>(), chunk_off.as<uint32_t>(), (uint64_t)n_unitigs + 1);
-    partial.ensure((size_t)n_chunks * sizeof(MinPartial<W>));
-    ac_launch("chunk_min", &stream, ChunkMinBody<W>{packed.as<uint64_t>(), seqs.as<SeqInfo>(), n_seqs, p, unitigs.as<DeviceUnitig>(), n_unitigs,
-                                                    chunk_off.as<uint32_t>(), partial.as<MinPartial<W>>()}, n_chunks);
-    ac_launch("unitig_min", &stream, UnitigMinBody<W>{chunk_off.as<uint32_t>(), partial.as<MinPartial<W>>(), unitigs.as<DeviceUnitig>()}, n_unitigs);
+    nchunks.ensure(((size_t)U_b + 1) * 4); chunk_off.ensure(((size_t)U_b + 1) * 4);
+    ac_memset(nchunks.p, 0, ((size_t)U_b + 1) * 4, &stream);
+    ac_launch_n("chunk_count", &stream, ChunkCountBody{unitigs.as<DeviceUnitig>(), nchunks.as<uint32_t>()}, cU, U_b);
+    exclusive_scan(nchunks.as<uint32_t>(), chunk_off.as<uint32_t>(), (uint64_t)U_b + 1, 0, false, cU1, M + M_CHUNKS);
+    partial.ensure((size_t)chunks_b * sizeof(MinPartial<W>));
+    ac_launch_n<AcSetNUnitigs>("chunk_min", &stream, ChunkMinBody<W>{packed.as<uint64_t>(), seqs.as<SeqInfo>(), n_seqs, p, unitigs.as<DeviceUnitig>(), 0,
+                                                                                    chunk_off.as<uint32_t>(), partial.as<MinPartial<W>>()}, dcount(M_CHUNKS), chunks_b, cU);
+    ac_launch_n("unitig_min", &stream, UnitigMinBody<W>{chunk_off.as<uint32_t>(), partial.as<MinPartial<W>>(), unitigs.as<DeviceUnitig>()}, cU, U_b);
     mark(8);
 
-    link_count.ensure((size_t)n_unitigs * 2 * 4); links.ensure((size_t)n_unitigs * 2 * AC_MAX_LINKS * 4);
-    ac_launch("links", &stream, LinkBody<W>{tv, p, any_dotted, unitigs.as<DeviceUnitig>(), pos_slot.as<uint32_t>(), slot_unitig.as<uint32_t>(),
-                                            link_count.as<uint32_t>(), links.as<uint32_t>()}, (uint64_t)n_unitigs * 2);
+    link_count.ensure((size_t)strands_b * 4); links.ensure((size_t)strands_b * AC_MAX_LINKS * 4);
+    ac_launch_n("links", &stream, LinkBody<W>{tv, p, any_dotted, unitigs.as<DeviceUnitig>(), pos_slot.as<uint32_t>(), slot_unitig.as<uint32_t>(),
+                                              link_count.as<uint32_t>(), links.as<uint32_t>()}, cS, strands_b);
     mark(9);
 
-    const uint32_t U = n_unitigs;
-    sort_a.ensure((size_t)U * 4); sort_b.ensure((size_t)U * 4); sort_ra.ensure((size_t)U * sizeof(SortRec)); sort_rb.ensure((size_t)U * sizeof(SortRec));
+    sort_a.ensure((size_t)U_b * 4); sort_b.ensure((size_t)U_b * 4); sort_ra.ensure((size_t)U_b * sizeof(SortRec)); sort_rb.ensure((size_t)U_b * sizeof(SortRec));
     const SeedLess seed_less{unitigs.as<DeviceUnitig>(), W};
-    const uint32_t* perm = sort_indices(&stream, seed_less, U, sort_a.as<uint32_t>(), sort_b.as<uint32_t>(), sort_ra.as<SortRec>(), sort_rb.as<SortRec>());
+    const uint32_t* perm = sort_indices(&stream, seed_less, U_b, sort_a.as<uint32_t>(), sort_b.as<uint32_t>(), sort_ra.as<SortRec>(), sort_rb.as<SortRec>(), cU);
     mark(10);
 
-    rank.ensure((size_t)U * 4); d_len.ensure((size_t)U * 4); d_depth.ensure((size_t)U * 4); need.ensure(((size_t)U + 1) * 4);
-    d_seq_off.ensure((size_t)U * 8); d_min_fpos.ensure((size_t)U * 4); d_min_rpos.ensure((size_t)U * 4);
-    ac_launch("seed_gather", &stream, SeedGatherBody{perm, unitigs.as<DeviceUnitig>(), U, rank.as<uint32_t>(), d_len.as<uint32_t>(), d_depth.as<uint32_t>(),
-                                                     need.as<uint32_t>(), d_min_fpos.as<uint32_t>(), d_min_rpos.as<uint32_t>()}, (uint64_t)U + 1);
-    {
-        if (n_windows + (uint64_t)U * 2 * AC_SEQ_SLACK >= 0xFFFFFFF0ull) throw std::runtime_error("unitig sequence arena would exceed 4 GB");
-    }
-    const uint64_t arena_bytes = exclusive_scan(need.as<uint32_t>(), need.as<uint32_t>(), (uint64_t)U + 1);
-    ac_launch("seq_off", &stream, SeqOffBody{need.as<uint32_t>(), d_seq_off.as<uint64_t>()}, U);
-    d_arena.ensure(arena_bytes);
-    ac_launch("emit_seq", &stream, EmitSeqBody{packed.as<uint64_t>(), p.h, unitigs.as<DeviceUnitig>(), U, chunk_off.as<uint32_t>(), rank.as<uint32_t>(),
-                                               d_seq_off.as<uint64_t>(), d_arena.as<char>()}, n_chunks);
-    const uint32_t n_strands = 2 * U;
-    strand_cnt.ensure(((size_t)n_strands + 1) * 4); d_next_off.ensure(((size_t)n_strands + 1) * 4);
-    prev_cnt.ensure(((size_t)n_strands + 1) * 4); d_prev_off.ensure(((size_t)n_strands + 1) * 4);
-    ac_launch("link_count", &stream, LinkCountBody{link_count.as<uint32_t>(), rank.as<uint32_t>(), unitigs.as<DeviceUnitig>(), n_strands, strand_cnt.as<uint32_t>()},
-              (uint64_t)n_strands + 1);
-    const uint64_t n_links = exclusive_scan(strand_cnt.as<uint32_t>(), d_next_off.as<uint32_t>(), (uint64_t)n_strands + 1);
-    d_next.ensure(n_links * 4); d_prev.ensure(n_links * 4);
-    ac_memset(prev_cnt.p, 0, ((size_t)n_strands + 1) * 4, &stream);
-    d_small.ensure(64); ac_memset(d_small.p, 0, 64, &stream);
-    ac_launch("link_order", &stream, LinkOrderBody{link_count.as<uint32_t>(), links.as<uint32_t>(), rank.as<uint32_t>(), unitigs.as<DeviceUnitig>(),
-                                                   d_next_off.as<uint32_t>(), d_next.as<UStrand>(), prev_cnt.as<uint32_t>(), d_small.as<uint32_t>()}, n_strands);
-    exclusive_scan(prev_cnt.as<uint32_t>(), d_prev_off.as<uint32_t>(), (uint64_t)n_strands + 1, 0, false);
-    ac_memset(prev_cnt.p, 0, ((size_t)n_strands + 1) * 4, &stream);
-    ac_launch("prev_fill", &stream, PrevFillBody{d_next_off.as<uint32_t>(), d_next.as<UStrand>(), d_prev_off.as<uint32_t>(), prev_cnt.as<uint32_t>(), d_prev.as<UStrand>()}, n_strands);
-    ac_launch("prev_sort", &stream, PrevSortBody{d_prev_off.as<uint32_t>(), d_prev.as<UStrand>()}, n_strands);
+    rank.ensure((size_t)U_b * 4); d_len.ensure((size_t)U_b * 4); d_depth.ensure((size_t)U_b * 4); need.ensure(((size_t)U_b + 1) * 4);
+    d_seq_off.ensure((size_t)U_b * 8); d_min_fpos.ensure((size_t)U_b * 4); d_min_rpos.ensure((size_t)U_b * 4);
+    ac_launch_n<AcSetN>("seed_gather", &stream, SeedGatherBody{perm, unitigs.as<DeviceUnitig>(), 0, rank.as<uint32_t>(), d_len.as<uint32_t>(), d_depth.as<uint32_t>(),
+                                                                         need.as<uint32_t>(), d_min_fpos.as<uint32_t>(), d_min_rpos.as<uint32_t>()}, cU1, (uint64_t)U_b + 1, cU);
+    exclusive_scan(need.as<uint32_t>(), need.as<uint32_t>(), (uint64_t)U_b + 1, 0, false, cU1, M + M_ARENA);
+    ac_launch_n("seq_off", &stream, SeqOffBody{need.as<uint32_t>(), d_seq_off.as<uint64_t>()}, cU, U_b);
+    d_arena.ensure(arena_b);
+    ac_launch_n<AcSetNUnitigs>("emit_seq", &stream, EmitSeqBody{packed.as<uint64_t>(), p.h, unitigs.as<DeviceUnitig>(), 0, chunk_off.as<uint32_t>(), rank.as<uint32_t>(),
+                                                                        d_seq_off.as<uint64_t>(), d_arena.as<char>()}, dcount(M_CHUNKS), chunks_b, cU);
+    strand_cnt.ensure((strands_b + 1) * 4); d_next_off.ensure((strands_b + 1) * 4);
+    prev_cnt.ensure((strands_b + 1) * 4); d_prev_off.ensure((strands_b + 1) * 4);
+    ac_launch_n<AcSetNStrands>("link_count", &stream, LinkCountBody{link_count.as<uint32_t>(), rank.as<uint32_t>(), unitigs.as<DeviceUnitig>(), 0, strand_cnt.as<uint32_t>()},
+                                           cS1, strands_b + 1, cS);
+    exclusive_scan(strand_cnt.as<uint32_t>(), d_next_off.as<uint32_t>(), strands_b + 1, 0, false, cS1, M + M_LINKS);
+    const uint64_t links_b = strands_b * AC_MAX_LINKS;
+    d_next.ensure(links_b * 4); d_prev.ensure(links_b * 4);
+    ac_memset(prev_cnt.p, 0, (strands_b + 1) * 4, &stream);
+    ac_launch_n("link_order", &stream, LinkOrderBody{link_count.as<uint32_t>(), links.as<uint32_t>(), rank.as<uint32_t>(), unitigs.as<DeviceUnitig>(),
+                                                     d_next_off.as<uint32_t>(), d_next.as<UStrand>(), prev_cnt.as<uint32_t>(), M + M_HAIRPINS}, cS, strands_b);
+    exclusive_scan(prev_cnt.as<uint32_t>(), d_prev_off.as<uint32_t>(), strands_b + 1, 0, false, cS1);
+    ac_memset(prev_cnt.p, 0, (strands_b + 1) * 4, &stream);
+    ac_launch_n("prev_fill", &stream, PrevFillBody{d_next_off.as<uint32_t>(), d_next.as<UStrand>(), d_prev_off.as<uint32_t>(), prev_cnt.as<uint32_t>(), d_prev.as<UStrand>()}, cS, strands_b);
+    ac_launch_n("prev_sort", &stream, PrevSortBody{d_prev_off.as<uint32_t>(), d_prev.as<UStrand>()}, cS, strands_b);
     d_path.ensure(n_runs * 4); d_path_off.ensure(((size_t)n_seqs + 1) * 8);
     ac_launch("path", &stream, PathBody{seqs.as<SeqInfo>(), n_seqs, run_start.as<uint64_t>(), run_len.as<uint32_t>(), run_unitig.as<uint32_t>(), rank.as<uint32_t>(),
                                         unitigs.as<DeviceUnitig>(), d_path.as<UStrand>(), d_min_fpos.as<uint32_t>(), d_min_rpos.as<uint32_t>()}, n_runs);
-    d_rec.ensure((size_t)U * sizeof(UnitigRec));
-    ac_launch("pack_rec", &stream, PackRecBody{d_seq_off.as<uint64_t>(), d_len.as<uint32_t>(), d_min_fpos.as<uint32_t>(), d_min_rpos.as<uint32_t>(), d_rec.as<UnitigRec>()}, U);
+    d_rec.ensure((size_t)U_b * sizeof(UnitigRec));
+    ac_launch_n("pack_rec", &stream, PackRecBody{d_seq_off.as<uint64_t>(), d_len.as<uint32_t>(), d_min_fpos.as<uint32_t>(), d_min_rpos.as<uint32_t>(), d_rec.as<UnitigRec>()}, cU, U_b);
     ac_launch("path_off", &stream, PathOffBody{seqs.as<SeqInfo>(), n_seqs, run_start.as<uint64_t>(), n_runs, d_path_off.as<uint64_t>()}, (uint64_t)n_seqs + 1);
-    num_prefix.ensure((size_t)U * 8);
-    ac_launch("number_key", &stream, NumberKeyBody{d_rec.as<UnitigRec>(), d_arena.as<char>(), num_prefix.as<uint64_t>()}, U);
+    num_prefix.ensure((size_t)U_b * 8);
+    ac_launch_n("number_key", &stream, NumberKeyBody{d_rec.as<UnitigRec>(), d_arena.as<char>(), num_prefix.as<uint64_t>()}, cU, U_b);
     const NumberLess number_less{d_rec.as<UnitigRec>(), d_depth.as<uint32_t>(), d_arena.as<char>(), num_prefix.as<uint64_t>(), nullptr};
-    uint32_t* ord_in = sort_indices(&stream, number_less, U, sort_a.as<uint32_t>(), sort_b.as<uint32_t>(), sort_ra.as<SortRec>(), sort_rb.as<SortRec>());
-    d_fixed.ensure((size_t)U * 4); ac_memset(d_fixed.p, 0, (size_t)U * 4, &stream);
-    uint8_t* seed_start = d_fixed.as<uint8_t>(); uint8_t* seed_end = seed_start + U; uint8_t* fix_start = seed_end + U; uint8_t* fix_end = fix_start + U;
+    uint32_t* ord_in = sort_indices(&stream, number_less, U_b, sort_a.as<uint32_t>(), sort_b.as<uint32_t>(), sort_ra.as<SortRec>(), sort_rb.as<SortRec>(), cU);
+    d_fixed.ensure((size_t)U_b * 4); ac_memset(d_fixed.p, 0, (size_t)U_b * 4, &stream);
+    uint8_t* seed_start = d_fixed.as<uint8_t>(); uint8_t* seed_end = seed_start + U_b; uint8_t* fix_start = seed_end + U_b; uint8_t* fix_end = fix_start + U_b;
     ac_launch("fixed_seed", &stream, FixedSeedBody{d_path_off.as<uint64_t>(), d_path.as<UStrand>(), seed_start, seed_end}, n_seqs);
-    ac_copy_dd(fix_start, seed_start, (size_t)U * 2, &stream);
-    ac_launch("fixed_spread", &stream, FixedSpreadBody{seed_start, seed_end, d_next_off.as<uint32_t>(), d_next.as<UStrand>(), d_prev_off.as<uint32_t>(), d_prev.as<UStrand>(),
-                                                       fix_start, fix_end}, U);
+    ac_copy_dd(fix_start, seed_start, (size_t)U_b * 2, &stream);
+    ac_launch_n("fixed_spread", &stream, FixedSpreadBody{seed_start, seed_end, d_next_off.as<uint32_t>(), d_next.as<UStrand>(), d_prev_off.as<uint32_t>(), d_prev.as<UStrand>(),
+                                                         fix_start, fix_end}, cU, U_b);
     const CandidateView cview{ord_in, d_next_off.as<uint32_t>(), d_next.as<UStrand>(), d_prev_off.as<uint32_t>(), d_prev.as<UStrand>(), fix_start, fix_end};
-    cand_flag.ensure((2 * (size_t)U + 1) * 4); cand_index.ensure((2 * (size_t)U + 1) * 4);
-    ac_launch("candidate_flag", &stream, CandidateFlagBody{cview, U, cand_flag.as<uint32_t>()}, 2ull * U + 1);
-    const uint64_t n_cands = exclusive_scan(cand_flag.as<uint32_t>(), cand_index.as<uint32_t>(), 2ull * U + 1);
-    d_cands.ensure((n_cands + 1) * sizeof(ExpandCandidate)); d_cand_at.ensure(2 * (size_t)U * 4 + 4); d_deps.ensure((size_t)U * sizeof(ExpandDeps) + 4); d_spec.ensure((n_cands + 1) * 4);
-    ac_launch("candidate_fill", &stream, CandidateFillBody{cview, cand_flag.as<uint32_t>(), cand_index.as<uint32_t>(), d_cands.as<ExpandCandidate>(), d_cand_at.as<int32_t>()}, 2ull * U);
-    ac_launch("dependents", &stream, DependentsBody{d_next_off.as<uint32_t>(), d_next.as<UStrand>(), d_prev_off.as<uint32_t>(), d_prev.as<UStrand>(), d_cand_at.as<int32_t>(),
-                                                    d_deps.as<ExpandDeps>()}, U);
-    ac_launch("common_length", &stream, CommonLengthBody{d_cands.as<ExpandCandidate>(), d_rec.as<UnitigRec>(), d_arena.as<char>(), d_spec.as<uint32_t>()}, n_cands);
+    cand_flag.ensure(cands_b * 4); cand_index.ensure(cands_b * 4);
+    ac_launch_n<AcSetN>("candidate_flag", &stream, CandidateFlagBody{cview, 0, cand_flag.as<uint32_t>()}, cS1, cands_b, cU);
+    exclusive_scan(cand_flag.as<uint32_t>(), cand_index.as<uint32_t>(), cands_b, 0, false, cS1, M + M_CANDS);
+    d_cands.ensure((cands_b + 1) * sizeof(ExpandCandidate)); d_cand_at.ensure(strands_b * 4 + 4); d_deps.ensure((size_t)U_b * sizeof(ExpandDeps) + 4); d_spec.ensure((cands_b + 1) * 4);
+    ac_launch_n("candidate_fill", &stream, CandidateFillBody{cview, cand_flag.as<uint32_t>(), cand_index.as<uint32_t>(), d_cands.as<ExpandCandidate>(), d_cand_at.as<int32_t>()}, cS, strands_b);
+    ac_launch_n("dependents", &stream, DependentsBody{d_next_off.as<uint32_t>(), d_next.as<UStrand>(), d_prev_off.as<uint32_t>(), d_prev.as<UStrand>(), d_cand_at.as<int32_t>(),
+                                                      d_deps.as<ExpandDeps>()}, cU, U_b);
+    ac_launch_n("common_length", &stream, CommonLengthBody{d_cands.as<ExpandCandidate>(), d_rec.as<UnitigRec>(), d_arena.as<char>(), d_spec.as<uint32_t>()}, cC, cands_b);
+    d_counters64.ensure((AC_PASS_WORDS + 8) * 8);
+    unsigned long long* c64 = d_counters64.as<unsigned long long>();
+    unsigned long long* res = c64 + AC_PASS_WORDS;
+    ac_memset(d_counters64.p, 0, (AC_PASS_WORDS + 8) * 8, &stream);
+    const RelocBoundBody bound_body{d_cands.as<ExpandCandidate>(), d_rec.as<UnitigRec>(), d_cand_at.as<int32_t>(), c64 + AC_PASS_SET(1) + 1};
+    if (fused) ac_launch_n("reloc_bound", &stream, bound_body, cC, cands_b);
+    h_meta.ensure(M_WORDS * 4 + AC_BOUND_STRIPES * 8);
+    ac_d2h(h_meta.p, M, M_WORDS * 4, &stream);
+    ac_d2h(h_meta.as<char>() + M_WORDS * 4, c64 + AC_PASS_SET(1) + 1, AC_BOUND_STRIPES * 8, &stream);
+    ac_sync(&stream);
+    const uint32_t* hm = h_meta.as<uint32_t>();
+    n_slots_used = is_multi ? n_slots_used : hm[M_KMERS];
+    out.n_slots_used = n_slots_used;
+    const uint32_t U = hm[M_UNITIGS], n_chunks = hm[M_CHUNKS];
+    const uint64_t arena_bytes = hm[M_ARENA], n_links = hm[M_LINKS], n_cands = hm[M_CANDS];
+    if (n_slots_used > n_b || U > U_b || n_chunks > chunks_b || arena_bytes > arena_b || n_links > links_b || n_cands > cands_b)
+        throw std::runtime_error("a graph count exceeds the bound its buffers were sized by");
+    const uint32_t n_strands = 2 * U;
     R = Pending();
-    R.U = U; R.n_links = n_links; R.n_cands = n_cands; R.n_strands = n_strands; R.order_built = ord_in; R.fix_start = fix_start;
+    R.U = U; R.U_b = U_b; R.n_links = n_links; R.n_cands = n_cands; R.n_strands = n_strands; R.order_built = ord_in; R.fix_start = fix_start; R.fix_end = fix_end;
+    R.hairpins = hm[M_HAIRPINS];
     R.arena_final = arena_bytes; R.arena_src = &d_arena;
     mark(11);
     if (fused && n_cands > 0) {
-        d_pred.ensure(n_cands * 7 * 4); d_level.ensure(n_cands * 4); d_flagmax.ensure(32); d_counters64.ensure((AC_PASS_WORDS + 8) * 8);
+        d_pred.ensure(n_cands * 7 * 4); d_level.ensure(n_cands * 4); d_flagmax.ensure(32);
         d_dirty.ensure(((n_cands + 63) / 64) * 8 + 8); d_exhausted.ensure(n_cands + 8);
-        unsigned long long* c64 = d_counters64.as<unsigned long long>();
-        unsigned long long* res = c64 + AC_PASS_WORDS;
         ac_launch("level_pred", &stream, LevelPredBody{d_cands.as<ExpandCandidate>(), d_deps.as<ExpandDeps>(), d_pred.as<int32_t>()}, n_cands);
         ac_memset(d_level.p, 0, n_cands * 4, &stream); ac_memset(d_flagmax.p, 0, 32, &stream);
         ac_launch_coop("levels", &stream, LevelsCoopBody{d_pred.as<int32_t>(), d_level.as<uint32_t>(), d_flagmax.as<uint32_t>(), n_cands}, n_cands, 4096);
-        ac_memset(d_counters64.p, 0, (AC_PASS_WORDS + 8) * 8, &stream);
-        const RelocBoundBody bound_body{d_cands.as<ExpandCandidate>(), d_rec.as<UnitigRec>(), d_cand_at.as<int32_t>(), c64 + AC_PASS_SET(1) + 1};
-        ac_launch("reloc_bound", &stream, bound_body, n_cands);
-        uint32_t fm[8]; unsigned long long h64[AC_PASS_WORDS + 8];
-        ac_d2h(fm, d_flagmax.p, 32, &stream); ac_d2h(h64, c64, sizeof h64, &stream); ac_sync(&stream);
-        if (fm[4]) throw std::runtime_error("candidate levels did not settle");
-        unsigned long long bound = 0; for (int x = 0; x < AC_BOUND_STRIPES; ++x) bound += h64[AC_PASS_SET(1) + 1 + x];
+        unsigned long long h64[AC_PASS_WORDS + 8]; uint32_t fm[8];
+        const unsigned long long* hb = (const unsigned long long*)(h_meta.as<char>() + M_WORDS * 4);
+        unsigned long long bound = 0; for (int x = 0; x < AC_BOUND_STRIPES; ++x) bound += hb[x];
         if (arena_bytes + bound >= 0xFFFFFFF0ull) throw std::runtime_error("unitig sequence arena would exceed 4 GB");
         d_arena2.ensure(arena_bytes + 2 * bound + 64);
         ac_copy_dd(d_arena2.p, d_arena.p, arena_bytes, &stream);
@@ -2786,7 +2834,7 @@
         ac_memset(d_dirty.p, 0, ((n_cands + 63) / 64) * 8 + 8, &stream); ac_memset(d_exhausted.p, 0, n_cands + 8, &stream);
         static const bool always_grow = getenv("AC_DEVICE_TIGHT_ARENA") != nullptr;
         uint32_t next_set = 0, next_due = 0; uint64_t passes = 0;
-        const uint32_t due_stride = fm[3] + 2;
+        const uint32_t due_stride = (uint32_t)n_cands + 2;
         d_due.ensure((size_t)3 * due_stride * 4); ac_memset(d_due.p, 0, (size_t)3 * due_stride * 4, &stream);
         for (bool first = true;; first = false) {
             const ApplyLevelBody apply{d_cands.as<ExpandCandidate>(), d_deps.as<ExpandDeps>(), d_level.as<uint32_t>(), 0, d_spec.as<uint32_t>(),
@@ -2794,7 +2842,8 @@
             const uint64_t room = always_grow ? 0 : d_arena2.cap;
             ac_launch_coop("simplify", &stream, SimplifyCoopBody{apply, bound_body, n_cands, d_flagmax.as<uint32_t>() + 3, c64, res, room, next_set, first,
                                                                  d_due.as<uint32_t>(), due_stride, next_due}, n_cands, 64);
-            ac_d2h(h64, c64, sizeof h64, &stream); ac_sync(&stream);
+            ac_d2h(h64, c64, sizeof h64, &stream); ac_d2h(fm, d_flagmax.p, 32, &stream); ac_sync(&stream);
+            if (fm[4]) throw std::runtime_error("candidate levels did not settle");
             const unsigned long long* r = h64 + AC_PASS_WORDS;
             R.arena_final = h64[0]; R.bases_removed = h64[AC_PASS_REMOVED]; R.any_moved = r[1] != 0;
             passes += r[2]; next_set = (uint32_t)r[5]; next_due = (uint32_t)r[7];
@@ -2805,7 +2854,7 @@
             bound = r[3];
             if (R.arena_final + bound >= 0xFFFFFFF0ull) throw std::runtime_error("unitig sequence arena would exceed 4 GB");
             d_arena3.ensure(std::max<size_t>((R.arena_final + bound) * 2 + 64, d_arena3.cap + (always_grow ? 64 : 0)));
-            ac_copy_dd(d_arena3.p, d_arena2.p, R.arena_final, &stream); ac_sync(&stream);
+            ac_copy_dd(d_arena3.p, d_arena2.p, R.arena_final, &stream);
             std::swap(d_arena2.p, d_arena3.p); std::swap(d_arena2.cap, d_arena3.cap);
         }
         R.arena_src = &d_arena2;
@@ -2869,14 +2918,13 @@
     if (before_results && *before_results) (*before_results)();
     out.fused = fused; out.graph_fetched = false;
     if (fused && !R.gfa_on_device) throw std::runtime_error("fused build: the device GFA writer did not run");
-    uint64_t d2h = 0;
+    uint64_t d2h = M_WORDS * 4 + AC_BOUND_STRIPES * 8;
     if (R.gfa_on_device) {
         h_text.ensure(R.gfa_bytes + 64);
         ac_d2h(h_text.p, d_text.p, R.gfa_bytes, &stream); d2h += R.gfa_bytes;
     }
-    uint32_t small[16];
-    ac_d2h(small, d_small.p, 64, &stream); ac_sync(&stream); d2h += 64;
-    out.links_single = (n_links - small[0]) / 2 + small[0];
+    if (R.gfa_on_device) ac_sync(&stream);
+    out.links_single = (n_links - R.hairpins) / 2 + R.hairpins;
     out.length_before = n_slots_used;
     out.length_after = n_slots_used - R.bases_removed;
     out.gfa_text = R.gfa_on_device ? h_text.as<char>() : nullptr; out.gfa_bytes = R.gfa_on_device ? R.gfa_bytes : 0;
@@ -2908,7 +2956,7 @@
     if (plain) {
         h_cands.ensure((n_cands + 1) * sizeof(ExpandCandidate)); h_deps.ensure((size_t)U * sizeof(ExpandDeps) + 4); h_spec.ensure((n_cands + 1) * 4); h_fixed.ensure((size_t)U * 2 + 4);
         pull(h_cands, d_cands, n_cands * sizeof(ExpandCandidate)); pull(h_deps, d_deps, (size_t)U * sizeof(ExpandDeps)); pull(h_spec, d_spec, n_cands * 4);
-        if (U) { ac_d2h(h_fixed.p, R.fix_start, (size_t)U * 2, &stream); d2h += (size_t)U * 2; }
+        if (U) { ac_d2h(h_fixed.p, R.fix_start, U, &stream); ac_d2h(h_fixed.as<uint8_t>() + U, R.fix_end, U, &stream); d2h += (size_t)U * 2; }
     } else { h_order2.ensure((size_t)U * 4 + 4); if (U) { ac_d2h(h_order2.p, R.final_order, (size_t)U * 4, &stream); d2h += (size_t)U * 4; } }
     mark(16);
     pull(h_arena, *R.arena_src, R.arena_final);
diff --git a/autocycler_b200/csrc/pipeline.h b/autocycler_b200/csrc/pipeline.h
--- a/autocycler_b200/csrc/pipeline.h
+++ b/autocycler_b200/csrc/pipeline.h
@@ -122,6 +122,7 @@
     void find_literals(const uint8_t* ascii, uint64_t total, const SeqInfo* seqs, uint32_t n_seqs, uint32_t h,
                        const uint64_t* needle_words, uint32_t n_needles, std::vector<LiteralHit>& hits);
     unsigned long long kernel_launches() const;
+    unsigned long long host_waits() const;
     struct Impl;
 private:
     Impl* impl;
diff --git a/include/autocycler_gpu.h b/include/autocycler_gpu.h
--- a/include/autocycler_gpu.h
+++ b/include/autocycler_gpu.h
@@ -62,6 +62,7 @@
     uint64_t table_capacity, table_used;
     uint64_t kernel_launches;
     uint64_t h2d_bytes, d2h_bytes;
+    uint64_t host_waits;
 } ac_timings;
 
 const char* ac_last_error(const ac_handle* h);
diff --git a/profiles/idle_gaps.py b/profiles/idle_gaps.py
--- /dev/null
+++ b/profiles/idle_gaps.py
@@ -0,0 +1,100 @@
+import argparse
+import json
+import os
+import sys
+import tempfile
+
+ap = argparse.ArgumentParser()
+ap.add_argument("--workload", default="cfg2")
+ap.add_argument("--k", type=int, default=51)
+ap.add_argument("--steps", type=int, default=3)
+ap.add_argument("--warmup", type=int, default=3)
+ap.add_argument("--gap-us", type=float, default=8.0, help="list the gaps at least this long")
+ap.add_argument("--root", default=os.path.dirname(os.path.dirname(os.path.abspath(__file__))))
+ap.add_argument("--out", default=None)
+args = ap.parse_args()
+sys.path.insert(0, os.path.abspath(args.root))
+
+import torch
+from torch.profiler import ProfilerActivity, profile
+
+from autocycler_b200 import api, synth
+
+with tempfile.TemporaryDirectory() as d:
+    synth.write_assemblies(synth.make_assemblies(args.workload), d)
+    kg, seqs, count = api.load_sequences(d, args.k)
+kg.upload()
+
+
+def step():
+    return api.UnitigGraph.compress(kg)
+
+
+for _ in range(args.warmup):
+    step()
+torch.cuda.synchronize()
+t0 = api.AcTimings(); kg._h.lib.ac_timings_get(kg._h.ptr, t0)
+with profile(activities=[ProfilerActivity.CUDA, ProfilerActivity.CPU]) as prof:
+    for _ in range(args.steps):
+        torch.cuda.synchronize()
+        step()
+        torch.cuda.synchronize()
+t1 = api.AcTimings(); kg._h.lib.ac_timings_get(kg._h.ptr, t1)
+
+with tempfile.TemporaryDirectory() as d:
+    path = os.path.join(d, "trace.json")
+    prof.export_chrome_trace(path)
+    trace = json.load(open(path))
+gpu = [e for e in trace["traceEvents"] if e.get("ph") == "X" and e.get("cat") in ("kernel", "gpu_memcpy", "gpu_memset")]
+gpu.sort(key=lambda e: e["ts"])
+gaps = [(gpu[i + 1]["ts"] - (gpu[i]["ts"] + gpu[i]["dur"]), i) for i in range(len(gpu) - 1)]
+cuts = sorted(i for _, i in sorted(gaps, reverse=True)[: args.steps - 1])
+bounds = [0] + [i + 1 for i in cuts] + [len(gpu)]
+
+
+def short(name):
+    name = name.split("(")[0]
+    for key in ("Body", "kernel"):
+        j = name.find(key)
+        if j > 0:
+            s = name.rfind("<", 0, j)
+            return name[s + 1: j + len(key)] if s >= 0 else name[: j + len(key)]
+    return name[:60]
+
+
+per_step = []
+for s in range(args.steps):
+    ev = gpu[bounds[s]: bounds[s + 1]]
+    span = ev[-1]["ts"] + ev[-1]["dur"] - ev[0]["ts"]
+    busy = 0.0; idle = 0.0; listed = []
+    for i, e in enumerate(ev):
+        busy += e["dur"]
+        if i + 1 < len(ev):
+            gap = ev[i + 1]["ts"] - (e["ts"] + e["dur"])
+            if gap > 0:
+                idle += gap
+            if gap >= args.gap_us:
+                listed.append({"gap_us": round(gap, 1), "after": short(e["name"]), "before": short(ev[i + 1]["name"])})
+    per_step.append({"span_us": round(span, 1), "busy_us": round(busy, 1), "idle_us": round(idle, 1), "activities": len(ev),
+                     "idle_in_long_gaps_us": round(sum(x["gap_us"] for x in listed), 1), "long_gaps": listed})
+
+name = torch.cuda.get_device_name()
+props = {"device": name}
+try:
+    import subprocess
+    props["nvidia_smi"] = subprocess.run(["nvidia-smi", "--query-gpu=name,power.limit,clocks.max.sm,clocks.sm", "--format=csv,noheader"],
+                                         capture_output=True, text=True, timeout=30).stdout.strip()
+except Exception as exc:
+    props["nvidia_smi"] = str(exc)
+waits = getattr(t1, "host_waits", None)
+out = {"root": os.path.abspath(args.root), "workload": args.workload, "k": args.k, "gpu": props,
+       "host_waits_per_step": None if waits is None else (t1.host_waits - t0.host_waits) / args.steps,
+       "steps": per_step}
+text = json.dumps(out, indent=1)
+print(json.dumps({"root": out["root"], "workload": args.workload, "host_waits_per_step": out["host_waits_per_step"],
+                  "span_us": [p["span_us"] for p in per_step], "idle_us": [p["idle_us"] for p in per_step],
+                  "long_gaps_us": [p["idle_in_long_gaps_us"] for p in per_step], "n_long_gaps": [len(p["long_gaps"]) for p in per_step]}))
+if args.out:
+    os.makedirs(os.path.dirname(os.path.abspath(args.out)), exist_ok=True)
+    with open(args.out, "w") as f:
+        f.write(text)
```

Result: no change. 5359, median of 6 (+0.7%).
